# aras-p/ToyPathTracer

Hardware: AMD Instinct MI355X
Metric: Mray/s (higher is better)
Workload: dtype f32

## Files before the change

include/tpt_hip.h:

```cpp
#ifndef TPT_HIP_H
#define TPT_HIP_H
#include <stdint.h>

#if defined(__GNUC__)
#define TPT_API __attribute__((visibility("default")))
#else
#define TPT_API
#endif

#ifdef __cplusplus
extern "C" {
#endif

enum { TPT_FLAG_ANIMATE = 1 << 0, TPT_FLAG_PROGRESSIVE = 1 << 1 };


TPT_API int tptInitialize(void);
TPT_API int tptShutdown(void);
TPT_API int tptUpdate(float time, int frameCount, int screenWidth, int screenHeight, unsigned testFlags);
TPT_API int tptDraw(float time, int frameCount, int screenWidth, int screenHeight, float* backbuffer, int* outRayCount,
            unsigned testFlags);
TPT_API int tptSetHostBufferMode(int hostBufferOnlyWrittenByDrawTest);
TPT_API int tptSetHostLookahead(int frames);
TPT_API int tptGetLookaheadHits(long long* outHits);
TPT_API int tptGetObjectCount(int* outCount, int* outObjectSize, int* outMaterialSize, int* outCamSize);
TPT_API int tptGetSceneDesc(void* outObjects, void* outMaterials, void* outCam, void* outEmissives, int* outEmissiveCount);


TPT_API int tptSetSamplesPerPixel(int spp);
TPT_API int tptSetConfig(int lightSampling, float animateSmoothing, int mitsubaCompare);
TPT_API int tptSetSeedMode(int mode);
TPT_API int tptSetFoldMode(int mode);
TPT_API int tptSetScene(const void* spheres, const void* materials, int count);
TPT_API int tptSetCamera(const float* lookFrom, const float* lookAt, float vfovDegrees, float aperture, float focusDist);


TPT_API int tptSetStream(void* hipStream);
TPT_API int tptSetRowShard(int stripeRows, int numParts, int part);
TPT_API int tptLocalRowCount(int screenHeight);
TPT_API int tptLocalRowToGlobal(int localRow);
TPT_API int tptDrawDevice(float time, int frameCount, int screenWidth, int screenHeight, float* deviceTile, unsigned testFlags);
TPT_API int tptDrawDeviceBatch(float time, int firstFrame, int nFrames, int screenWidth, int screenHeight, float* deviceTile, unsigned testFlags);
TPT_API int tptDrawDeviceAnimation(int firstFrame, int nFrames, const float* times, int screenWidth, int screenHeight,
                                   float* deviceTile, float* deviceFrameImages, int64_t* deviceFrameRays, unsigned testFlags);
TPT_API int tptDrawDeviceAov(float time, int frameCount, int screenWidth, int screenHeight, float* deviceTile,
                             float* deviceAlbedo, float* deviceNormalDepth, unsigned testFlags);
enum { TPT_DENOISE_DEMODULATE = 1 << 0 };
TPT_API int tptDenoiseDevice(int screenWidth, int screenHeight, const float* deviceColour, const float* deviceAlbedo,
                             const float* deviceNormalDepth, float* deviceOut, int iterations, float sigmaColour,
                             float sigmaNormal, float sigmaDepth, unsigned denoiseFlags);
TPT_API int tptDrawDeviceMoments(float time, int frameCount, int screenWidth, int screenHeight, float* deviceTile,
                                 float* deviceAlbedo, float* deviceNormalDepth, float* deviceMoments, unsigned testFlags);
TPT_API int tptDrawDeviceAnimationMoments(int firstFrame, int nFrames, const float* times, int screenWidth, int screenHeight,
                                          float* deviceTile, float* deviceMoments,
                                          float* deviceFrameImages, float* deviceFrameAlbedo, float* deviceFrameNormalDepth,
                                          float* deviceFrameMoments, int64_t* deviceFrameRays, unsigned testFlags);
TPT_API int tptDrawDeviceCameraClip(int firstFrame, int nFrames, const float* times, const float* views,
                                    int screenWidth, int screenHeight, float* deviceTile, float* deviceMoments,
                                    float* deviceFrameImages, float* deviceFrameAlbedo, float* deviceFrameNormalDepth,
                                    float* deviceFrameMoments, int64_t* deviceFrameRays, void* outCameras, unsigned testFlags);
#define TPT_DENOISE_VARIANCE_EPS 1e-4f
TPT_API int tptDenoiseDeviceVariance(int screenWidth, int screenHeight, const float* deviceColour, const float* deviceAlbedo,
                                     const float* deviceNormalDepth, const float* deviceMoments, float samples, float* deviceOut,
                                     int iterations, float sigmaLuminance, float sigmaNormal, float sigmaDepth, unsigned denoiseFlags);
#define TPT_TEMPORAL_SNAP (1.0f / 128)
TPT_API int tptTemporalAccumulateDevice(int screenWidth, int screenHeight, const void* camera, const void* prevCamera,
                                        const float* deviceColour, const float* deviceAlbedo, const float* deviceNormalDepth,
                                        const float* deviceMoments, const float* devicePrevColour, const float* devicePrevAlbedo,
                                        const float* devicePrevNormalDepth, const float* devicePrevMoments, float* deviceOutColour,
                                        float* deviceOutAlbedo, float* deviceOutMoments, float* deviceOutVariance, float maxHistory,
                                        float depthTolerance, float normalTolerance, float coverageTolerance);
TPT_API int tptDrawDeviceAdaptive(float time, int frameCount, int screenWidth, int screenHeight, float* deviceTile, float* deviceAlbedo,
                                  float* deviceNormalDepth, float* deviceMoments, const int32_t* deviceSampleCounts,
                                  unsigned testFlags);
#define TPT_ADAPTIVE_LUM_FLOOR 1e-2f
TPT_API int tptAdaptiveSamplesDevice(int screenWidth, int screenHeight, const float* deviceMoments, float targetError, int minSamples,
                                     int maxSamples, int32_t* deviceSampleCounts, float* deviceOutVariance,
                                     int64_t* deviceTotalSamples);
TPT_API int tptDrawDeviceViews(float time, int frameCount, int screenWidth, int screenHeight, int nViews, const float* views,
                               float* deviceTiles, int64_t* deviceViewRays, unsigned testFlags);
TPT_API int tptSetFrameOverlap(int frames);
TPT_API int tptSetStreamBatching(int enable);
TPT_API int tptDisplayRGBA8(const float* deviceTile, int screenWidth, int screenHeight, unsigned char* deviceRGBA);
TPT_API int tptRayCounterRead(int64_t* outTotalRays);
TPT_API int tptSetRayCounter(void* deviceU64);
TPT_API int tptSetTileMirror(float* deviceMirror, void* deviceCounterOut);
TPT_API int tptSynchronize(void);

#define TPT_COMM_ID_BYTES 128
TPT_API int tptCommGetUniqueId(void* outId128);
TPT_API int tptCommInit(const void* id128, int nRanks, int rank, int stripeRows);
TPT_API int tptCommInitLoopback(int nRanks, int stripeRows);
TPT_API int tptCommInfo(int* outRanks, int* outRank, int* outLoopback);
TPT_API int tptCommDestroy(void);
TPT_API int tptDrawSharded(float time, int frameCount, int screenWidth, int screenHeight, float* deviceImageOnRoot, unsigned testFlags);
TPT_API int tptSetShardExchangeInterval(int everyKFrames);
TPT_API int tptDrawShardedBatch(float time, int firstFrame, int nFrames, int screenWidth, int screenHeight, float* deviceImageOnRoot, unsigned testFlags);
TPT_API int tptShardedFinish(int64_t* outTotalRays);

TPT_API int tptTimerBegin(void);
TPT_API int tptTimerEnd(float* outMilliseconds);

TPT_API int tptKernelTimingBegin(int maxLaunches);
TPT_API int tptKernelTimingEnd(float* outSumMilliseconds, int* outLaunches);


TPT_API int tptSetKernelVariant(int hitSpheres, int persistent, int ldsScene);
TPT_API int tptGetSceneInfo(int* outSpheres, int* outGroups, int* outBoundsOnMatrixCores);
TPT_API int tptGetLaunchInfo(int* outBlocksPerCU, int* outLdsBytes, int* outGridBlocks, int* outNumCUs);
TPT_API int tptGetPipelineInfo(int* outHwQueues, int* outOverlapEffective, int* outStreamDepth, int* outSlotReservations);
TPT_API const char* tptGetLastError(void);
typedef void (*tptErrorHandler)(const char* where, const char* message);
TPT_API int tptSetErrorHandler(tptErrorHandler handler);
TPT_API const char* tptGetDeviceName(void);

#ifdef __cplusplus
}
#endif
#endif
```

include/tpt_test_hooks.h:

```cpp
#ifndef TPT_TEST_HOOKS_H
#define TPT_TEST_HOOKS_H
#include "tpt_hip.h"
#ifdef __cplusplus
extern "C" {
#endif
TPT_API int tptTestMath(int op, const float* a, const float* b, float* out, int n);
TPT_API int tptTestHitSpheres(int hitSpheres, const float* rays, int* outId, float* outT, int n);
TPT_API int tptTestMathExhaustive(int op, unsigned lo, unsigned hi, unsigned long long* outMismatches, unsigned* outFirst8);
TPT_API int tptTestMatrixFilter(const float* rays, unsigned long long* outMask, int* outId, float* outT, int n);
TPT_API int tptTestGroupFilter(const float* rays, int n, unsigned long long* outViolations, unsigned long long* outTouched, unsigned long long* outExact);
TPT_API int tptTestSetDealCapacities(int superGroupEntries, int groupEntries, int survivorEntries);
TPT_API int tptDebugStats(unsigned long long* out128, int reset);
TPT_API int tptDebugChunkOrder(unsigned* outCost, unsigned* outOrder, int capacity);
#ifdef __cplusplus
}
#endif
#endif
```

toypathtracer_amd/api.py:

```python
import ctypes as C
import os

import numpy as np

kFlagAnimate = 1 << 0
kFlagProgressive = 1 << 1
SEED_ROW_SERIAL, SEED_PER_PIXEL = 0, 1
FOLD_RECURSIVE, FOLD_FORWARD = 0, 1

SPHERE_DT = np.dtype([("cx", "<f4"), ("cy", "<f4"), ("cz", "<f4"), ("radius", "<f4"), ("invRadius", "<f4")])
MATERIAL_DT = np.dtype([("type", "<i4"), ("albedo", "<f4", 3), ("emissive", "<f4", 3), ("roughness", "<f4"), ("ri", "<f4")])
CAMERA_DT = np.dtype([("origin", "<f4", 3), ("lowerLeftCorner", "<f4", 3), ("horizontal", "<f4", 3), ("vertical", "<f4", 3),
                      ("uu", "<f4", 3), ("vv", "<f4", 3), ("ww", "<f4", 3), ("lensRadius", "<f4")])


class TptError(RuntimeError):
    pass


_lib = None
_product = None
_hooks = None

C_ABI_SYMBOLS = [
    "tptInitialize", "tptShutdown", "tptUpdate", "tptDraw", "tptGetObjectCount", "tptGetSceneDesc",
    "tptSetSamplesPerPixel", "tptSetConfig", "tptSetSeedMode", "tptSetFoldMode", "tptSetScene", "tptSetCamera", "tptSetStream",
    "tptSetRowShard", "tptLocalRowCount", "tptLocalRowToGlobal", "tptDrawDevice", "tptRayCounterRead", "tptSetRayCounter", "tptSetFrameOverlap", "tptDisplayRGBA8", "tptKernelTimingBegin", "tptKernelTimingEnd",
    "tptSynchronize", "tptTimerBegin", "tptTimerEnd", "tptSetKernelVariant",
    "tptDrawDeviceBatch", "tptDrawDeviceViews", "tptDrawDeviceAnimation", "tptDrawDeviceAov", "tptDenoiseDevice", "tptDrawDeviceMoments", "tptDrawDeviceAnimationMoments", "tptDrawDeviceCameraClip", "tptDenoiseDeviceVariance", "tptTemporalAccumulateDevice", "tptDrawDeviceAdaptive", "tptAdaptiveSamplesDevice", "tptDrawShardedBatch", "tptGetLookaheadHits", "tptCommGetUniqueId", "tptCommInit", "tptCommInitLoopback", "tptCommInfo", "tptCommDestroy", "tptDrawSharded", "tptSetShardExchangeInterval", "tptShardedFinish", "tptGetLaunchInfo", "tptGetPipelineInfo", "tptGetSceneInfo", "tptSetHostBufferMode", "tptSetHostLookahead", "tptSetStreamBatching", "tptSetTileMirror", "tptGetLastError", "tptSetErrorHandler", "tptGetDeviceName",
]
HOOK_SYMBOLS = ["tptTestMath", "tptTestMathExhaustive", "tptTestHitSpheres", "tptTestMatrixFilter", "tptTestGroupFilter", "tptTestSetDealCapacities", "tptDebugStats", "tptDebugChunkOrder"]
CXX_ABI_SYMBOLS = [
    "_Z14InitializeTestv", "_Z12ShutdownTestv", "_Z10UpdateTestfiiij", "_Z8DrawTestfiiiPfRij",
    "_Z14GetObjectCountRiS_S_S_", "_Z12GetSceneDescPvS_S_S_Pi",
]


def _lib_dir():
    return os.environ.get("TPT_LIB_DIR") or os.path.join(os.path.dirname(os.path.abspath(__file__)), "lib")


def library_path():
    return os.environ.get("TPT_LIB") or os.path.join(_lib_dir(), "libtoypathtracer_hip.so")


def hooks_library_path():
    return os.environ.get("TPT_LIB") or os.path.join(_lib_dir(), "libtoypathtracer_hip_hooks.so")


def _bind(path, hooks):
    lib = C.CDLL(path)
    i, f, u, p = C.c_int, C.c_float, C.c_uint, C.c_void_p
    sigs = {
        "tptInitialize": [], "tptShutdown": [], "tptUpdate": [f, i, i, i, u],
        "tptDraw": [f, i, i, i, p, C.POINTER(i), u],
        "tptGetObjectCount": [C.POINTER(i)] * 4, "tptGetSceneDesc": [p, p, p, p, C.POINTER(i)],
        "tptSetSamplesPerPixel": [i], "tptSetConfig": [i, f, i], "tptSetSeedMode": [i], "tptSetFoldMode": [i], "tptSetScene": [p, p, i],
        "tptSetCamera": [p, p, f, f, f], "tptSetStream": [p], "tptSetRowShard": [i, i, i], "tptLocalRowCount": [i],
        "tptLocalRowToGlobal": [i], "tptDrawDevice": [f, i, i, i, p, u], "tptRayCounterRead": [C.POINTER(C.c_int64)],
        "tptSetRayCounter": [p], "tptSetTileMirror": [p, p], "tptSetFrameOverlap": [i], "tptDisplayRGBA8": [p, i, i, p], "tptKernelTimingBegin": [i],
        "tptKernelTimingEnd": [C.POINTER(f), C.POINTER(i)],
        "tptSynchronize": [], "tptTimerBegin": [], "tptTimerEnd": [C.POINTER(f)], "tptSetKernelVariant": [i, i, i],
        "tptGetLaunchInfo": [C.POINTER(i)] * 4, "tptGetPipelineInfo": [C.POINTER(i)] * 4, "tptGetSceneInfo": [C.POINTER(i)] * 3, "tptCommGetUniqueId": [p], "tptCommInit": [p, i, i, i], "tptCommInitLoopback": [i, i], "tptCommInfo": [C.POINTER(i)] * 3, "tptCommDestroy": [], "tptDrawSharded": [f, i, i, i, p, u], "tptSetShardExchangeInterval": [i], "tptDrawShardedBatch": [f, i, i, i, i, p, u], "tptDrawDeviceBatch": [f, i, i, i, i, p, u], "tptDrawDeviceViews": [f, i, i, i, i, p, p, p, u], "tptDrawDeviceAnimation": [i, i, p, i, i, p, p, p, u], "tptDrawDeviceAov": [f, i, i, i, p, p, p, u], "tptDenoiseDevice": [i, i, p, p, p, p, i, f, f, f, u], "tptDrawDeviceMoments": [f, i, i, i, p, p, p, p, u], "tptDrawDeviceAnimationMoments": [i, i, p, i, i] + [p] * 7 + [u], "tptDrawDeviceCameraClip": [i, i, p, p, i, i] + [p] * 8 + [u], "tptDenoiseDeviceVariance": [i, i, p, p, p, p, f, p, i, f, f, f, u], "tptTemporalAccumulateDevice": [i, i] + [p] * 14 + [f] * 4, "tptDrawDeviceAdaptive": [f, i, i, i, p, p, p, p, p, u], "tptAdaptiveSamplesDevice": [i, i, p, f, i, i, p, p, p], "tptShardedFinish": [C.POINTER(C.c_int64)], "tptSetHostBufferMode": [i], "tptGetLookaheadHits": [C.POINTER(C.c_longlong)], "tptSetHostLookahead": [i], "tptSetStreamBatching": [i],
    }
    if hooks:
        sigs.update({"tptDebugStats": [p, i], "tptDebugChunkOrder": [p, p, i], "tptTestMath": [i, p, p, p, i], "tptTestMathExhaustive": [i, u, u, p, p],
                     "tptTestHitSpheres": [i, p, p, p, i], "tptTestMatrixFilter": [p, p, p, p, i], "tptTestGroupFilter": [p, i, p, p, p], "tptTestSetDealCapacities": [i, i, i]})
    for name, args in sigs.items():
        fn = getattr(lib, name)
        fn.argtypes = args
        fn.restype = i
    lib.tptGetLastError.restype = C.c_char_p
    lib.tptGetDeviceName.restype = C.c_char_p
    return lib


def _preload():
    try:
        import torch
    except ImportError:
        pass


def load_library():
    global _lib, _product
    if _lib is not None:
        return _lib
    _preload()
    path = library_path()
    if not os.path.exists(path):
        raise TptError(f"{path} is missing: build it with `python -c 'import __graft_entry__ as g; g.build()'` "
                       "(toypathtracer_amd/csrc/build.sh). There is no CPU fallback.")
    _product = _bind(path, hooks=bool(os.environ.get("TPT_LIB")) and _has_hooks(path))
    _lib = _product
    return _lib


def _has_hooks(path):
    try:
        return hasattr(C.CDLL(path), "tptTestMath")
    except OSError:
        return False


class using_hooks:

    def __enter__(self):
        global _lib, _hooks
        load_library()
        if _hooks is None:
            path = hooks_library_path()
            if path == library_path():
                _hooks = _product
            else:
                if not os.path.exists(path):
                    raise TptError(f"{path} is missing (toypathtracer_amd/csrc/build.sh builds it beside the product library)")
                _hooks = _bind(path, hooks=True)
        self._prev = _lib
        _lib = _hooks
        _chk(_lib.tptInitialize(), "tptInitialize (hooks build)")
        return self

    def __exit__(self, *exc):
        global _lib
        if _lib is not _product:
            _lib.tptShutdown()
        _lib = self._prev
        return False


def shutdown_hooks():
    global _hooks
    if _hooks is not None and _hooks is not _product:
        _hooks.tptShutdown()
    _hooks = None


def _hook(name):
    fn = getattr(load_library(), name, None)
    if fn is None:
        raise TptError(f"{name} is a unit-test hook (include/tpt_test_hooks.h): call it inside `with api.using_hooks():` -- the product library does not export it")
    return fn


def _chk(rc, where):
    if rc != 0:
        raise TptError(f"{where}: {_lib.tptGetLastError().decode()}")


def InitializeTest():
# ... 382 lines not shown
def temporal_accumulate_device(w, h, camera, colour_ptr, albedo_ptr, normal_depth_ptr, moments_ptr, out_colour_ptr, out_albedo_ptr,
                               out_moments_ptr, out_variance_ptr, prev=None, max_history=TEMPORAL_DEFAULTS["max_history"],
                               depth_tolerance=TEMPORAL_DEFAULTS["depth_tolerance"],
                               normal_tolerance=TEMPORAL_DEFAULTS["normal_tolerance"],
                               coverage_tolerance=TEMPORAL_DEFAULTS["coverage_tolerance"]):
    _positive_ints(("w", w), ("h", h))
    cur = (("colour_ptr", colour_ptr), ("albedo_ptr", albedo_ptr), ("normal_depth_ptr", normal_depth_ptr), ("moments_ptr", moments_ptr),
           ("out_colour_ptr", out_colour_ptr), ("out_albedo_ptr", out_albedo_ptr), ("out_moments_ptr", out_moments_ptr),
           ("out_variance_ptr", out_variance_ptr))
    _pointers(*cur)
    if not all(v for _, v in cur):
        raise ValueError("%s: device buffers are required" % ", ".join(n for n, v in cur if not v))
    cam = _camera_bytes("camera", camera)
    prev_cam, prev_ptrs = None, (None,) * 4
    if prev is not None:
        if not isinstance(prev, (tuple, list)) or len(prev) != 5:
            raise ValueError("prev: None or (camera, colour_ptr, albedo_ptr, normal_depth_ptr, moments_ptr) expected, got %r" % (prev,))
        prev_cam = _camera_bytes("prev camera", prev[0])
        named = tuple(zip(("prev colour_ptr", "prev albedo_ptr", "prev normal_depth_ptr", "prev moments_ptr"), prev[1:]))
        _pointers(*named)
        if not all(v for _, v in named):
            raise ValueError("prev: all four device buffers are required")
        prev_ptrs = tuple(C.c_void_p(v) for v in prev[1:])
    if not isinstance(max_history, (int, float, np.integer, np.floating)) or isinstance(max_history, bool) or not 1 <= max_history <= 65536:
        raise ValueError("max_history: a number in 1..65536 expected, got %r" % (max_history,))
    _sigmas(("depth_tolerance", depth_tolerance), ("normal_tolerance", normal_tolerance), ("coverage_tolerance", coverage_tolerance))
    _chk(load_library().tptTemporalAccumulateDevice(w, h, cam, prev_cam, C.c_void_p(colour_ptr), C.c_void_p(albedo_ptr),
                                                    C.c_void_p(normal_depth_ptr), C.c_void_p(moments_ptr), *prev_ptrs,
                                                    C.c_void_p(out_colour_ptr), C.c_void_p(out_albedo_ptr), C.c_void_p(out_moments_ptr),
                                                    C.c_void_p(out_variance_ptr), max_history, depth_tolerance, normal_tolerance,
                                                    coverage_tolerance), "tptTemporalAccumulateDevice")


ADAPTIVE_MAX_SAMPLES = 2047


def draw_device_adaptive(time, frame, w, h, tile_ptr, moments_ptr, counts_ptr, flags, albedo_ptr=None, normal_depth_ptr=None):
    _positive_ints(("w", w), ("h", h))
    _pointers(("tile_ptr", tile_ptr), ("moments_ptr", moments_ptr), ("counts_ptr", counts_ptr), ("albedo_ptr", albedo_ptr),
              ("normal_depth_ptr", normal_depth_ptr))
    if not tile_ptr or not moments_ptr or not counts_ptr:
        raise ValueError("tile_ptr, moments_ptr, counts_ptr: device buffers are required")
    _chk(load_library().tptDrawDeviceAdaptive(time, frame, w, h, C.c_void_p(tile_ptr), C.c_void_p(albedo_ptr) if albedo_ptr else None,
                                              C.c_void_p(normal_depth_ptr) if normal_depth_ptr else None, C.c_void_p(moments_ptr),
                                              C.c_void_p(counts_ptr), flags), "tptDrawDeviceAdaptive")


def adaptive_samples_device(w, h, moments_ptr, target_error, counts_ptr, min_samples=0, max_samples=64, out_variance_ptr=None,
                            total_ptr=None):
    _positive_ints(("w", w), ("h", h))
    _pointers(("moments_ptr", moments_ptr), ("counts_ptr", counts_ptr), ("out_variance_ptr", out_variance_ptr), ("total_ptr", total_ptr))
    if not moments_ptr or not counts_ptr:
        raise ValueError("moments_ptr, counts_ptr: device buffers are required")
    if not isinstance(target_error, (int, float, np.integer, np.floating)) or isinstance(target_error, bool) or not 0 < target_error <= 1e6:
        raise ValueError("target_error: a float in (0, 1e6] expected, got %r" % (target_error,))
    for name, v in (("min_samples", min_samples), ("max_samples", max_samples)):
        if not isinstance(v, (int, np.integer)) or isinstance(v, bool) or not 0 <= v <= ADAPTIVE_MAX_SAMPLES:
            raise ValueError("%s: an int in 0..%d expected, got %r" % (name, ADAPTIVE_MAX_SAMPLES, v))
    if min_samples > max_samples:
        raise ValueError("min_samples: at most max_samples (%d) expected, got %d" % (max_samples, min_samples))
    _chk(load_library().tptAdaptiveSamplesDevice(w, h, C.c_void_p(moments_ptr), target_error, min_samples, max_samples,
                                                 C.c_void_p(counts_ptr), C.c_void_p(out_variance_ptr) if out_variance_ptr else None,
                                                 C.c_void_p(total_ptr) if total_ptr else None), "tptAdaptiveSamplesDevice")


def sharded_finish():
    v = C.c_int64()
    _chk(load_library().tptShardedFinish(C.byref(v)), "tptShardedFinish")
    return v.value


def set_host_buffer_mode(only_written_by_drawtest):
    _chk(load_library().tptSetHostBufferMode(1 if only_written_by_drawtest else 0), "tptSetHostBufferMode")


def set_host_lookahead(frames):
    _chk(load_library().tptSetHostLookahead(frames), "tptSetHostLookahead")


def set_stream_batching(enable):
    _chk(load_library().tptSetStreamBatching(1 if enable else 0), "tptSetStreamBatching")


def lookahead_hits():
    v = C.c_longlong()
    _chk(load_library().tptGetLookaheadHits(C.byref(v)), "tptGetLookaheadHits")
    return v.value


def pipeline_info():
    v = [C.c_int() for _ in range(4)]
    _chk(load_library().tptGetPipelineInfo(*[C.byref(x) for x in v]), "tptGetPipelineInfo")
    return dict(hw_queues=v[0].value, overlap_effective=v[1].value, stream_depth=v[2].value, slot_reservations=v[3].value)


def scene_info():
    v = [C.c_int() for _ in range(3)]
    _chk(load_library().tptGetSceneInfo(*[C.byref(x) for x in v]), "tptGetSceneInfo")
    return dict(spheres=v[0].value, groups=v[1].value, bounds_on_matrix_cores=bool(v[2].value))


def debug_stats(reset=True):
    out = np.zeros(128, np.uint64)
    _chk(_hook("tptDebugStats")(out.ctypes.data, 1 if reset else 0), "tptDebugStats")
    return out


def debug_chunk_order(capacity=1 << 20):
    cost = np.zeros(capacity, np.uint32)
    order = np.zeros(capacity, np.uint32)
    n = _hook("tptDebugChunkOrder")(cost.ctypes.data, order.ctypes.data, capacity)
    if n < 0:
        raise TptError("tptDebugChunkOrder: " + _lib.tptGetLastError().decode())
    return cost[:n].copy(), order[:n].copy()


def device_name():
    return load_library().tptGetDeviceName().decode()


def test_math(op, a, b=None):
    a = np.ascontiguousarray(a, np.float32)
    out = np.empty_like(a)
    bp = None
    if b is not None:
        b = np.ascontiguousarray(b, np.float32)
        bp = b.ctypes.data
    _chk(_hook("tptTestMath")(op, a.ctypes.data, bp, out.ctypes.data, a.size), "tptTestMath")
    return out


def test_math_exhaustive(op, lo=0, hi=0xFFFFFFFF):
    bad = C.c_ulonglong(0)
    first = (C.c_uint * 8)()
    _chk(_hook("tptTestMathExhaustive")(op, lo, hi, C.byref(bad), first), "tptTestMathExhaustive")
    return int(bad.value), [int(v) for v in first][: min(8, int(bad.value))]


def test_hit_spheres(rays, hit_spheres=0):
    rays = np.ascontiguousarray(rays, np.float32).reshape(-1, 6)
    n = rays.shape[0]
    ids = np.empty(n, np.int32)
    ts = np.empty(n, np.float32)
    _chk(_hook("tptTestHitSpheres")(hit_spheres, rays.ctypes.data, ids.ctypes.data, ts.ctypes.data, n),
         "tptTestHitSpheres")
    return ids, ts


def test_matrix_filter(rays, hits=False):
    rays = np.ascontiguousarray(rays, np.float32).reshape(-1, 6)
    n = rays.shape[0]
    masks = np.empty(n, np.uint64)
    ids = np.empty(n, np.int32) if hits else None
    ts = np.empty(n, np.float32) if hits else None
    _chk(_hook("tptTestMatrixFilter")(rays.ctypes.data, masks.ctypes.data, ids.ctypes.data if hits else None,
                                            ts.ctypes.data if hits else None, n), "tptTestMatrixFilter")
    return (masks, ids, ts) if hits else masks


def test_set_deal_capacities(super_group_entries=0, group_entries=0, survivor_entries=0):
    _chk(_hook("tptTestSetDealCapacities")(super_group_entries, group_entries, survivor_entries), "tptTestSetDealCapacities")


def test_group_filter(rays):
    rays = np.ascontiguousarray(rays, np.float32).reshape(-1, 6)
    n = rays.shape[0]
    v = [C.c_ulonglong(0) for _ in range(3)]
    _chk(_hook("tptTestGroupFilter")(rays.ctypes.data, n, C.byref(v[0]), C.byref(v[1]), C.byref(v[2])), "tptTestGroupFilter")
    return int(v[0].value), v[1].value / n, v[2].value / n
```

toypathtracer_amd/csrc/tpt_context.h:

```cpp
#pragma once
#include "../../include/tpt_hip.h"
#if defined(TPT_TEST_HOOKS)
#include "../../include/tpt_test_hooks.h"
#endif
#include "../../include/tpt_test_api.h"
#include "tpt_device.h"
#include "tpt_queue_layout.h"
#include "tpt_scene.h"
#include "tpt_shard.h"
#include "tpt_stream_batch.h"
#include "tpt_animation.h"
#include <hip/hip_runtime.h>
#include <thread>
#include <rccl/rccl.h>
#include <chrono>
#include <dlfcn.h>
#include <map>
#include <stdio.h>
#include <stdlib.h>
#include <string>


namespace tpth {
using namespace tpt;

const int kMaxBatch = 32;
static_assert(kMaxBatch == TPT_Q_VIEWS_MAX, "a batch's cameras, centres and ray counts have their places in the path-queue kernel's LDS");
struct TraceTicket {
    int slot = 0, nPixels = 0;
    bool pipelined = false, valid = false;
    float lerpFac = 0;
    const f4* colour = nullptr;
    int batch = 1;
    tptLerpTable lerp = {};
    const f4* moments = nullptr;
    TraceTicket plane(int j) const
    {
        TraceTicket t = *this;
        t.colour = colour + (size_t)j * (size_t)nPixels;
        if (batch > 1) t.lerpFac = lerp.v[j];
        t.batch = 1;
        return t;
    }
};

struct Streak {
    int frame = 0, w = 0, h = 0, n = 0;
    unsigned flags = 0;
    unsigned long long key = 0;
    int next(int frame_, int w_, int h_, unsigned flags_, unsigned long long key_)
    {
        n = frame_ == frame + 1 && w_ == w && h_ == h && flags_ == flags && key_ == key ? n + 1 : 0;
        frame = frame_; w = w_; h = h_; flags = flags_; key = key_;
        return n;
    }
};

struct PendingLaunch {
    enum Kind { AHEAD, ROW_SERIAL, STREAM } kind = AHEAD;
    TraceTicket T;
    int firstFrame = 0, next = 0;
    int w = 0, h = 0;
    unsigned flags = 0;
    unsigned long long key = 0;
    unsigned long long* rays = nullptr;
};
struct LaunchQueue {
    static const int kCap = 4;
    PendingLaunch e[kCap];
    int n = 0;
    bool empty() const { return n == 0; }
    bool holds(PendingLaunch::Kind kind) const { return n > 0 && e[0].kind == kind; }
    bool frontMatches(PendingLaunch::Kind kind, int frame, int w, int h, unsigned flags, unsigned long long key) const;
    void serveFront(bool wasOpen, TraceTicket& T, const unsigned long long*& rays);
    int push(const PendingLaunch& L);
    int discard();
    void closeStream();
};

struct Context {
    static const int kMaxOverlap = 16;
    static const int kMaxSlots = 2 * kMaxOverlap;
    static const int kOrderTables = kMaxSlots + 2;
    bool inited = false;
    int device = 0, numCUs = 0;
    int traceCUs = 0;
    std::string deviceName, err;
    hipStream_t ownStream = nullptr, stream = nullptr;
    hipEvent_t ev0 = nullptr, ev1 = nullptr;

    std::vector<SpherePOD> spheres;
    std::vector<MaterialPOD> mats;
    CameraSetup camSetup = defaultCameraSetup();
    CameraPOD cam;
    PackedScene packed;
    bool sceneDirty = true;
    bool updated = false;
    int updatedW = 0, updatedH = 0;

    static const int kSceneSets = 2 * kMaxSlots;
    struct SceneSet {
        char* dev = nullptr;
        char* stage = nullptr;
        size_t cap = 0, bytes = 0;
        size_t offSph4 = 0, offInvR = 0, offMats = 0, offLights = 0;
        size_t offGPairs = 0, offGSph = 0, offGId = 0, offBSph = 0, offBId = 0;
        size_t offSPairs = 0;
        int nSuperPairs = 0;
        size_t offAmat = 0;
        int mxR1 = -1;
        size_t offGmat = 0;
        int gmxTiles = 0;
        int flags = 0;
        int nSpheres = 0, nPairs = 0, nLights = 0;
        int nGroups = 0, nGroupPairs = 0, nBig = 0;
        hipEvent_t evUploaded = nullptr;
        hipStream_t uploadStream = nullptr;
        bool copyEnqueued = false, copyDone = false;
    } sets[kSceneSets];
    int curSet = -1, pendingSet = -1;
    unsigned uploadSeq = 0;

    int spp = 4;
    int config = CFG_LIGHT_SAMPLING;
    float animateSmoothing = 0.9f;
    int seedMode = SEED_PER_PIXEL;
    int foldMode = FOLD_RECURSIVE;
    int allowGroups = 1;
    int useMatrix = 1;
    int groupMatrix = 0;
    int hs = HS_TWO_PHASE, persist = 3, ldsScene = -1;
    int stripeRows = 0, numParts = 1, part = 0;
    int gridFill = 0;
    int gridDiv = 0;
    unsigned long long oldestPending = 0;
    int streamDepth = 1, prevInFlight = -1;
    int depthOverride = 0;
    int ldsStackLevels = 6;

    float* mirror = nullptr;
    unsigned long long* mirrorCounter = nullptr;
    unsigned* dWork = nullptr;
    unsigned long long* dRays = nullptr;
    unsigned long long* dRaysOwn = nullptr;
    long long lastTotal = 0;

    f4* dStack[kMaxSlots] = {};
    size_t stackCap = 0, colourCap = 0;
    int slotsReserved = 0;
    int smallStreak = 0;
    int slotReservations = 0;
    unsigned* dChunkCost = nullptr;
    unsigned* dChunkOrder[kOrderTables] = {};
    unsigned* dChunkSnap[kMaxOverlap] = {};
    int chunkCap = 0, chunkCount = 0;
    int costOrder = 1;
    hipEvent_t evOrder = nullptr;
    hipStream_t orderStream = nullptr;
    unsigned long long orderSeq = 0;
    int lastOrderTable = 0;
    float* dFrame = nullptr;
    hipStream_t hostStream2 = nullptr;
    hipEvent_t evBand = nullptr, evBandEnd = nullptr;
    int hostTrust = 0;
    const float* tileSrc = nullptr;
    int tileW = 0, tileH = 0;
    int lookahead = 2;
    LaunchQueue pending;
    struct HostCaller {
        Streak seq;
        int refusedW = 0, refusedH = 0;
        unsigned long long refusedKey = 0;
    } hostCaller;
    static const int kStreamBatchMax = 8, kStreamRing = 64;
    unsigned long long streamBatches = 0;
    int streamRun = 0, streamNext = -1;
    int streamBatch = 1;
    struct DeviceCaller {
        int lastSlot = -1, syncStreak = 0;
        Streak seq;
    } devCaller;
    struct ViewSlot {
        CameraPOD* dev = nullptr;
        unsigned long long* rays = nullptr;
        CameraPOD* stage = nullptr;
        hipEvent_t evUploaded = nullptr;
        bool copyEnqueued = false;
    } views[kMaxSlots];
    char* dViews = nullptr;
    CameraPOD* hViewsStage = nullptr;
    f4* dAovSums = nullptr;
    size_t aovSumsBytes = 0;
    hipEvent_t evAov = nullptr;
    f4* dMoments = nullptr;
    size_t momentsBytes = 0;
    hipEvent_t evClip[2] = {nullptr, nullptr};
    unsigned clipSeq = 0;
    f4* dDenoise = nullptr;
    size_t denoiseBytes = 0;
    long long aheadHits = 0;
    unsigned long long *dRaysAhead = nullptr, *dRaysBatch = nullptr, *dRaysStream = nullptr;
    unsigned long long configEpoch = 1;

    struct Shard {
        static const int kRing = 4;
        void* lib = nullptr;
        ncclComm_t comm = nullptr;
        bool active = false, loopback = false;
        int nRanks = 0, rank = 0, stripeRows = 8;
        int w = 0, h = 0, padRows = 0;
        hipStream_t commStream = nullptr;
        float* tile = nullptr;
        float* send[kRing] = {};
        float* gathered = nullptr;
        hipEvent_t evSnap[kRing] = {}, evSent[kRing] = {};
        bool sentRecorded[kRing] = {};
        unsigned long long frames = 0;
        int exchangeEvery = 0;
        int pendCount = 0, pendFirst = 0, pendW = 0, pendH = 0;
        unsigned pendFlags = 0;
        float pendTime = 0.0f;
        float* lastImage = nullptr;
        decltype(&ncclGetUniqueId) GetUniqueId = nullptr;
        decltype(&ncclCommInitRank) CommInitRank = nullptr;
        decltype(&ncclCommDestroy) CommDestroy = nullptr;
        decltype(&ncclGather) Gather = nullptr;
        decltype(&ncclCommCount) CommCount = nullptr;
        decltype(&ncclCommUserRank) CommUserRank = nullptr;
        decltype(&ncclGetErrorString) GetErrorString = nullptr;
    } shard;
    size_t frameCap = 0;

    int overlap = 16;
    hipStream_t traceStream[kMaxOverlap] = {};
    hipEvent_t evTrace[kMaxSlots] = {}, evResolve[kMaxSlots] = {};
    bool resolveRecorded[kMaxSlots] = {};
    f4* dColour[kMaxSlots] = {};
    int hwQueues = 0, overlapCap = kMaxOverlap;
    int slotFactor = 2;
    hipEvent_t evPre[kMaxSlots] = {};
    struct HelperRec {
        KernelArgs a;
        bool ldsScene = false, valid = false, helped = false;
        hipStream_t ts = nullptr;
        int blocks = 0, maxBlocks = 0;
        size_t lds = 0;
    } hrec[kMaxSlots];
    unsigned launchGen = 0;
    int helpersOn = 1;
    static const int kHelperPct = 3;
    static const int kHelperMax = 8;
    long long helperLaunches = 0;
    int hostPace = 1;
    int shardOverlapCap = kMaxOverlap;
    unsigned long long frameSeq = 0;

    bool kernelTiming = false;
    std::vector<hipEvent_t> ktStart, ktStop;
    size_t ktUsed = 0;

    std::map<int, int> occCache;
    int lastBlocksPerCU = 0, lastLds = 0, lastGrid = 0;
};

extern Context g;

struct DepthScope {
    explicit DepthScope(int d) { g.depthOverride = d; }
    ~DepthScope() { g.depthOverride = 0; }
};

const unsigned kOrderingEvent = hipEventDisableTiming;
const unsigned kTimingEvent = hipEventDefault;

inline int fail(const std::string& what)
{
    g.err = what;
    return -1;
}
inline int hipFail(hipError_t e, const char* what)
{
    g.err = std::string(what) + ": " + hipGetErrorString(e);
    (void)hipGetLastError();
    return -2;
}
const int kRefused = -4;
inline int refuse(const std::string& what)
{
    g.err = what;
    return kRefused;
}
inline bool overlapsAny(const void* p, std::initializer_list<const void*> others, uintptr_t bytes)
{
    const uintptr_t a = reinterpret_cast<uintptr_t>(p);
    for (const void* other : others) {
        const uintptr_t o = reinterpret_cast<uintptr_t>(other);
        if (other && a < o + bytes && o < a + bytes) return true;
    }
    return false;
}
#define HIPCHK(x)                                   \
    do {                                            \
        hipError_t _e = (x);                        \
        if (_e != hipSuccess) return hipFail(_e, #x); \
    } while (0)

int localRows(int h);
int localToGlobal(int ly);
int stageScene();
Context::SceneSet* activeSet();
SceneView deviceView();
int enqueueSceneUpload(hipStream_t ts);
int framesInFlight(int nOverlap);
int uploadBackbuffer(const float* backbuffer, int w, int h);
int requireInit();
int drainPipeline();
int effectiveOverlap();
struct BatchTable {
    const CameraPOD* cams = nullptr;
    const f4* centres = nullptr;
};
struct AovPlanes {
    f4* albedo = nullptr;
    f4* normalDepth = nullptr;
    bool moments = false;
    bool continues = false;
    const int32_t* sampleCounts = nullptr;
};
int enqueueTrace(int frameCount, int w, int h, unsigned testFlags, unsigned long long* frameRays, TraceTicket& T, int batch = 1, int rayStride = 0,
                 const BatchTable* table = nullptr, const AovPlanes* aov = nullptr);
int enqueueResolve(const TraceTicket& T, float* deviceTile, const unsigned long long* frameRays);
int syncAllStreams();
int launchTailHelpers();
int flushShardDeferred();
int traceAhead(int frameCount, int w, int h, unsigned testFlags, unsigned long long key, int want);

}
```

toypathtracer_amd/csrc/tpt_device.h:

```cpp
#pragma once
#include "tpt_trace.h"

#ifndef TPT_BLOCK
#define TPT_BLOCK 64
#endif
#define TPT_CHUNK_PIXELS 256

namespace tpt {

struct KernelArgs {
    SceneView scene;
    FrameConsts fc;
    f4* frameColour;
    int nLocalRows, stripeRows, stripeStride, stripeOffset;
    int tilesX;
    int numItems;
    int numChunks, chunkSize;
    int batchFrames, chunksPerFrame, framePlane;
    unsigned totalWaves;
    int laneCap;
    int noRefill;
    f4* stackBuf;
    int stackStride;
    int ldsStackLevels;
    f4* pathBuf;
    const unsigned* chunkOrder;
    unsigned* chunkCost;
    int chunkShift;
    unsigned* work;
    unsigned long long* rayCounter;
    int rayCounterStride;
    unsigned gen;
    int helperBase;
    int helperPct;
    int ldsGroupPairs;
    const CameraPOD* viewCams = nullptr;
    const f4* moveCentres = nullptr;
    f4* aovSums = nullptr;
    f4* aovAlbedo = nullptr;
    f4* aovNormalDepth = nullptr;
    f4* momentsOut = nullptr;
    int aovPlane = 0;
    const int32_t* sampleCounts = nullptr;
};

}

hipError_t tptLaunchTrace(const tpt::KernelArgs& a, int hs, int fold, bool ldsScene, int blocks, size_t lds, hipStream_t stream);
int tptTraceOccupancy(int hs, int fold, bool ldsScene, size_t lds);
hipError_t tptLaunchTraceQueue(const tpt::KernelArgs& a, bool ldsScene, int blocks, size_t lds, hipStream_t stream);
int tptQueueMatrixFilter();
int tptQueueGroupMatrixBounds();
hipError_t tptLaunchDisplay(const float* tile, unsigned char* rgba, int width, int height, hipStream_t stream);
__attribute__((weak)) hipError_t tptLaunchDenoise(const float* colour, const float* albedo, const float* normalDepth, float* out,
                                                  float* scratch, int width, int height, int iterations, float ic, float in, float id,
                                                  bool demodulate, hipStream_t stream);
__attribute__((weak)) hipError_t tptLaunchDenoiseVariance(const float* colour, const float* albedo, const float* normalDepth,
                                                          const float* moments, float* out, float* scratch, int width, int height,
                                                          int iterations, float samples, float sl2, float in, float id, bool demodulate,
                                                          hipStream_t stream);
struct tptTemporalConsts {
    float o[3], ll[3], H[3], V[3];
    float po[3], pa[3], pw[3], pH[3], pV[3];
    float pf, phh, pvv;
    float maxHistory, depthTol, normalTol, coverageTol;
};
__attribute__((weak)) hipError_t tptLaunchTemporal(const float* colour, const float* albedo, const float* normalDepth, const float* moments,
                                                   const float* prevColour, const float* prevAlbedo, const float* prevNormalDepth,
                                                   const float* prevMoments, float* outColour, float* outAlbedo, float* outMoments,
                                                   float* outVariance, int width, int height, const tptTemporalConsts& k,
                                                   hipStream_t stream);
__attribute__((weak)) hipError_t tptLaunchAdaptiveResolve(float* tile, float* moments, const tpt::f4* frameColour, const tpt::f4* stagedMoments,
                                                          const int32_t* counts, int nPixels, bool progressive, hipStream_t stream);
__attribute__((weak)) hipError_t tptLaunchAdaptivePlan(const float* moments, int32_t* counts, float* outVariance, int64_t* totalSamples,
                                                       int width, int height, float targetError, int minSamples, int maxSamples,
                                                       hipStream_t stream);
hipError_t tptLaunchAssemble(const float* gathered, float* image, int width, int height, int stripeRows, int nRanks, int padRows, hipStream_t stream);
hipError_t tptLaunchQueueProbe(unsigned long long ticks, hipStream_t stream);
hipError_t tptLaunchChunkOrder(const unsigned* cost, unsigned* snap, unsigned* order, int numChunks, hipStream_t stream);
struct tptLerpTable { float v[32]; };
hipError_t tptLaunchResolveBatch(float* tile, const tpt::f4* frameColour, int nPixels, int planeStride, int nFrames, const tptLerpTable& lerp,
                                 float* mirror, unsigned long long* rayCounter, unsigned long long* counterOut, hipStream_t stream);
hipError_t tptLaunchResolve(float* tile, const tpt::f4* frameColour, int nPixels, float lerpFac, float* mirror,
                            unsigned long long* rayCounter, unsigned long long* counterOut, const unsigned long long* frameRays, hipStream_t stream);
hipError_t tptLaunchMathTest(int op, const float* a, const float* b, float* out, int n, hipStream_t stream);
hipError_t tptLaunchMathExhaustive(int op, unsigned lo, unsigned hi, unsigned long long* nBad, unsigned* firstBad, hipStream_t stream);
hipError_t tptLaunchMatrixFilterTest(const tpt::KernelArgs& a, const float* rays, unsigned long long* outMask, int* outId, float* outT, int n, hipStream_t stream);
hipError_t tptSetDealCapacitiesForTest(int ca, int cb, int cs);
hipError_t tptLaunchGroupFilterTest(const tpt::KernelArgs& a, const float* rays, int n, int nPad, unsigned long long* out4, hipStream_t stream);
hipError_t tptLaunchHitTest(const tpt::KernelArgs& a, int hs, const float* rays, int* outId, float* outT, int n, hipStream_t stream);
int tptReadStats(unsigned long long* out64);
int tptResetStats();
```

toypathtracer_amd/csrc/tpt_host.cpp:

```cpp
#include "tpt_context.h"

using namespace tpt;
using namespace tpth;

namespace tpth {

Context g;

int localRows(int h) { return shardLocalRows(h, g.stripeRows, g.numParts, g.part); }
int localToGlobal(int ly) { return shardLocalToGlobal(ly, g.stripeRows, g.numParts, g.part); }

template <class T>
int ensureDev(T*& p, int& cap, int need)
{
    if (need <= cap && p) return 0;
    if (p) HIPCHK(hipFree(p));
    p = nullptr;
    int n = need < 64 ? 64 : need;
    HIPCHK(hipMalloc(reinterpret_cast<void**>(&p), sizeof(T) * (size_t)n));
    cap = n;
    return 0;
}

size_t align256(size_t v) { return (v + 255) & ~(size_t)255; }
// ... 198 lines not shown
}

int createTraceStreams()
{
    g.traceCUs = g.numCUs;
    for (int k = 0; k < Context::kMaxOverlap; ++k) HIPCHK(hipStreamCreateWithFlags(&g.traceStream[k], hipStreamNonBlocking));
    return 0;
}

int drainPipeline()
{
    if (g.inited) {
        if (g.pending.discard()) return -2;
        HIPCHK(hipStreamSynchronize(g.stream));
        for (int k = 0; k < Context::kMaxOverlap; ++k)
            if (g.traceStream[k]) HIPCHK(hipStreamSynchronize(g.traceStream[k]));
    }
    g.oldestPending = g.frameSeq;
    g.streamDepth = 1; g.prevInFlight = -1;
    for (int k = 0; k < Context::kMaxSlots; ++k) g.resolveRecorded[k] = false;
    return 0;
}
int effectiveOverlap()
{
    int n = g.overlap < 1 ? 1 : (g.overlap > Context::kMaxOverlap ? Context::kMaxOverlap : g.overlap);
    if (n > g.overlapCap) n = g.overlapCap;
    if (n > g.shardOverlapCap) n = g.shardOverlapCap;
    return n;
}

}

extern "C" {

const char* tptGetLastError(void) { return g.err.c_str(); }
const char* tptGetDeviceName(void) { return g.deviceName.c_str(); }

int tptInitialize(void)
{
    if (g.inited) return 0;
    int count = 0;
    hipError_t e = hipGetDeviceCount(&count);
    if (e != hipSuccess || count <= 0)
        return fail("tptInitialize: no HIP device visible (this library has no CPU fallback)");
    int dev = 0;
    const char* env = getenv("TPT_DEVICE");
    if (!env) env = getenv("LOCAL_RANK");
    if (env) dev = atoi(env);
    if (dev < 0) return fail("tptInitialize: negative device index in TPT_DEVICE / LOCAL_RANK");
    if (dev >= count) dev = dev % count;
    HIPCHK(hipSetDevice(dev));
    hipDeviceProp_t prop;
    HIPCHK(hipGetDeviceProperties(&prop, dev));
    g.device = dev;
    g.numCUs = prop.multiProcessorCount;
    g.deviceName = std::string(prop.name) + " (" + prop.gcnArchName + ")";
    HIPCHK(hipStreamCreateWithFlags(&g.ownStream, hipStreamDefault));
    g.stream = g.ownStream;
    HIPCHK(hipEventCreateWithFlags(&g.evOrder, kOrderingEvent));
    HIPCHK(hipEventCreate(&g.ev0));
    HIPCHK(hipEventCreate(&g.ev1));
    HIPCHK(hipMalloc(reinterpret_cast<void**>(&g.dWork), 64 * Context::kMaxSlots));
    HIPCHK(hipMemsetAsync(g.dWork, 0, 64 * Context::kMaxSlots, g.stream));
    {
        int rc = createTraceStreams();
        if (rc) return rc;
    }
    for (int k = 0; k < Context::kMaxSlots; ++k) {
        HIPCHK(hipEventCreateWithFlags(&g.evTrace[k], kOrderingEvent));
        HIPCHK(hipEventCreateWithFlags(&g.evResolve[k], kOrderingEvent));
        g.resolveRecorded[k] = false;
    }

    g.frameSeq = 0;
    g.oldestPending = 0;
    HIPCHK(hipStreamCreateWithFlags(&g.hostStream2, hipStreamNonBlocking));
    HIPCHK(hipEventCreateWithFlags(&g.evBand, kOrderingEvent));
    HIPCHK(hipEventCreateWithFlags(&g.evBandEnd, kOrderingEvent));
    const size_t pendingRays = sizeof(unsigned long long) * (Context::kMaxSlots + 2 * kMaxBatch + Context::kStreamRing * Context::kStreamBatchMax);
    HIPCHK(hipMalloc(reinterpret_cast<void**>(&g.dRaysAhead), pendingRays));
    HIPCHK(hipMemsetAsync(g.dRaysAhead, 0, pendingRays, g.stream));
    g.dRaysBatch = g.dRaysAhead + Context::kMaxSlots;
    g.dRaysStream = g.dRaysBatch + 2 * kMaxBatch;
    g.pending.n = 0;
    if (const char* esb = getenv("TPT_STREAM_BATCH")) g.streamBatch = atoi(esb) != 0;
    HIPCHK(hipMalloc(reinterpret_cast<void**>(&g.dRaysOwn), 64));
    HIPCHK(hipMemsetAsync(g.dRaysOwn, 0, 64, g.stream));
    HIPCHK(hipStreamSynchronize(g.stream));
    g.dRays = g.dRaysOwn;
    g.lastTotal = 0;
    if (g.spheres.empty()) defaultScene(g.spheres, g.mats);
    if (const char* e6 = getenv("TPT_GRID_FILL")) g.gridFill = atoi(e6);
    if (const char* e7 = getenv("TPT_HOST_PACE")) g.hostPace = atoi(e7);
    if (const char* eh = getenv("TPT_TAIL_HELPERS")) g.helpersOn = atoi(eh) != 0;
    for (int k = 0; k < Context::kMaxSlots; ++k) {
        HIPCHK(hipEventCreateWithFlags(&g.evPre[k], kOrderingEvent));
        g.hrec[k].valid = false;
    }
    g.launchGen = 0;
    if (const char* e5 = getenv("TPT_GRID_DIV")) g.gridDiv = atoi(e5) > 0 ? atoi(e5) : 0;
    g.sceneDirty = true;
    {
        int rc = probeHardwareQueues();
        if (rc) return rc;
    }
    g.inited = true;
    return 0;
}

int tptShutdown(void)
{
    if (!g.inited) return 0;
    (void)g.pending.discard();
    (void)tptCommDestroy();
    (void)hipStreamSynchronize(g.stream);
    (void)hipDeviceSynchronize();
    for (int k = 0; k < Context::kMaxSlots; ++k) {
        if (g.evPre[k]) (void)hipEventDestroy(g.evPre[k]);
        g.evPre[k] = nullptr;
        g.hrec[k].valid = false;
    }
    for (int k = 0; k < Context::kSceneSets; ++k) {
        Context::SceneSet& S = g.sets[k];
        (void)hipFree(S.dev);
        if (S.stage) (void)hipHostFree(S.stage);
        if (S.evUploaded) (void)hipEventDestroy(S.evUploaded);
        S = Context::SceneSet();
    }
    g.curSet = -1; g.pendingSet = -1; g.uploadSeq = 0;
    (void)hipFree(g.dWork); (void)hipFree(g.dRaysOwn); (void)hipFree(g.dFrame);
    (void)hipFree(g.dChunkCost); g.dChunkCost = nullptr; g.chunkCap = 0; g.chunkCount = 0; g.orderSeq = 0;
    for (int k = 0; k < Context::kOrderTables; ++k) { (void)hipFree(g.dChunkOrder[k]); g.dChunkOrder[k] = nullptr; }
    for (int k = 0; k < Context::kMaxOverlap; ++k) { (void)hipFree(g.dChunkSnap[k]); g.dChunkSnap[k] = nullptr; }
    g.dWork = nullptr; g.dRays = nullptr; g.dRaysOwn = nullptr; g.dFrame = nullptr;
    g.frameCap = 0;
    for (size_t i = 0; i < g.ktStart.size(); ++i) { (void)hipEventDestroy(g.ktStart[i]); (void)hipEventDestroy(g.ktStop[i]); }
    g.ktStart.clear(); g.ktStop.clear(); g.ktUsed = 0; g.kernelTiming = false;
    for (int k = 0; k < Context::kMaxOverlap; ++k) {
        if (g.traceStream[k]) { (void)hipStreamSynchronize(g.traceStream[k]); (void)hipStreamDestroy(g.traceStream[k]); }
        g.traceStream[k] = nullptr;
    }
    for (int k = 0; k < Context::kMaxSlots; ++k) {
        if (g.evTrace[k]) (void)hipEventDestroy(g.evTrace[k]);
        if (g.evResolve[k]) (void)hipEventDestroy(g.evResolve[k]);
        (void)hipFree(g.dColour[k]);
        (void)hipFree(g.dStack[k]); g.dStack[k] = nullptr;
        g.evTrace[k] = nullptr; g.evResolve[k] = nullptr; g.dColour[k] = nullptr;
    }
    g.stackCap = g.colourCap = 0; g.slotsReserved = 0; g.slotReservations = 0;
    (void)hipEventDestroy(g.ev0); (void)hipEventDestroy(g.ev1);
    if (g.evOrder) { (void)hipEventDestroy(g.evOrder); g.evOrder = nullptr; }
    (void)hipStreamDestroy(g.ownStream);
    g.ownStream = g.stream = nullptr;
    for (int k = 0; k < Context::kMaxSlots; ++k) {
        if (g.views[k].evUploaded) (void)hipEventDestroy(g.views[k].evUploaded);
        g.views[k] = Context::ViewSlot();
    }
    (void)hipFree(g.dViews); g.dViews = nullptr;
    (void)hipFree(g.dAovSums); g.dAovSums = nullptr;
    g.aovSumsBytes = 0;
    if (g.evAov) { (void)hipEventDestroy(g.evAov); g.evAov = nullptr; }
    for (hipEvent_t& e : g.evClip)
        if (e) { (void)hipEventDestroy(e); e = nullptr; }
    (void)hipFree(g.dMoments); g.dMoments = nullptr;
    g.momentsBytes = 0;
    (void)hipFree(g.dDenoise); g.dDenoise = nullptr;
    g.denoiseBytes = 0;
    if (g.hViewsStage) (void)hipHostFree(g.hViewsStage);
    g.hViewsStage = nullptr;
    g.inited = false;
    g.updated = false;
    g.updatedW = g.updatedH = 0;
    g.occCache.clear();
    g.mirror = nullptr; g.mirrorCounter = nullptr;
    if (g.hostStream2) { (void)hipStreamSynchronize(g.hostStream2); (void)hipStreamDestroy(g.hostStream2); g.hostStream2 = nullptr; }
    if (g.evBand) { (void)hipEventDestroy(g.evBand); g.evBand = nullptr; }
    if (g.evBandEnd) { (void)hipEventDestroy(g.evBandEnd); g.evBandEnd = nullptr; }
    g.tileSrc = nullptr; g.tileW = g.tileH = 0;
    g.pending.n = 0;
    (void)hipFree(g.dRaysAhead); g.dRaysAhead = g.dRaysBatch = g.dRaysStream = nullptr;
    g.orderStream = nullptr; g.oldestPending = 0; g.frameSeq = 0;
    g.streamDepth = 1; g.prevInFlight = -1;
    g.hostCaller = Context::HostCaller(); g.devCaller = Context::DeviceCaller();
    g.smallStreak = 0; g.configEpoch = 1;
    return 0;
}

int tptSetStream(void* hipStream)
{
    if (int rc_ = flushShardDeferred()) return rc_;
    if (requireInit()) return -1;
    if (g.pending.discard()) return -2;
    HIPCHK(hipStreamSynchronize(g.stream));
    g.stream = hipStream ? reinterpret_cast<hipStream_t>(hipStream) : g.ownStream;
    return 0;
}

int tptSetSamplesPerPixel(int spp)
{
    if (int rc_ = flushShardDeferred()) return rc_;
    if (spp < 1 || spp > 65536) return fail("tptSetSamplesPerPixel: spp out of range");
    if (spp == g.spp) return 0;
    g.spp = spp;
    g.configEpoch++;
    return 0;
}
int tptSetConfig(int lightSampling, float animateSmoothing, int mitsubaCompare)
{
    if (int rc_ = flushShardDeferred()) return rc_;
    const int config = (lightSampling ? CFG_LIGHT_SAMPLING : 0) | (mitsubaCompare ? CFG_MITSUBA_COMPARE : 0);
    if (config == g.config && animateSmoothing == g.animateSmoothing) return 0;
    g.config = config;
    g.animateSmoothing = animateSmoothing;
    g.configEpoch++;
    return 0;
}
int tptSetSeedMode(int mode)
{
    if (int rc_ = flushShardDeferred()) return rc_;
    if (mode != SEED_ROW_SERIAL && mode != SEED_PER_PIXEL) return fail("tptSetSeedMode: 0 (ROW_SERIAL) or 1 (PER_PIXEL)");
    if (mode == g.seedMode) return 0;
    g.seedMode = mode;
    g.configEpoch++;
    return 0;
}
int tptSetFoldMode(int mode)
{
    if (int rc_ = flushShardDeferred()) return rc_;
    if (mode != FOLD_RECURSIVE && mode != FOLD_FORWARD) return fail("tptSetFoldMode: 0 (RECURSIVE) or 1 (FORWARD)");
    if (mode == g.foldMode) return 0;
    g.foldMode = mode;
    g.configEpoch++;
    return 0;
}
int tptKernelTimingBegin(int maxLaunches)
{
    if (requireInit()) return -1;
    if (maxLaunches < 1) maxLaunches = 1;
    while ((int)g.ktStart.size() < maxLaunches) {
        hipEvent_t a = nullptr, b = nullptr;
        HIPCHK(hipEventCreateWithFlags(&a, kTimingEvent));
        HIPCHK(hipEventCreateWithFlags(&b, kTimingEvent));
        g.ktStart.push_back(a);
        g.ktStop.push_back(b);
    }
    g.ktUsed = 0;
    g.kernelTiming = true;
    return 0;
}

int tptKernelTimingEnd(float* outSumMs, int* outLaunches)
{
    if (requireInit()) return -1;
    g.kernelTiming = false;
    HIPCHK(hipStreamSynchronize(g.stream));
    double sum = 0;
    for (size_t i = 0; i < g.ktUsed; ++i) {
        HIPCHK(hipEventSynchronize(g.ktStop[i]));
        float ms = 0;
        HIPCHK(hipEventElapsedTime(&ms, g.ktStart[i], g.ktStop[i]));
        sum += ms;
    }
    if (outSumMs) *outSumMs = (float)sum;
// ... 219 lines not shown
```

toypathtracer_amd/csrc/tpt_host_draw.cpp:

```cpp
#include "tpt_context.h"

using namespace tpt;
using namespace tpth;

namespace tpth {

bool LaunchQueue::frontMatches(PendingLaunch::Kind kind, int frame, int w, int h, unsigned flags, unsigned long long key) const
{
    const PendingLaunch& F = e[0];
    return holds(kind) && frame == F.firstFrame + F.next && F.w == w && F.h == h && F.flags == flags && F.key == key;
}

void LaunchQueue::serveFront(bool wasOpen, TraceTicket& T, const unsigned long long*& rays)
{
    PendingLaunch& F = e[0];
    if (wasOpen && F.kind != PendingLaunch::STREAM) g.aheadHits++;
    T = F.T.plane(F.next);
    rays = F.rays + F.next;
    if (++F.next < F.T.batch) return;
    for (int k = 0; k + 1 < n; ++k) e[k] = e[k + 1];
    --n;
}

int LaunchQueue::push(const PendingLaunch& L)
{
    if (n == kCap || (n > 0 && !holds(L.kind))) return fail("internal: launch queue full or of another kind");
    e[n++] = L;
    return 0;
}

int LaunchQueue::discard()
{
    if (n > 0 && !holds(PendingLaunch::STREAM))
        for (int k = 0; k < Context::kMaxOverlap; ++k) HIPCHK(hipStreamSynchronize(g.traceStream[k]));
    n = 0;
    return 0;
}

void LaunchQueue::closeStream()
{
    if (holds(PendingLaunch::STREAM)) n = 0;
    g.streamNext = -1;
}

int traceAhead(int frameCount, int w, int h, unsigned testFlags, unsigned long long key, int want)
{
    LaunchQueue& Q = g.pending;
    int nextFrame = Q.n ? Q.e[Q.n - 1].firstFrame + 1 : frameCount + 1;
    const int nSlots = effectiveOverlap();
    const int maxAhead = want < nSlots - 2 ? want : nSlots - 2;
    while (Q.n < maxAhead) {
        PendingLaunch A;
        A.firstFrame = nextFrame++; A.w = w; A.h = h; A.flags = testFlags; A.key = key;
        A.rays = g.dRaysAhead + g.frameSeq % (unsigned long long)Context::kMaxSlots;
        int rc = enqueueTrace(A.firstFrame, w, h, testFlags, A.rays, A.T);
        if (rc) return rc;
        if (!A.T.valid) break;
        if ((rc = Q.push(A))) return rc;
    }
    return 0;
}

static int checkDenoise(const char* fn, bool variance, int w, int h, const float* colour, const float* albedo, const float* normalDepth,
                        const float* moments, const float* out, int iterations, float samples, float sigma0, float sigmaNormal,
                        float sigmaDepth, unsigned flags)
{
    const std::string f(fn);
    if (w < 1 || w > 8192 || h < 1 || h > 8192) return fail(f + ": w and h must lie in 1..8192");
    if (!colour || !out) return fail(f + ": deviceColour and deviceOut are required");
    if (variance && !moments) return fail(f + ": deviceMoments is required");
    if (overlapsAny(out, {colour, albedo, normalDepth, moments}, (uintptr_t)w * (uintptr_t)h * 16u)) return fail(f + ": deviceOut overlaps an input");
    if (iterations < 1 || iterations > 8) return fail(f + ": iterations must lie in 1..8");
    auto sigmaOk = [](float s) { return s == 0.0f || (s >= 1e-6f && s <= 1e6f); };
    if (variance) {
        if (!(samples >= 1.0f && samples <= 3.40282347e38f)) return fail(f + ": samples must be finite and at least 1");
        if (!(sigma0 > 0.0f && sigma0 <= 1e6f)) return fail(f + ": sigmaLuminance must lie in (0, 1e6]");
        if (!sigmaOk(sigmaNormal) || !sigmaOk(sigmaDepth)) return fail(f + ": sigmaNormal and sigmaDepth must be 0 or lie in [1e-6, 1e6]");
    } else if (!sigmaOk(sigma0) || !sigmaOk(sigmaNormal) || !sigmaOk(sigmaDepth)) {
        return fail(f + ": every sigma must be 0 or lie in [1e-6, 1e6]");
    }
    if ((sigmaNormal != 0.0f || sigmaDepth != 0.0f) && !normalDepth) return fail(f + ": sigmaNormal and sigmaDepth need deviceNormalDepth");
    if (flags & ~(unsigned)TPT_DENOISE_DEMODULATE) return fail(f + ": unknown flag bits");
    if ((flags & TPT_DENOISE_DEMODULATE) && !albedo) return fail(f + ": TPT_DENOISE_DEMODULATE needs deviceAlbedo");
    return 0;
}

static int ensureDenoisePlane(int w, int h)
{
    const uintptr_t bytes = (uintptr_t)w * (uintptr_t)h * 16u;
    if (bytes <= g.denoiseBytes) return 0;
    HIPCHK(hipStreamSynchronize(g.stream));
    (void)hipFree(g.dDenoise);
    g.dDenoise = nullptr;
    g.denoiseBytes = 0;
    HIPCHK(hipMalloc(reinterpret_cast<void**>(&g.dDenoise), bytes));
    g.denoiseBytes = bytes;
    return 0;
}

}

extern "C" {

int tptSetHostBufferMode(int hostBufferOnlyWrittenByDrawTest)
{
    g.hostTrust = hostBufferOnlyWrittenByDrawTest ? 1 : 0;
    g.tileSrc = nullptr;
    return 0;
}

int tptSetStreamBatching(int enable)
{
    if (requireInit()) return -1;
    int rc = g.pending.discard();
    if (rc) return rc;
    g.streamBatch = enable ? 1 : 0;
    return 0;
}

int tptSetHostLookahead(int frames)
{
    if (frames < 0 || frames > 3) return fail("tptSetHostLookahead: 0..3");
    if (g.inited) {
        int rc = g.pending.discard();
        if (rc) return rc;
// ... 270 lines not shown
```

toypathtracer_amd/csrc/tpt_host_hooks.cpp:

```cpp
#include "tpt_context.h"

using namespace tpt;
using namespace tpth;

extern "C" {
#if defined(TPT_TEST_HOOKS)
int tptDebugChunkOrder(unsigned* outCost, unsigned* outOrder, int capacity)
{
    if (requireInit()) return -1;
    HIPCHK(hipStreamSynchronize(g.stream));
    for (int k = 0; k < Context::kMaxOverlap; ++k) HIPCHK(hipStreamSynchronize(g.traceStream[k]));
    int n = g.chunkCount < capacity ? g.chunkCount : capacity;
    if (n <= 0 || !g.dChunkCost) return 0;
    if (outCost) HIPCHK(hipMemcpy(outCost, g.dChunkCost, sizeof(unsigned) * n, hipMemcpyDeviceToHost));
    if (outOrder) HIPCHK(hipMemcpy(outOrder, g.dChunkOrder[g.lastOrderTable], sizeof(unsigned) * n, hipMemcpyDeviceToHost));
    return n;
}

int tptDebugStats(unsigned long long* out64, int reset)
{
    if (requireInit()) return -1;
    HIPCHK(hipStreamSynchronize(g.stream));
    int rc = out64 ? tptReadStats(out64) : 0;
    if (rc == -1) return fail("tptDebugStats: library not built with -DTPT_STATS (profiling build, tools/build_stats.sh)");
// ... 69 lines not shown
    HIPCHK(hipMemcpy(dr, padded.data(), sizeof(float) * 6 * nPad, hipMemcpyHostToDevice));
    HIPCHK(tptLaunchMatrixFilterTest(a, dr, dm, outId ? di : nullptr, dt, nPad, g.stream));
    HIPCHK(hipStreamSynchronize(g.stream));
    if (outMask) HIPCHK(hipMemcpy(outMask, dm, sizeof(unsigned long long) * n, hipMemcpyDeviceToHost));
    if (outId) {
        HIPCHK(hipMemcpy(outId, di, sizeof(int) * n, hipMemcpyDeviceToHost));
        HIPCHK(hipMemcpy(outT, dt, sizeof(float) * n, hipMemcpyDeviceToHost));
    }
    (void)hipFree(dr); (void)hipFree(dm); (void)hipFree(di); (void)hipFree(dt);
    return 0;
}

int tptTestGroupFilter(const float* rays, int n, unsigned long long* outViolations, unsigned long long* outTouched, unsigned long long* outExact)
{
    if (requireInit()) return -1;
    if (!rays || n <= 0 || !outViolations) return fail("tptTestGroupFilter: bad arguments");
    if (g.sceneDirty || (g.curSet < 0 && g.pendingSet < 0)) {
        int rc = stageScene();
        if (rc) return rc;
    }
    int rc = enqueueSceneUpload(g.stream);
    if (rc) return rc;
    KernelArgs a;
    memset(&a, 0, sizeof(a));
    a.scene = deviceView();
    if (a.scene.nGroups <= 0 || (a.scene.gmxTiles <= 0 && a.scene.nSuperPairs <= 0)) return fail("tptTestGroupFilter: the current scene is not grouped (fewer than 256 spheres, a group too loose, or hit-spheres variant 2)");
    const int nPad = (n + 63) / 64 * 64;
    float* dr = nullptr;
    unsigned long long* dout = nullptr;
    HIPCHK(hipMalloc(reinterpret_cast<void**>(&dr), sizeof(float) * 6 * (size_t)nPad));
    HIPCHK(hipMalloc(reinterpret_cast<void**>(&dout), sizeof(unsigned long long) * 4));
    HIPCHK(hipMemsetAsync(dr, 0, sizeof(float) * 6 * (size_t)nPad, g.stream));
    HIPCHK(hipMemsetAsync(dout, 0, sizeof(unsigned long long) * 4, g.stream));
    HIPCHK(hipMemcpyAsync(dr, rays, sizeof(float) * 6 * (size_t)n, hipMemcpyHostToDevice, g.stream));
    HIPCHK(tptLaunchGroupFilterTest(a, dr, n, nPad, dout, g.stream));
    unsigned long long h[4] = {0, 0, 0, 0};
    HIPCHK(hipMemcpyAsync(h, dout, sizeof(h), hipMemcpyDeviceToHost, g.stream));
    HIPCHK(hipStreamSynchronize(g.stream));
    *outViolations = h[0];
    if (outTouched) *outTouched = h[1];
    if (outExact) *outExact = h[2];
    (void)hipFree(dr); (void)hipFree(dout);
    return 0;
}

int tptTestSetDealCapacities(int superGroupEntries, int groupEntries, int survivorEntries)
{
    if (requireInit()) return -1;
    if (int rc = tptSynchronize()) return rc;
    if (tptSetDealCapacitiesForTest(superGroupEntries, groupEntries, survivorEntries) != hipSuccess)
        return fail("tptTestSetDealCapacities: each size between 64 and its compiled value, or 0, 0, 0 for the compiled ones");
    return 0;
}

int tptTestHitSpheres(int hitSpheres, const float* rays, int* outId, float* outT, int n)
{
    if (requireInit()) return -1;
    if (!rays || !outId || !outT || n <= 0) return fail("tptTestHitSpheres: bad arguments");
    if (g.sceneDirty || (g.curSet < 0 && g.pendingSet < 0)) {
        int rc = stageScene();
        if (rc) return rc;
    }
    {
        int rc = enqueueSceneUpload(g.stream);
        if (rc) return rc;
    }
    float *dr = nullptr, *dt = nullptr;
    int* di = nullptr;
    HIPCHK(hipMalloc(reinterpret_cast<void**>(&dr), sizeof(float) * 6 * n));
    HIPCHK(hipMalloc(reinterpret_cast<void**>(&dt), sizeof(float) * n));
    HIPCHK(hipMalloc(reinterpret_cast<void**>(&di), sizeof(int) * n));
    HIPCHK(hipMemcpy(dr, rays, sizeof(float) * 6 * n, hipMemcpyHostToDevice));
    KernelArgs a;
    memset(&a, 0, sizeof(a));
    a.scene = deviceView();
    HIPCHK(tptLaunchHitTest(a, hitSpheres == 1 ? HS_SIMPLE : HS_TWO_PHASE, dr, di, dt, n, g.stream));
    HIPCHK(hipStreamSynchronize(g.stream));
    HIPCHK(hipMemcpy(outId, di, sizeof(int) * n, hipMemcpyDeviceToHost));
    HIPCHK(hipMemcpy(outT, dt, sizeof(float) * n, hipMemcpyDeviceToHost));
    (void)hipFree(dr); (void)hipFree(dt); (void)hipFree(di);
    return 0;
}

#endif
}
```

toypathtracer_amd/csrc/tpt_host_pipeline.cpp:

```cpp
#include "tpt_context.h"

using namespace tpt;
using namespace tpth;

namespace tpth {

struct FramePlan {
    KernelArgs a;
    bool rowSerial = false, queued = false, ldsScene = false, useOrder = false;
    size_t lds = 0;
    int occ = 0, threadsPerBlock = 0, blocks = 0;
    int nOverlap = 1;
    int nSlots = 1, slot = 0;
    int batch = 1;
};

int syncAllStreams();
int reserveSlotBuffers(int nSlots, size_t colourBytes, size_t stackBytes)
{
    const bool small = colourBytes * 4 <= g.colourCap && g.colourCap * (size_t)g.slotsReserved > (1ull << 30);
    g.smallStreak = small ? g.smallStreak + 1 : 0;
    const bool shrink = small && g.smallStreak >= 8 && g.pending.empty();
    if (shrink) g.smallStreak = 0;
    if (!shrink && nSlots <= g.slotsReserved && colourBytes <= g.colourCap && stackBytes <= g.stackCap) return 0;
// ... 266 lines not shown
    }
    if (g.chunkCount != a.numChunks) {
        int rc = syncAllStreams();
        if (rc) return rc;
        HIPCHK(hipMemsetAsync(g.dChunkCost, 0, bytes, g.stream));
        HIPCHK(hipStreamSynchronize(g.stream));
        g.chunkCount = a.numChunks;
        g.orderSeq = 0;
    }
    a.chunkCost = g.dChunkCost;
    return 0;
}

int enqueueChunkOrder(FramePlan& P, hipStream_t ts)
{
    if (!P.useOrder) return 0;
    if (g.orderSeq > 0) {
        const int fresh = (int)(g.orderSeq % Context::kOrderTables);
        if (g.orderSeq <= (unsigned long long)(2 * P.nSlots + 2) || (g.orderSeq & 31ull) == 0ull) {
            HIPCHK(tptLaunchChunkOrder(g.dChunkCost, g.dChunkSnap[P.slot % P.nOverlap], g.dChunkOrder[fresh], P.a.numChunks, ts));
            HIPCHK(hipEventRecord(g.evOrder, ts));
            g.orderStream = ts;
            g.lastOrderTable = fresh;
        } else if (g.orderStream && g.orderStream != ts) {
            HIPCHK(hipStreamWaitEvent(ts, g.evOrder, 0));
        }
        P.a.chunkOrder = g.dChunkOrder[g.lastOrderTable];
    }
    g.orderSeq++;
    return 0;
}

static const size_t kViewCamBytes = sizeof(CameraPOD) * kMaxBatch;
int ensureViewSlots()
{
    if (g.dViews) return 0;
    const size_t camBytes = kViewCamBytes, tableBytes = camBytes + 2 * sizeof(f4) * kMaxBatch, perSlot = tableBytes + sizeof(unsigned long long) * kMaxBatch;
    static_assert(kViewCamBytes % 16 == 0, "the centres and the ray counters behind a slot's cameras stay aligned");
    HIPCHK(hipMalloc(reinterpret_cast<void**>(&g.dViews), perSlot * Context::kMaxSlots));
    if (hipHostMalloc(reinterpret_cast<void**>(&g.hViewsStage), tableBytes * Context::kMaxSlots, 0) != hipSuccess) {
        (void)hipFree(g.dViews);
        g.dViews = nullptr;
        g.hViewsStage = nullptr;
        return hipFail(hipErrorOutOfMemory, "tptDrawDeviceViews: pinned camera staging");
    }
    for (int k = 0; k < Context::kMaxSlots; ++k) {
        Context::ViewSlot& V = g.views[k];
        V.dev = reinterpret_cast<CameraPOD*>(g.dViews + perSlot * k);
        V.rays = reinterpret_cast<unsigned long long*>(g.dViews + perSlot * k + tableBytes);
        V.stage = reinterpret_cast<CameraPOD*>(reinterpret_cast<char*>(g.hViewsStage) + tableBytes * k);
        V.copyEnqueued = false;
        if (!V.evUploaded) HIPCHK(hipEventCreateWithFlags(&V.evUploaded, kOrderingEvent));
    }
    return 0;
}

int ensureAovSums(const FramePlan& P, size_t momentsBytes, int halves)
{
    if (!g.evAov) HIPCHK(hipEventCreateWithFlags(&g.evAov, kOrderingEvent));
    for (hipEvent_t& e : g.evClip)
        if (!e) HIPCHK(hipEventCreateWithFlags(&e, kOrderingEvent));
    const size_t need = (momentsBytes ? 3 : 2) * sizeof(f4) * (size_t)maxGridBlocks(P) * (size_t)tptQueuePathsPerBlock() * (size_t)halves;
    momentsBytes *= (size_t)halves;
    if (need <= g.aovSumsBytes && momentsBytes <= g.momentsBytes) return 0;
    int rc = syncAllStreams();
    if (rc) return rc;
    if (need > g.aovSumsBytes) {
        (void)hipFree(g.dAovSums);
        g.dAovSums = nullptr;
        g.aovSumsBytes = 0;
        HIPCHK(hipMalloc(reinterpret_cast<void**>(&g.dAovSums), need));
        g.aovSumsBytes = need;
    }
    if (momentsBytes > g.momentsBytes) {
        (void)hipFree(g.dMoments);
        g.dMoments = nullptr;
        g.momentsBytes = 0;
        HIPCHK(hipMalloc(reinterpret_cast<void**>(&g.dMoments), momentsBytes));
        g.momentsBytes = momentsBytes;
    }
    return 0;
}

int enqueueTrace(int frameCount, int w, int h, unsigned testFlags, unsigned long long* frameRays, TraceTicket& T, int batch, int rayStride,
                 const BatchTable* table, const AovPlanes* aov)
{
    const CameraPOD* viewCams = table ? table->cams : nullptr;
    const f4* centres = table ? table->centres : nullptr;
    if (g.sceneDirty || (g.curSet < 0 && g.pendingSet < 0)) {
        int rc = stageScene();
        if (rc) return rc;
    }
    FramePlan P;
    KernelArgs& a = P.a;
    a.scene = deviceView();
    a.fc = makeFrameConsts(g.cam, w, h, g.spp, frameCount, testFlags, g.seedMode, g.config, g.animateSmoothing);
    a.nLocalRows = localRows(h);
    if (g.numParts > 1 && g.stripeRows > 0) {
        a.stripeRows = g.stripeRows;
        a.stripeStride = g.stripeRows * g.numParts;
        a.stripeOffset = g.stripeRows * g.part;
    } else {
        a.stripeRows = h > 0 ? h : 1;
        a.stripeStride = a.stripeRows;
        a.stripeOffset = 0;
    }
    T.valid = false;
    if (a.nLocalRows <= 0) return 0;
    a.tilesX = (w + 7) / 8;
    const int tilesY = (a.nLocalRows + 7) / 8;
    a.numItems = g.seedMode == SEED_ROW_SERIAL ? a.nLocalRows : a.tilesX * tilesY * 64;
    P.batch = batch;
    a.batchFrames = batch;
    a.framePlane = a.nLocalRows * w;
    a.chunksPerFrame = 0;
    P.nOverlap = effectiveOverlap();
    P.nSlots = P.nOverlap;
    const size_t colourBytesPerSlot = (size_t)a.nLocalRows * (size_t)w * sizeof(f4) * (size_t)batch;
    if (P.nOverlap > 1 && g.slotFactor > 1 && colourBytesPerSlot <= (32ull << 20)) P.nSlots = 2 * P.nOverlap;
    if (colourBytesPerSlot > (4ull << 30))
        return refuse("tptDrawDeviceBatch: " + std::to_string(colourBytesPerSlot >> 20) + " MiB of frame colour per launch (rows x width x 16 B x frames): over the 4096 MiB limit, use a smaller batch");
    while (P.nSlots > 2 && colourBytesPerSlot * (size_t)P.nSlots > (8ull << 30)) P.nSlots /= 2;
    if (rayStride > 0 && g.seedMode == SEED_ROW_SERIAL && P.nSlots > 4) P.nSlots = 4;
    if (P.nOverlap > P.nSlots) P.nOverlap = P.nSlots;
    P.slot = (int)(g.frameSeq % (unsigned long long)P.nSlots);
    g.frameSeq++;
    struct SeqGuard {
        bool launched = false;
        ~SeqGuard() { if (!launched) g.frameSeq--; }
    } seqGuard;

    int rc = 0;
    a.viewCams = nullptr;
    a.moveCentres = nullptr;
    a.sampleCounts = aov ? aov->sampleCounts : nullptr;
    if (table) {
        if ((rc = ensureViewSlots())) return rc;
        if (viewCams) a.viewCams = g.views[P.slot].dev;
        if (centres) a.moveCentres = reinterpret_cast<const f4*>(reinterpret_cast<const char*>(g.views[P.slot].dev) + (viewCams ? kViewCamBytes : 0));
        frameRays = g.views[P.slot].rays;
        rayStride = 1;
    }
    if ((rc = chooseKernel(P))) return rc;
    if (viewCams && !P.queued)
        return refuse("tptDrawDeviceViews: needs the path-queue kernel (per-pixel seeds, recursive fold, two-phase HitSpheres, at most 2047 spp)");
    if (centres && (!P.queued || a.scene.nGroups > 0))
        return refuse("tptDrawDeviceAnimation: one launch per batch needs the path-queue kernel and a flat scene");
    const bool clip = aov && aov->moments && centres;
    if (viewCams && centres && !clip) return fail("enqueueTrace: a camera and the centres per frame go with a clip's planes");
    if (aov && (!P.queued || !(clip || (batch == 1 && !viewCams && !centres))))
        return refuse("tptDrawDeviceAov: needs the path-queue kernel (per-pixel seeds, recursive fold, two-phase HitSpheres, at most 2047 spp)");
    if (batch > 1 && (!(P.queued || P.rowSerial) || w > 8192 || h > 8192 || (long long)a.nLocalRows * w * batch > (1ll << 30)))
        return refuse("tptDrawDeviceBatch: needs the path-queue kernel (per-pixel seeds, recursive fold, two-phase HitSpheres) or row-serial seeds, and a frame of at most 8192 x 8192 (2^30 pixels per batch)");
    sizeGrid(P);
    if ((rc = ensureFrameBuffers(P, w))) return rc;
    a.aovSums = a.aovAlbedo = a.aovNormalDepth = a.momentsOut = nullptr;
    if (aov) {
        if ((rc = ensureAovSums(P, aov->moments ? (size_t)a.nLocalRows * (size_t)w * sizeof(f4) * (size_t)batch : 0, clip ? 2 : 1))) return rc;
        const size_t half = clip ? (size_t)(g.clipSeq & 1u) : 0;
        a.aovSums = g.dAovSums + half * (g.aovSumsBytes / (2 * sizeof(f4)));
        a.aovAlbedo = aov->albedo;
        a.aovNormalDepth = aov->normalDepth;
        if (aov->moments) a.momentsOut = g.dMoments + half * (g.momentsBytes / (2 * sizeof(f4)));
        a.aovPlane = clip ? h * w : 0;
    }
    if (frameRays) a.rayCounter = frameRays;
    a.rayCounterStride = rayStride;
    if ((rc = prepareChunkOrder(P))) return rc;
    g.lastBlocksPerCU = P.occ;
    g.lastLds = (int)P.lds;
    g.lastGrid = P.blocks;

    const int slot = P.slot;
    const bool pipelined = P.nOverlap > 1;
    hipStream_t ts = pipelined ? g.traceStream[slot % P.nOverlap] : g.stream;
    if (pipelined && g.resolveRecorded[slot]) {
        if (g.hostPace) {
            const auto t0 = std::chrono::steady_clock::now();
            unsigned spins = 0;
            while (hipEventQuery(g.evResolve[slot]) == hipErrorNotReady) {
                std::this_thread::yield();
                if ((++spins & 255u) == 0u && std::chrono::steady_clock::now() - t0 > std::chrono::milliseconds(200)) break;
            }
            (void)hipGetLastError();
        }
        HIPCHK(hipStreamWaitEvent(ts, g.evResolve[slot], 0));
    }
    if ((rc = enqueueSceneUpload(ts))) return rc;
    if (aov && ts != g.stream) {
        if (clip) {
            const unsigned h = g.clipSeq & 1u;
            HIPCHK(hipEventRecord(g.evClip[h ^ 1u], g.stream));
            HIPCHK(hipStreamWaitEvent(ts, aov->continues ? g.evClip[h] : g.evClip[h ^ 1u], 0));
        } else {
            HIPCHK(hipEventRecord(g.evAov, g.stream));
            HIPCHK(hipStreamWaitEvent(ts, g.evAov, 0));
        }
    }
    if (clip) g.clipSeq++;
    if (viewCams || centres) {
        static_assert(2 * sizeof(f4) * kMaxBatch <= sizeof(CameraPOD) * kMaxBatch, "a batch's moving centres fit the slot's camera table");
        Context::ViewSlot& V = g.views[slot];
        const size_t camBytes = sizeof(CameraPOD) * (size_t)batch, centreBytes = 2 * sizeof(f4) * (size_t)batch;
        const size_t bytes = viewCams && centres ? kViewCamBytes + centreBytes : (viewCams ? camBytes : centreBytes);
        if (V.copyEnqueued) HIPCHK(hipEventSynchronize(V.evUploaded));
        if (viewCams) memcpy(V.stage, viewCams, camBytes);
        if (centres) memcpy(reinterpret_cast<char*>(V.stage) + (viewCams ? kViewCamBytes : 0), centres, centreBytes);
        HIPCHK(hipMemcpyAsync(V.dev, V.stage, bytes, hipMemcpyHostToDevice, ts));
        HIPCHK(hipEventRecord(V.evUploaded, ts));
        V.copyEnqueued = true;
    }
    if ((rc = enqueueChunkOrder(P, ts))) return rc;
    if (frameRays && frameRays != g.dRays) HIPCHK(hipMemsetAsync(frameRays, 0, sizeof(unsigned long long) * (size_t)(rayStride > 0 ? batch : 1), ts));
    const bool helpable = P.queued && pipelined && batch == 1 && !P.rowSerial && !table && !aov;
    a.helperBase = 0;
    a.helperPct = 0;
    a.gen = 0u;
    g.hrec[slot].valid = false;
    if (helpable) {
        if (++g.launchGen == 0u) g.launchGen = 1u;
        a.gen = g.launchGen;
        HIPCHK(hipEventRecord(g.evPre[slot], ts));
    }
    const bool timeIt = g.kernelTiming && g.ktUsed < g.ktStart.size();
    if (timeIt) HIPCHK(hipEventRecord(g.ktStart[g.ktUsed], ts));
    if (P.queued)
        HIPCHK(tptLaunchTraceQueue(a, P.ldsScene, P.blocks, P.lds, ts));
    else
        HIPCHK(tptLaunchTrace(a, g.hs, g.foldMode, P.ldsScene, P.blocks, P.lds, ts));
    seqGuard.launched = true;
    if (timeIt) {
        HIPCHK(hipEventRecord(g.ktStop[g.ktUsed], ts));
        g.ktUsed++;
    }
    if (pipelined) HIPCHK(hipEventRecord(g.evTrace[slot], ts));
    if (helpable) {
        Context::HelperRec& R = g.hrec[slot];
        R.a = a; R.ldsScene = P.ldsScene; R.blocks = P.blocks; R.maxBlocks = maxGridBlocks(P); R.lds = P.lds;
        R.helped = false; R.valid = true; R.ts = ts;
    }
    T.slot = slot;
    T.nPixels = a.nLocalRows * w;
    T.pipelined = pipelined;
    T.lerpFac = a.fc.lerpFac;
    T.colour = a.frameColour;
    T.moments = a.momentsOut;
    T.batch = batch;
    for (int j = 0; j < batch && batch > 1; ++j)
        T.lerp.v[j] = makeFrameConsts(g.cam, w, h, g.spp, frameCount + j, testFlags, g.seedMode, g.config, g.animateSmoothing).lerpFac;
    T.valid = true;
    return 0;
}

int enqueueResolve(const TraceTicket& T, float* deviceTile, const unsigned long long* frameRays)
{
    if (!T.valid) return 0;
    if (T.pipelined) HIPCHK(hipStreamWaitEvent(g.stream, g.evTrace[T.slot], 0));
    if (T.batch > 1)
        HIPCHK(tptLaunchResolveBatch(deviceTile, T.colour, T.nPixels, T.nPixels, T.batch, T.lerp, g.mirror, g.dRays, g.mirrorCounter, g.stream));
    else
        HIPCHK(tptLaunchResolve(deviceTile, T.colour, T.nPixels, T.lerpFac, g.mirror, g.dRays, g.mirrorCounter, frameRays, g.stream));
    if (T.pipelined) {
        HIPCHK(hipEventRecord(g.evResolve[T.slot], g.stream));
        g.resolveRecorded[T.slot] = true;
    }
    return 0;
}


enum { kQueueKernel = 1, kQueueSpp = 2 };
template <typename Own>
static int checkPathQueueDraw(const char* fn, const char* things, int w, int h, unsigned checks, Own own)
{
    const std::string f(fn);
    if (!g.updated || w != g.updatedW || h != g.updatedH) return fail(f + ": call tptUpdate (UpdateTest) at this size first");
    if (w > 8192 || h > 8192) return fail(f + ": frames of at most 8192 x 8192");
    if (int rc = own()) return rc;
    if (checks & kQueueKernel) {
        if (g.seedMode == SEED_ROW_SERIAL) return fail(f + ": needs per-pixel seeds (tptSetSeedMode(1)); row-serial " + things + " not supported");
        if (g.foldMode != FOLD_RECURSIVE) return fail(f + ": needs the recursive fold (tptSetFoldMode(0))");
        if (g.persist != 3 || g.hs != HS_TWO_PHASE) return fail(f + ": needs the path-queue kernel (tptSetKernelVariant(0, 3, ..))");
    }
    if ((checks & kQueueSpp) && g.spp > 2047) return fail(f + ": at most 2047 samples per pixel (the path-queue kernel)");
    if (g.numParts > 1 || g.shard.active) return fail(f + ": not with row sharding or a communicator (sharded " + things + " not supported)");
    if (g.mirror) return fail(f + ": not with a tile mirror (tptSetTileMirror)");
    return 0;
}

static int enqueuePlaneResolves(const TraceTicket& T, float* tiles, size_t tileStep, bool ownLerp, float* images, int64_t* rays,
                                float* moments = nullptr, float* momentImages = nullptr)
{
    const Context::ViewSlot& V = g.views[T.slot];
    if (T.pipelined) HIPCHK(hipStreamWaitEvent(g.stream, g.evTrace[T.slot], 0));
    if (rays) HIPCHK(hipMemcpyAsync(rays, V.rays, sizeof(unsigned long long) * (size_t)T.batch, hipMemcpyDeviceToDevice, g.stream));
    const size_t plane = (size_t)T.nPixels * 4;
    for (int j = 0; j < T.batch; ++j) {
        const TraceTicket P = T.plane(j);
        HIPCHK(tptLaunchResolve(tiles + (size_t)j * tileStep, P.colour, T.nPixels, ownLerp ? P.lerpFac : T.lerpFac,
                                images ? images + (size_t)j * plane : nullptr, g.dRays, nullptr, V.rays + j, g.stream));
        if (moments)
            HIPCHK(tptLaunchResolve(moments, T.moments + (size_t)j * (size_t)T.nPixels, T.nPixels, ownLerp ? P.lerpFac : T.lerpFac,
                                    momentImages ? momentImages + (size_t)j * plane : nullptr, g.dRays, nullptr, nullptr, g.stream));
    }
    if (T.pipelined) {
        HIPCHK(hipEventRecord(g.evResolve[T.slot], g.stream));
        g.resolveRecorded[T.slot] = true;
    }
    return 0;
}

static CameraSetup viewSetup(const float* p)
{
    CameraSetup cs = defaultCameraSetup();
    for (int i = 0; i < 3; ++i) {
        cs.lookFrom[i] = p[i];
        cs.lookAt[i] = p[3 + i];
    }
    cs.vfov = p[6];
// ... 73 lines not shown
}

static int drawClip(const char* name, int firstFrame, int nFrames, const float* times, bool cameras, const float* views, int w, int h,
                    float* deviceTile, const ClipPlanes& planes, float* deviceFrameImages, int64_t* deviceFrameRays, CameraPOD* outCameras,
                    unsigned testFlags)
{
    const std::string fn = name;
    float* const deviceMoments = planes.moments;
    if (int rc_ = flushShardDeferred()) return rc_;
    if (requireInit()) return -1;
    if (nFrames < 1) return fail(fn + ": nFrames must be at least 1");
    if (!times || (cameras && !views) || !deviceTile || !deviceMoments || w <= 0 || h <= 0)
        return fail(fn + (cameras ? ": bad arguments (times, views, deviceTile, deviceMoments, size)" : ": bad arguments (times, deviceTile, deviceMoments, size)"));
    const bool animate = (testFlags & TPT_FLAG_ANIMATE) && g.spheres.size() > 8;
    const bool flat = g.spheres.size() < TPT_GROUP_MIN_SPHERES;
    const int perLaunch = flat && (animate || (cameras && g.spheres.size() > 8)) ? kMaxBatch : 1;
    int rc = checkPathQueueDraw(fn.c_str(), "clip planes are", w, h, kQueueKernel | kQueueSpp, [&] {
        const size_t plane = (size_t)h * (size_t)w * sizeof(f4), staged = 2 * plane * (size_t)(nFrames < perLaunch ? nFrames : perLaunch);
        if (staged > (4ull << 30))
            return refuse(fn + ": " + std::to_string(staged >> 20) + " MiB of frame colour and moments per launch: over the 4096 MiB limit");
        if (g.spheres.size() > 65534) return fail(fn + ": at most 65534 spheres (the path-queue kernel)");
        const struct { const void* p; size_t bytes; } bufs[7] = {
            {deviceTile, plane}, {deviceMoments, plane}, {deviceFrameImages, plane * (size_t)nFrames}, {planes.frameAlbedo, plane * (size_t)nFrames},
            {planes.frameNormalDepth, plane * (size_t)nFrames}, {planes.frameMoments, plane * (size_t)nFrames},
            {deviceFrameRays, sizeof(int64_t) * (size_t)nFrames}};
        for (int i = 0; i < 7; ++i)
            for (int k = i + 1; k < 7; ++k) {
                const uintptr_t a = reinterpret_cast<uintptr_t>(bufs[i].p), b = reinterpret_cast<uintptr_t>(bufs[k].p);
                if (a && b && a < b + bufs[k].bytes && b < a + bufs[i].bytes) return fail(fn + ": two of the tile, moments and per-frame buffers overlap");
            }
        return 0;
    });
    if (rc) return rc;
    return enqueueAnimation(firstFrame, nFrames, times, w, h, deviceTile, deviceFrameImages, deviceFrameRays, testFlags, animate, perLaunch, &planes,
                            views, outCameras);
}

}

extern "C" {

int tptDrawDevice(float time, int frameCount, int w, int h, float* deviceTile, unsigned testFlags)
{
    (void)time;
    if (int rc_ = flushShardDeferred()) return rc_;
    if (requireInit()) return -1;
    if (!g.updated) return fail("tptDrawDevice: call tptUpdate (UpdateTest) first");
    if (!deviceTile || w <= 0 || h <= 0) return fail("tptDrawDevice: bad arguments");
    Context::DeviceCaller& D = g.devCaller;
    const unsigned long long key = g.configEpoch;
    const bool pipelined = effectiveOverlap() > 1;
    const bool stable = !g.sceneDirty && g.pendingSet < 0 && !(testFlags & TPT_FLAG_ANIMATE);
    bool prevDone = false;
    if (D.lastSlot >= 0 && g.resolveRecorded[D.lastSlot]) {
        prevDone = hipEventQuery(g.evResolve[D.lastSlot]) == hipSuccess;
        (void)hipGetLastError();
    }
    D.syncStreak = prevDone ? D.syncStreak + 1 : 0;
    const int seqStreak = D.seq.next(frameCount, w, h, testFlags, key);
    const bool lookAhead = pipelined && stable && !g.mirror && g.lookahead > 0 && D.syncStreak >= 2 && seqStreak >= 2;

    LaunchQueue& Q = g.pending;
    TraceTicket T;
    const unsigned long long* rays = nullptr;
    int rc;
    const bool hit = stable && !g.mirror && Q.frontMatches(PendingLaunch::AHEAD, frameCount, w, h, testFlags, key);
    if (!hit && !lookAhead) {
        if (stable && Q.frontMatches(PendingLaunch::STREAM, frameCount, w, h, testFlags, key)) {
            Q.serveFront(true, T, rays);
        } else {
            const bool continues = Q.empty() && seqStreak >= 2 && frameCount == g.streamNext;
            if ((rc = Q.discard())) return rc;
            g.streamNext = -1;
            int nBatch = 1;
            if (g.streamBatch && pipelined && stable && seqStreak >= 2 && pathQueueContext() && w <= 8192 && h <= 8192) {
                g.streamRun = continues ? g.streamRun + 1 : 0;
                nBatch = streamBatchFrames((long long)localRows(h) * w * g.spp, effectiveOverlap(), Context::kMaxOverlap, g.streamRun,
                                           (long long)localRows(h) * w * (long long)sizeof(f4), Context::kStreamBatchMax);
            }
            if (nBatch > 1) {
                PendingLaunch S;
                S.kind = PendingLaunch::STREAM;
                S.firstFrame = frameCount; S.w = w; S.h = h; S.flags = testFlags; S.key = key;
                S.rays = g.dRaysStream + (g.streamBatches % (unsigned long long)Context::kStreamRing) * Context::kStreamBatchMax;
                rc = enqueueTrace(frameCount, w, h, testFlags, S.rays, S.T, nBatch, 1);
                if (rc == kRefused && localRows(h) * (long long)w * g.spp >= kStreamLaunchSamples) {
                    nBatch = 1;
                } else if (rc) {
                    return rc;
                } else if (S.T.valid) {
                    g.streamBatches++;
                    g.streamNext = frameCount + nBatch;
                    if ((rc = Q.push(S))) return rc;
                    Q.serveFront(false, T, rays);
                }
            }
            if (nBatch == 1 && (rc = enqueueTrace(frameCount, w, h, testFlags, nullptr, T)))
                return rc;
        }
        rc = enqueueResolve(T, deviceTile, rays);
        if (T.valid) D.lastSlot = T.slot;
        return rc;
    }
    const int devAhead = g.lookahead + 1 < 3 ? g.lookahead + 1 : 3;
    DepthScope depthScope(1 + devAhead);
    if (hit) {
        Q.serveFront(true, T, rays);
    } else {
        if ((rc = Q.discard())) return rc;
        unsigned long long* own = g.dRaysAhead + g.frameSeq % (unsigned long long)Context::kMaxSlots;
        if ((rc = enqueueTrace(frameCount, w, h, testFlags, own, T))) return rc;
        rays = T.valid ? own : nullptr;
    }
    if (lookAhead && T.valid && (rc = traceAhead(frameCount, w, h, testFlags, key, devAhead))) return rc;
    rc = enqueueResolve(T, deviceTile, rays);
    if (T.valid) D.lastSlot = T.slot;
    return rc;
}

int tptDrawDeviceBatch(float time, int firstFrame, int nFrames, int w, int h, float* deviceTile, unsigned testFlags)
{
    (void)time;
    if (int rc_ = flushShardDeferred()) return rc_;
    if (requireInit()) return -1;
    if (!g.updated) return fail("tptDrawDeviceBatch: call tptUpdate (UpdateTest) first");
    if (!deviceTile || w <= 0 || h <= 0 || nFrames < 1) return fail("tptDrawDeviceBatch: bad arguments");
    if (nFrames > 1 && (testFlags & TPT_FLAG_ANIMATE))
        return fail("tptDrawDeviceBatch: an animated scene changes every frame (Test.cpp:304-308): one tptUpdate + tptDrawDevice per frame");
    int rc = g.pending.discard();
    if (rc) return rc;
    for (int f = 0; f < nFrames; f += kMaxBatch) {
        const int n = nFrames - f < kMaxBatch ? nFrames - f : kMaxBatch;
        TraceTicket T;
        if ((rc = enqueueTrace(firstFrame + f, w, h, testFlags, nullptr, T, n))) return rc;
        if ((rc = enqueueResolve(T, deviceTile, nullptr))) return rc;
    }
    return 0;
}

int tptDrawDeviceViews(float time, int frameCount, int w, int h, int nViews, const float* views, float* deviceTiles, int64_t* deviceViewRays,
                       unsigned testFlags)
{
    (void)time;
    if (int rc_ = flushShardDeferred()) return rc_;
    if (requireInit()) return -1;
    if (nViews < 1 || nViews > kMaxBatch) return fail("tptDrawDeviceViews: nViews must be 1.." + std::to_string(kMaxBatch));
    if (!views || !deviceTiles || w <= 0 || h <= 0) return fail("tptDrawDeviceViews: bad arguments (views, deviceTiles, size)");
    int rc = checkPathQueueDraw("tptDrawDeviceViews", "views are", w, h, kQueueKernel, [&] {
        const size_t colour = (size_t)h * (size_t)w * sizeof(f4) * (size_t)nViews;
        return colour > (4ull << 30) ? refuse("tptDrawDeviceViews: " + std::to_string(colour >> 20) + " MiB of view colour per launch: over the 4096 MiB limit, use fewer views") : 0;
    });
    if (rc) return rc;
    CameraPOD cams[kMaxBatch];
    for (int v = 0; v < nViews; ++v) cams[v] = viewCamera(viewSetup(views + 9 * v), w, h);
    if ((rc = g.pending.discard())) return rc;
    TraceTicket T;
    BatchTable table;
    table.cams = cams;
    if ((rc = enqueueTrace(frameCount, w, h, testFlags, nullptr, T, nViews, 1, &table))) return rc;
    return T.valid ? enqueuePlaneResolves(T, deviceTiles, (size_t)T.nPixels * 4, false, nullptr, deviceViewRays) : 0;
}

int tptDrawDeviceAnimation(int firstFrame, int nFrames, const float* times, int w, int h, float* deviceTile, float* deviceFrameImages,
                           int64_t* deviceFrameRays, unsigned testFlags)
{
    if (int rc_ = flushShardDeferred()) return rc_;
    if (requireInit()) return -1;
    if (nFrames < 1) return fail("tptDrawDeviceAnimation: nFrames must be at least 1");
    if (!times || !deviceTile || w <= 0 || h <= 0) return fail("tptDrawDeviceAnimation: bad arguments (times, deviceTile, size)");
    const bool animate = (testFlags & TPT_FLAG_ANIMATE) && g.spheres.size() > 8;
    const int perLaunch = pathQueueContext() && (!animate || g.spheres.size() < TPT_GROUP_MIN_SPHERES) ? kMaxBatch : 1;
    int rc = checkPathQueueDraw("tptDrawDeviceAnimation", "animation is", w, h, 0, [&] {
        const size_t colour = (size_t)h * (size_t)w * sizeof(f4) * (size_t)(nFrames < perLaunch ? nFrames : perLaunch);
        return colour > (4ull << 30) ? refuse("tptDrawDeviceAnimation: " + std::to_string(colour >> 20) + " MiB of frame colour per launch: over the 4096 MiB limit") : 0;
    });
// ... 34 lines not shown
    aov.normalDepth = reinterpret_cast<f4*>(deviceNormalDepth);
    if ((rc = enqueueTrace(frameCount, w, h, testFlags, nullptr, T, 1, 0, nullptr, &aov))) return rc;
    return enqueueResolve(T, deviceTile, nullptr);
}

int tptDrawDeviceMoments(float time, int frameCount, int w, int h, float* deviceTile, float* deviceAlbedo, float* deviceNormalDepth,
                         float* deviceMoments, unsigned testFlags)
{
    (void)time;
    if (int rc_ = flushShardDeferred()) return rc_;
    if (requireInit()) return -1;
    if (!deviceTile || !deviceMoments || w <= 0 || h <= 0)
        return fail("tptDrawDeviceMoments: bad arguments (deviceTile, deviceMoments, size)");
    int rc = checkPathQueueDraw("tptDrawDeviceMoments", "moments are", w, h, kQueueKernel | kQueueSpp, [&] {
        return overlapsAny(deviceMoments, {deviceTile, deviceAlbedo, deviceNormalDepth}, (uintptr_t)w * (uintptr_t)h * 16u)
                   ? fail("tptDrawDeviceMoments: deviceMoments overlaps the tile or a plane") : 0;
    });
    if (rc || (rc = g.pending.discard())) return rc;
    TraceTicket T;
    AovPlanes aov;
    aov.albedo = reinterpret_cast<f4*>(deviceAlbedo);
    aov.normalDepth = reinterpret_cast<f4*>(deviceNormalDepth);
    aov.moments = true;
    if ((rc = enqueueTrace(frameCount, w, h, testFlags, nullptr, T, 1, 0, nullptr, &aov))) return rc;
    if ((rc = enqueueResolve(T, deviceTile, nullptr))) return rc;
    if (!T.valid) return 0;
    HIPCHK(tptLaunchResolve(deviceMoments, g.dMoments, T.nPixels, T.lerpFac, nullptr, g.dRays, nullptr, nullptr, g.stream));
    return 0;
}

int tptDrawDeviceAdaptive(float time, int frameCount, int w, int h, float* deviceTile, float* deviceAlbedo, float* deviceNormalDepth,
                          float* deviceMoments, const int32_t* deviceSampleCounts, unsigned testFlags)
{
    (void)time;
    const std::string fn = "tptDrawDeviceAdaptive";
    if (int rc_ = flushShardDeferred()) return rc_;
    if (requireInit()) return -1;
    if (!deviceTile || !deviceMoments || !deviceSampleCounts || w <= 0 || h <= 0)
        return fail(fn + ": bad arguments (deviceTile, deviceMoments, deviceSampleCounts, size)");
    int rc = checkPathQueueDraw(fn.c_str(), "sample counts are", w, h, kQueueKernel, [&] {
        const uintptr_t plane = (uintptr_t)w * (uintptr_t)h * 16u, counts = (uintptr_t)w * (uintptr_t)h * 4u;
        if (overlapsAny(deviceMoments, {deviceTile, deviceAlbedo, deviceNormalDepth}, plane))
            return fail(fn + ": deviceMoments overlaps the tile or a plane");
        const uintptr_t c = reinterpret_cast<uintptr_t>(deviceSampleCounts);
        for (const void* out : {(const void*)deviceTile, (const void*)deviceMoments, (const void*)deviceAlbedo, (const void*)deviceNormalDepth}) {
            const uintptr_t o = reinterpret_cast<uintptr_t>(out);
            if (out && c < o + plane && o < c + counts) return fail(fn + ": deviceSampleCounts overlaps the tile, the moments or a plane");
        }
        return 0;
    });
    if (rc) return rc;
    if (!tptLaunchAdaptiveResolve) return fail(fn + ": this build has no adaptive blend kernel");
    if ((rc = g.pending.discard())) return rc;
    TraceTicket T;
    AovPlanes aov;
    aov.albedo = reinterpret_cast<f4*>(deviceAlbedo);
    aov.normalDepth = reinterpret_cast<f4*>(deviceNormalDepth);
    aov.moments = true;
    aov.sampleCounts = deviceSampleCounts;
    if ((rc = enqueueTrace(frameCount, w, h, testFlags, nullptr, T, 1, 0, nullptr, &aov))) return rc;
    if (!T.valid) return 0;
    if (T.pipelined) HIPCHK(hipStreamWaitEvent(g.stream, g.evTrace[T.slot], 0));
    HIPCHK(tptLaunchAdaptiveResolve(deviceTile, deviceMoments, T.colour, T.moments, deviceSampleCounts, T.nPixels,
                                    (testFlags & TPT_FLAG_PROGRESSIVE) != 0, g.stream));
    if (T.pipelined) {
        HIPCHK(hipEventRecord(g.evResolve[T.slot], g.stream));
        g.resolveRecorded[T.slot] = true;
    }
    return 0;
}

int tptRayCounterRead(int64_t* outTotalRays)
{
    if (int rc_ = flushShardDeferred()) return rc_;
    if (requireInit()) return -1;
    g.pending.closeStream();
    unsigned long long v = 0;
    HIPCHK(hipMemcpyAsync(&v, g.dRays, sizeof(v), hipMemcpyDeviceToHost, g.stream));
    HIPCHK(hipStreamSynchronize(g.stream));
    if (outTotalRays) *outTotalRays = (int64_t)v;
    return 0;
}

int tptSetTileMirror(float* deviceMirror, void* deviceCounterOut)
{
    g.mirror = deviceMirror;
    g.mirrorCounter = deviceMirror ? static_cast<unsigned long long*>(deviceCounterOut) : nullptr;
    return 0;
}

int tptSetRayCounter(void* deviceU64)
{
    if (int rc_ = flushShardDeferred()) return rc_;
    if (requireInit()) return -1;
    if (g.pending.discard()) return -2;
    HIPCHK(hipStreamSynchronize(g.stream));
    g.dRays = deviceU64 ? static_cast<unsigned long long*>(deviceU64) : g.dRaysOwn;
    int64_t total = 0;
    int rc = tptRayCounterRead(&total);
    if (rc) return rc;
    g.lastTotal = total;
    return 0;
}

int tptSynchronize(void)
{
    if (int rc_ = flushShardDeferred()) return rc_;
    if (requireInit()) return -1;
    g.pending.closeStream();
    if (int rc = launchTailHelpers()) return rc;
    HIPCHK(hipStreamSynchronize(g.stream));
    return 0;
}

int tptTimerBegin(void)
{
    if (requireInit()) return -1;
    HIPCHK(hipEventRecord(g.ev0, g.stream));
    return 0;
}
int tptTimerEnd(float* outMs)
{
    if (int rc_ = flushShardDeferred()) return rc_;
    if (requireInit()) return -1;
    HIPCHK(hipEventRecord(g.ev1, g.stream));
    if (int rc = launchTailHelpers()) return rc;
    HIPCHK(hipEventSynchronize(g.ev1));
    float ms = 0;
    HIPCHK(hipEventElapsedTime(&ms, g.ev0, g.ev1));
    if (outMs) *outMs = ms;
    return 0;
}

}
```

toypathtracer_amd/csrc/tpt_host_shard.cpp:

```cpp
#include "tpt_context.h"

using namespace tpt;
using namespace tpth;

namespace tpth {
int flushShardDeferred()
{
    Context::Shard& S = g.shard;
    if (!S.active || S.pendCount <= 0) return 0;
    const int first = S.pendFirst, n = S.pendCount;
    S.pendCount = 0;
    const int keep = S.exchangeEvery;
    S.exchangeEvery = 1;
    const int rc = tptDrawShardedBatch(S.pendTime, first, n, S.pendW, S.pendH, S.lastImage, S.pendFlags);
    S.exchangeEvery = keep;
    return rc;
}
}

extern "C" {
namespace {
int loadRccl()
{
    Context::Shard& S = g.shard;
// ... 131 lines not shown
    for (int k = 0; k < Context::Shard::kRing; ++k) {
        if (S.evSnap[k]) (void)hipEventDestroy(S.evSnap[k]);
        if (S.evSent[k]) (void)hipEventDestroy(S.evSent[k]);
        S.evSnap[k] = S.evSent[k] = nullptr;
    }
    if (S.commStream) (void)hipStreamDestroy(S.commStream);
    S.commStream = nullptr;
    S.nRanks = 0;
    return tptSetRowShard(0, 1, 0);
}

int tptDrawSharded(float time, int frameCount, int w, int h, float* deviceImageOnRoot, unsigned testFlags)
{
    return tptDrawShardedBatch(time, frameCount, 1, w, h, deviceImageOnRoot, testFlags);
}

int tptDrawShardedBatch(float time, int frameCount, int nFrames, int w, int h, float* deviceImageOnRoot, unsigned testFlags)
{
    if (requireInit()) return -1;
    Context::Shard& S = g.shard;
    if (!S.active) return fail("tptDrawSharded: call tptCommInit first");
    if (w <= 0 || h <= 0 || nFrames < 1 || nFrames > kMaxBatch) return fail("tptDrawSharded: bad size / batch (1..32 frames)");
    if (S.rank == 0 && !deviceImageOnRoot) return fail("tptDrawSharded: rank 0 needs the image buffer");
    if (w != S.w || h != S.h) {
        int rc = releaseShardBuffers();
        if (rc) return rc;
        HIPCHK(hipStreamSynchronize(g.stream));
        S.padRows = shardPadRows(h, S.stripeRows, S.nRanks);
        const size_t rowBytes = (size_t)w * 4 * sizeof(float);
        HIPCHK(hipMalloc(reinterpret_cast<void**>(&S.tile), rowBytes * (size_t)S.padRows));
        HIPCHK(hipMemsetAsync(S.tile, 0, rowBytes * (size_t)S.padRows, g.stream));
        for (int k = 0; k < Context::Shard::kRing; ++k) {
            HIPCHK(hipMalloc(reinterpret_cast<void**>(&S.send[k]), shardSnapshotPixels(S.padRows, w) * sizeof(f4)));
            HIPCHK(hipMemsetAsync(S.send[k], 0, shardSnapshotPixels(S.padRows, w) * sizeof(f4), g.stream));
        }
        if (S.rank == 0) {
            HIPCHK(hipMalloc(reinterpret_cast<void**>(&S.gathered), shardSnapshotPixels(S.padRows, w) * sizeof(f4) * (size_t)S.nRanks));
            HIPCHK(hipMemsetAsync(S.gathered, 0, shardSnapshotPixels(S.padRows, w) * sizeof(f4) * (size_t)S.nRanks, g.stream));
            HIPCHK(hipStreamSynchronize(g.stream));
        }
        S.w = w; S.h = h;
    }
    S.lastImage = deviceImageOnRoot;
    int every = S.exchangeEvery;
    if (every <= 0) {
        const long long samples = (long long)shardPadRows(h, S.stripeRows, S.nRanks) * w * g.spp;
        every = (S.nRanks <= 1 || (testFlags & TPT_FLAG_ANIMATE) || samples >= 2400000) ? 1 : (samples >= 1200000 ? 2 : samples >= 600000 ? 4 : 8);
    }
    if (every > kMaxBatch) every = kMaxBatch;
    if (S.pendCount > 0 && !(nFrames == 1 && every > 1 && frameCount == S.pendFirst + S.pendCount && w == S.pendW && h == S.pendH && testFlags == S.pendFlags)) {
        int rc = flushShardDeferred();
        if (rc) return rc;
    }
    if (nFrames == 1 && every > 1) {
        if (S.pendCount == 0) { S.pendFirst = frameCount; S.pendW = w; S.pendH = h; S.pendFlags = testFlags; S.pendTime = time; }
        if (++S.pendCount < every) return 0;
        frameCount = S.pendFirst; nFrames = S.pendCount; time = S.pendTime;
        S.pendCount = 0;
    }
    const int k = shardRingSlot(S.frames, Context::Shard::kRing);
    S.frames++;
    if (S.sentRecorded[k]) HIPCHK(hipStreamWaitEvent(g.stream, S.evSent[k], 0));
    const size_t tileFloats = shardCounterPixel(S.padRows, w) * 4;
    int rc = tptSetTileMirror(S.send[k], S.send[k] + tileFloats);
    if (rc) return rc;
    if ((rc = nFrames > 1 ? tptDrawDeviceBatch(time, frameCount, nFrames, w, h, S.tile, testFlags) : tptDrawDevice(time, frameCount, w, h, S.tile, testFlags))) return rc;
    return enqueueExchange(k);
}

int tptSetShardExchangeInterval(int k)
{
    if (k < 0 || k > kMaxBatch) return fail("tptSetShardExchangeInterval: 0 (automatic) or 1..32 frames");
    if (int rc = flushShardDeferred()) return rc;
    g.shard.exchangeEvery = k;
    return 0;
}

int tptShardedFinish(int64_t* outTotalRays)
{
    if (requireInit()) return -1;
    Context::Shard& S = g.shard;
    if (!S.active) return fail("tptShardedFinish: call tptCommInit first");
    if (int rc = flushShardDeferred()) return rc;
    if (int rc = launchTailHelpers()) return rc;
    HIPCHK(hipStreamSynchronize(g.stream));
    HIPCHK(hipStreamSynchronize(S.commStream));
    long long total = 0;
    if (S.frames == 0 || !S.w) {
        int64_t own = 0;
        int rc = tptRayCounterRead(&own);
        if (rc) return rc;
        if (outTotalRays) *outTotalRays = own;
        return 0;
    }
    if (S.rank == 0) {
        for (int r = 0; r < S.nRanks; ++r) {
            unsigned long long v = 0;
            const char* src = reinterpret_cast<const char*>(S.gathered) + sizeof(f4) * ((size_t)r * shardSnapshotPixels(S.padRows, S.w) + shardCounterPixel(S.padRows, S.w));
            HIPCHK(hipMemcpy(&v, src, sizeof(v), hipMemcpyDeviceToHost));
            total += (long long)v;
        }
    } else {
        const int k = shardRingSlot(S.frames - 1, Context::Shard::kRing);
        unsigned long long v = 0;
        HIPCHK(hipMemcpy(&v, reinterpret_cast<const char*>(S.send[k]) + sizeof(f4) * shardCounterPixel(S.padRows, S.w), sizeof(v), hipMemcpyDeviceToHost));
        total = (long long)v;
    }
    if (outTotalRays) *outTotalRays = total;
    return 0;
}

}
```

toypathtracer_amd/csrc/tpt_kernels.hip:

```cpp
#include "../../include/tpt_hip.h"
#include "tpt_device.h"
#include "tpt_queue_layout.h"
#include "tpt_shard.h"

namespace tpt {

__device__ __forceinline__ unsigned waveReduceAdd(unsigned v)
{
#pragma unroll
    for (int off = 32; off > 0; off >>= 1) v += __shfl_down(v, off, 64);
    return v;
}

__device__ __forceinline__ void storeColour(const KernelArgs& a, const Lane& L)
{
    f3 c = lanePixelColour(L, a.fc);
    f4 v;
    v.x = c.x; v.y = c.y; v.z = c.z; v.w = 0.0f;
    a.frameColour[L.pix] = v;
}

__global__ void __launch_bounds__(256) tptResolveKernel(float* __restrict__ tile, const f4* __restrict__ colour, int nPixels, float lerpFac,
                                                        const unsigned long long* frameRays, unsigned long long* totalRays)
{
// ... 1078 lines not shown
            if (go && memberFilter(s, o, dk1)) testSphereTie(s, sid, o, d, TPT_MIN_T, hitT, id);
        }
    }
    TPT_DEAL_T(tb1_);
    TPT_DEAL_ADD(90, tb0_, tb1_);
    const v2f ox = {o.x, o.x}, oy = {o.y, o.y}, oz = {o.z, o.z};
    const float gx = d.x * TPT_PG_K, gy = d.y * TPT_PG_K, gz = d.z * TPT_PG_K;
    const v2f dx = {gx, gx}, dy = {gy, gy}, dz = {gz, gz};
    bool parked = false;
    const bool boundsOnMatrix = TPT_MATRIX_FILTER && TPT_GROUP_MATRIX_BOUNDS && sv.gmxTiles > 0;
    const bool twoLevel = !boundsOnMatrix && boundsMode >= 0 && sv.nSuperPairs > 0;
    if (twoLevel) {
        if (boundsMode > 0)
            dealThreeStage<PATHS>(sv, ldsGpairs, TPT_GPAIR_LDS_STRIDE, go, o, d, ox, oy, oz, dx, dy, dz, list, listCount, st, p, lane, hitT, id, parked);
        else
            dealThreeStage<PATHS>(sv, sv.gpairs, (TPT_SUPER / 2) * 8, go, o, d, ox, oy, oz, dx, dy, dz, list, listCount, st, p, lane, hitT, id, parked);
    }
    MatrixRayOps mops;
    if (boundsOnMatrix) matrixRayOperands(o, d, 1, mops);
    for (int pb0 = 0; !twoLevel && pb0 < sv.nGroupPairs; pb0 += 128) {
        uint64_t cm0 = 0, cm1 = 0, cm2 = 0, cm3 = 0;
        if (boundsOnMatrix) {
            const int g0 = pb0 * 2, left = sv.nGroups - g0;
            const uint4* A = reinterpret_cast<const uint4*>(sv.gmatH) + (size_t)(g0 / 64) * (TPT_MXH_TABLE_DWORDS / 4);
            cm0 = matrixApply(A, 16, left < 64 ? left : 64, mops);
            if (left > 64) cm1 = matrixApply(A + TPT_MXH_TABLE_DWORDS / 4, 16, left - 64 < 64 ? left - 64 : 64, mops);
            if (left > 128) cm2 = matrixApply(A + 2 * (TPT_MXH_TABLE_DWORDS / 4), 16, left - 128 < 64 ? left - 128 : 64, mops);
            if (left > 192) cm3 = matrixApply(A + 3 * (TPT_MXH_TABLE_DWORDS / 4), 16, left - 192 < 64 ? left - 192 : 64, mops);
        } else {
            const int left = sv.nGroupPairs - pb0;
            cm0 = phase1Chunk(pairPtr(sv.gpairs + (size_t)pb0 * 8), left < 32 ? left : 32, ox, oy, oz, dx, dy, dz);
            if (left > 32) cm1 = phase1Chunk(pairPtr(sv.gpairs + (size_t)(pb0 + 32) * 8), left - 32 < 32 ? left - 32 : 32, ox, oy, oz, dx, dy, dz);
            if (left > 64) cm2 = phase1Chunk(pairPtr(sv.gpairs + (size_t)(pb0 + 64) * 8), left - 64 < 32 ? left - 64 : 32, ox, oy, oz, dx, dy, dz);
            if (left > 96) cm3 = phase1Chunk(pairPtr(sv.gpairs + (size_t)(pb0 + 96) * 8), left - 96 < 32 ? left - 96 : 32, ox, oy, oz, dx, dy, dz);
        }
        if (!go) cm0 = cm1 = cm2 = cm3 = 0ull;
        while (__ballot((cm0 | cm1 | cm2 | cm3) != 0ull) != 0ull) {
            const unsigned n = (unsigned)(__popcll(cm0) + __popcll(cm1) + __popcll(cm2) + __popcll(cm3));
            if (lane == 0) *listCount = 0u;
            __builtin_amdgcn_wave_barrier();
            if (n != 0u) {
                unsigned pos = atomicAdd(listCount, n);
                while (pos < (unsigned)TPT_GROUP_DEAL_CAP) {
                    const int sel = cm0 ? 0 : cm1 ? 1 : cm2 ? 2 : 3;
                    const uint64_t w = cm0 ? cm0 : cm1 ? cm1 : cm2 ? cm2 : cm3;
                    if (!w) break;
                    const int k = __builtin_clzll(w);
                    const uint64_t keep = ~(0x8000000000000000ull >> k);
                    cm0 &= sel == 0 ? keep : ~0ull;
                    cm1 &= sel == 1 ? keep : ~0ull;
                    cm2 &= sel == 2 ? keep : ~0ull;
                    cm3 &= sel == 3 ? keep : ~0ull;
                    list[pos] = ((unsigned)p << 16) | (unsigned)((pb0 + sel * 32) * 2 + k);
                    ++pos;
                }
                if (!parked) {
                    st[p] = mk4(u2f((uint32_t)id), hitT, o.x, o.y);
                    st[PATHS + p] = mk4(o.z, d.x, d.y, d.z);
                    parked = true;
                }
            }
            __builtin_amdgcn_wave_barrier();
            dealProcessList<PATHS>(sv, list, listCount, st, lane);
            __builtin_amdgcn_wave_barrier();
        }
    }
    if (parked) {
        const f4 k = st[p];
        id = (int)f2u(k.x);
        hitT = k.y;
    }
    outT = hitT;
    return id;
}
#endif

#ifndef TPT_Q_MIN_WAVES_PER_SIMD
#define TPT_Q_MIN_WAVES_PER_SIMD 4
#endif
#ifndef TPT_Q_MAX_VGPR
#define TPT_Q_MAX_VGPR 60
#endif
template <bool LDS_SCENE, bool BATCH, bool VIEWS = false, bool MOVING = false, bool AOV = false, bool MOMENTS = false, bool ADAPTIVE = false,
          bool CAMERAS = false>
__device__ __forceinline__ void traceQueueBody(const KernelArgs& a)
{
    extern __shared__ __attribute__((aligned(16))) unsigned char smem[];
    static_assert(BATCH || !VIEWS, "views are frames of a batched launch");
    static_assert((BATCH || !MOVING) && !(VIEWS && MOVING), "animation frames are frames of a batched launch of their own");
    static_assert(!AOV || !BATCH || (MOVING && MOMENTS), "first-hit planes are made by single-frame launches, or beside the moments of an animated clip's frames");
    static_assert(!MOMENTS || AOV, "moments are summed beside the first-hit sums");
    static_assert(!ADAPTIVE || (MOMENTS && !BATCH), "a count per pixel belongs to a single frame with its moments");
    static_assert(!CAMERAS || (BATCH && MOVING && AOV && MOMENTS && !VIEWS && !ADAPTIVE), "a camera per frame belongs to the frames of a clip with their planes");
    constexpr bool CAM_TABLE = VIEWS || CAMERAS;
    constexpr int kPaths = (LDS_SCENE ? TPT_Q_PATHS : TPT_Q_PATHS_GROUPED) - (CAM_TABLE ? TPT_Q_VIEW_PATHS : 0) -
                           (MOVING ? TPT_Q_ANIM_PATHS : 0);
    constexpr int kOffSt = LDS_SCENE ? TPT_Q_SPH_FIXED : 0;
    constexpr int kOffQ = kOffSt + TPT_Q_NF4 * kPaths * 16;
    constexpr int kOffCtl = kOffQ + Q_COUNT * TPT_Q_P * 2;
    constexpr int kOffDeal = kOffCtl + (((int)sizeof(QueueCtl) + 63) & ~63);
    constexpr int kDealBytes = (!LDS_SCENE && TPT_GROUP_DEAL) ? TPT_Q_WAVES * TPT_GROUP_DEAL_WAVE_BYTES : 0;
    constexpr int kOffFc = kOffDeal + kDealBytes;
    constexpr int kOffCams = kOffFc + (((int)sizeof(FrameConsts) + 15) & ~15);
    constexpr int kOffMoved = kOffCams + (CAM_TABLE ? TPT_Q_VIEW_CAM_BYTES : 0);
    constexpr int kOffScene = kOffMoved + (MOVING ? TPT_Q_ANIM_TABLE_BYTES : 0);
    f4* st = reinterpret_cast<f4*>(smem + kOffSt);
    LdsRing q = (LdsRing)(smem + kOffQ);
    QueueCtl* ctl = reinterpret_cast<QueueCtl*>(smem + kOffCtl);
    FrameConsts* ldsFc = reinterpret_cast<FrameConsts*>(smem + kOffFc);
    CameraPOD* ldsCams = reinterpret_cast<CameraPOD*>(smem + kOffCams);
    f4* ldsMoved = reinterpret_cast<f4*>(smem + kOffMoved);
    const LdsMovedPtr movedLds = (LdsMovedPtr)ldsMoved;
    const int nPad = a.scene.nPairs * 2;
    const bool sphFixed = LDS_SCENE && nPad * 16 <= TPT_Q_SPH_FIXED;
    f4* ldsSphFixed = reinterpret_cast<f4*>(smem);
    f4* ldsSph = sphFixed ? ldsSphFixed : reinterpret_cast<f4*>(smem + kOffScene);
    int off = kOffScene + ((LDS_SCENE && !sphFixed) ? nPad * 16 : 0);
    float* ldsInvR = reinterpret_cast<float*>(smem + off);
    off += LDS_SCENE ? ((nPad * 4 + 15) & ~15) : 0;
    f4* ldsLights = reinterpret_cast<f4*>(smem + off);
    off += a.scene.nLights * 32;
    f4* ldsMats = reinterpret_cast<f4*>(smem + off);
    off += LDS_SCENE ? a.scene.nSpheres * 48 : 0;
#if TPT_MATRIX_FILTER
    const bool useMatrix = LDS_SCENE && a.scene.mxR1 >= 0;
    uint32_t* ldsA = reinterpret_cast<uint32_t*>(smem + off);
#endif

    const int tid = threadIdx.x, lane = tid & 63;
    const bool helper = a.helperBase > 0;
    if (helper) {
        unsigned* seen = reinterpret_cast<unsigned*>(smem);
        if (tid == 0) {
            const unsigned was = __hip_atomic_fetch_add(&a.work[2], 1u, __ATOMIC_RELAXED, __HIP_MEMORY_SCOPE_AGENT);
            const unsigned closed = __hip_atomic_fetch_or(&a.work[3], dependentZero(was), __ATOMIC_RELAXED, __HIP_MEMORY_SCOPE_AGENT);
            const unsigned taken = __hip_atomic_load(&a.work[0], __ATOMIC_RELAXED, __HIP_MEMORY_SCOPE_AGENT);
            const long long left = (long long)a.numChunks - (long long)taken;
            const bool join = (int)(closed - a.gen) < 0 && left > 0 && left * 100 >= (long long)a.numChunks * a.helperPct;
            if (!join) __hip_atomic_fetch_sub(&a.work[2], 1u, __ATOMIC_RELAXED, __HIP_MEMORY_SCOPE_AGENT);
            *seen = join ? 1u : 0u;
        }
        __syncthreads();
        const unsigned join = *seen;
        __syncthreads();
        if (!join) return;
    }
    SceneView sv = a.scene;
    if (LDS_SCENE) {
        for (int i = tid; i < nPad; i += TPT_Q_T) {
            ldsSph[i] = a.scene.sph4[i];
            ldsInvR[i] = a.scene.invR[i];
        }
        for (int i = tid; i < a.scene.nSpheres * 3; i += TPT_Q_T) ldsMats[i] = a.scene.mats[i];
        sv.sph4 = ldsSph;
        sv.invR = ldsInvR;
        sv.mats = ldsMats;
    }
    for (int i = tid; i < a.scene.nLights * 2; i += TPT_Q_T) ldsLights[i] = a.scene.lights[i];
    sv.lights = ldsLights;
    float* ldsGpairs = reinterpret_cast<float*>(smem + ((off + 15) & ~15));
    if (!LDS_SCENE && a.ldsGroupPairs > 0)
        for (int i = tid; i < a.ldsGroupPairs * 8; i += TPT_Q_T) ldsGpairs[(i / TPT_GPAIR_FLOATS) * TPT_GPAIR_LDS_STRIDE + (i % TPT_GPAIR_FLOATS)] = a.scene.gpairs[i];
#if TPT_MATRIX_FILTER
    if (useMatrix)
        for (int i = tid; i < TPT_MXH_TABLE_DWORDS; i += TPT_Q_T) ldsA[i] = a.scene.amatH[i];
    const int mxR1 = a.scene.mxR1;
#endif
#if defined(__HIP_DEVICE_COMPILE__) && defined(TPT_STATS) && TPT_STATS >= 2
    if (tid < 4) g_hsLds[tid] = 0ull;
#if TPT_GROUP_DEAL
    if (tid < 18) g_dealLds[tid] = 0ull;
#endif
#endif
    for (int i = tid; i < (int)(sizeof(FrameConsts) / 4); i += TPT_Q_T) reinterpret_cast<uint32_t*>(ldsFc)[i] = reinterpret_cast<const uint32_t*>(&a.fc)[i];
    if (CAM_TABLE)
        for (int i = tid; i < a.batchFrames * (int)(sizeof(CameraPOD) / 4); i += TPT_Q_T)
            reinterpret_cast<uint32_t*>(ldsCams)[i] = reinterpret_cast<const uint32_t*>(a.viewCams)[i];
    if (MOVING)
        for (int i = tid; i < a.batchFrames * 2; i += TPT_Q_T) ldsMoved[i] = a.moveCentres[i];
    for (int i = tid; i < Q_COUNT * TPT_Q_P; i += TPT_Q_T) q[i] = (unsigned short)(i < kPaths ? i : 0xFFFF);
    if (tid < 8) {
        ctl->head[tid] = 0u;
        ctl->tail[tid] = tid == Q_FREE ? (unsigned)kPaths : 0u;
    }
    if (tid == 0) {
        ctl->poolTotal = 0u;
        ctl->globalExhausted = 0u;
    }
    if (BATCH && tid < 32) ctl->frameRays[tid] = 0u;
    __syncthreads();

    const FrameConsts& fc = a.fc;
    const unsigned long long laneBelow = (1ull << lane) - 1ull;
#if TPT_MATRIX_FILTER
    SceneView svM = sv;
    svM.sph4 = ldsSphFixed;
#endif
#if TPT_GROUP_DEAL
    LdsList dealList = (LdsList)(smem + kOffDeal + (tid >> 6) * TPT_GROUP_DEAL_WAVE_BYTES);
    unsigned* dealCount = reinterpret_cast<unsigned*>(smem + kOffDeal + (tid >> 6) * TPT_GROUP_DEAL_WAVE_BYTES + TPT_GROUP_DEAL_ENTRIES * 4);
    const bool groupDeal = !MOVING && !LDS_SCENE && sv.nGroups > 0 && sv.nGroups <= 65536;
#endif
    f4* colSum = st + 2 * kPaths;
    int chunkNext = 0, chunkEnd = 0;
    int chunkFrame = 0;
    bool noMoreChunks = false;
    unsigned myRays = 0;
#if defined(TPT_STATS)
    const unsigned long long qT0 = wall_clock64();
    unsigned qSteps = 0, qBatches = 0, qIdle = 0;
    unsigned long long qSec[5] = {0, 0, 0, 0, 0};
#endif

#if defined(TPT_STATS)
#define TPT_TSTAMP(v)                      \
    __builtin_amdgcn_sched_barrier(0);     \
    __builtin_amdgcn_s_waitcnt(0);         \
    const unsigned long long v = __builtin_amdgcn_s_memtime(); \
    __builtin_amdgcn_sched_barrier(0)
#if TPT_STATS < 2
#define TPT_TADD(slot, a, b) do { if (lane == 0) atomicAdd(&g_tptStats[slot], (b) - (a)); } while (0)
#else
#define TPT_TADD(slot, a, b) do { qSec[(slot) == 64 + 24 ? 4 : ((slot) & 3)] += (b) - (a); } while (0)
#endif
#else
#define TPT_TSTAMP(v) do { } while (0)
#define TPT_TADD(slot, a, b) do { } while (0)
#endif
    for (;;) {
        TPT_TSTAMP(tsTop);
        unsigned myAvail = 0, myHead = 0, myTail = 0;
        if (lane < Q_COUNT) {
            myTail = __hip_atomic_load(&ctl->tail[lane], __ATOMIC_RELAXED, __HIP_MEMORY_SCOPE_WORKGROUP);
            myHead = __hip_atomic_load(&ctl->head[lane], __ATOMIC_RELAXED, __HIP_MEMORY_SCOPE_WORKGROUP);
            myAvail = myTail - myHead;
        }
        unsigned avail[Q_COUNT];
#pragma unroll
        for (int c = 0; c < Q_COUNT; ++c) avail[c] = (unsigned)__builtin_amdgcn_readlane((int)myAvail, c);
        const bool canStart = (chunkEnd > chunkNext) || !noMoreChunks;
        int pick = -1;
        unsigned best = 0;
        if (canStart && avail[Q_FREE] >= 64u) pick = Q_FREE;
        if (pick < 0) {
#pragma unroll
            for (int c = 1; c < Q_COUNT; ++c)
                if (avail[c] >= 64u && avail[c] > best) {
                    best = avail[c];
                    pick = c;
                }
        }
        if (pick < 0) {
#pragma unroll
            for (int c = 0; c < Q_COUNT; ++c)
                if ((c != Q_FREE || canStart) && avail[c] > best) {
                    best = avail[c];
                    pick = c;
                }
        }
        if (pick < 0) {
            const unsigned pool = __hip_atomic_load(&ctl->poolTotal, __ATOMIC_RELAXED, __HIP_MEMORY_SCOPE_WORKGROUP);
            const unsigned exhausted = __hip_atomic_load(&ctl->globalExhausted, __ATOMIC_RELAXED, __HIP_MEMORY_SCOPE_WORKGROUP);
            if (avail[Q_FREE] == (unsigned)kPaths && pool == 0u && exhausted != 0u && !canStart) break;
            if (exhausted != 0u && pool == 0u) noMoreChunks = true;
            TPT_STAT(ST_REFILL);
#if defined(TPT_STATS)
            qIdle++;
#endif
            __builtin_amdgcn_s_sleep(4);
            TPT_TSTAMP(tsIdle);
            TPT_TADD(64 + 24, tsTop, tsIdle);
            continue;
        }
        int p = 0;
        const int n = qPop(q + pick * TPT_Q_P, &ctl->head[pick], &ctl->tail[pick], lane, p, (unsigned)__builtin_amdgcn_readlane((int)myHead, pick),
                           (unsigned)__builtin_amdgcn_readlane((int)myTail, pick));
        if (n == 0) continue;
#if defined(TPT_STATS)
        qBatches++;
#endif
        __builtin_amdgcn_fence(__ATOMIC_ACQUIRE, "workgroup");
        TPT_TSTAMP(tsPop);
        TPT_TADD(64 + pick * 4 + 0, tsTop, tsPop);
        const bool mine = lane < n;
#if defined(TPT_STATS)
        if (mine) { TPT_STAT(16 + pick); }
#endif

        f3 ro = mk3(0, 0, 0), rd = mk3(0, 0, 0);
        uint32_t rng = 0;
        int sample = 0, depth = 0, recId = -1;
        bool doMatE = true;
        bool ray = false;
        bool toFree = false;
        bool toEnd = false;
        QStack stack;
        stack.l0 = (LdsF4Ptr)(st + 3 * kPaths + p);
        stack.spill = a.stackBuf + ((size_t)(blockIdx.x + (unsigned)a.helperBase) * TPT_Q_PATHS + p);
        stack.stride = a.stackStride;
        constexpr int kAovSums = MOMENTS ? 3 : 2;
        auto aovSum = [&]() { return a.aovSums + kAovSums * ((size_t)(blockIdx.x + (unsigned)a.helperBase) * TPT_Q_PATHS + p); };
        QLambert lam;
        lam.sdir = lam.nl = lam.albedo = lam.lightE = mk3(0, 0, 0);
        lam.cosAMax = 0.0f;
        int movedAt = 0;
        if (pick != Q_FREE && mine) {
            if (MOVING) movedAt = 2 * (int)(f2u(colSum[p].w) >> 26);
            const f4 r0 = st[0 * kPaths + p], r1 = st[1 * kPaths + p];
            ro = mk3(r0.x, r0.y, r0.z);
            rng = f2u(r0.w);
            rd = mk3(r1.x, r1.y, r1.z);
            const uint32_t w = f2u(r1.w);
            sample = (int)(w & 0x7ffu);
            depth = (int)((w >> 11) & 15u);
            doMatE = ((w >> 15) & 1u) != 0;
            recId = (w >> 16) == 0xffffu ? -1 : (int)(w >> 16);
        }

        if (pick == Q_FREE) {
            bool need = mine, got = false;
            int px = 0, py = 0, laneFrame = 0;
            [[maybe_unused]] uint32_t laneCount = 0u;
            for (;;) {
                const unsigned long long needMask = __ballot(need);
                if (needMask == 0ull) break;
                if (chunkNext >= chunkEnd) {
                    if (noMoreChunks) break;
                    int c = 0;
                    if (lane == 0) {
                        atomicAdd(&ctl->poolTotal, 64u);
                        c = (int)atomicAdd(&a.work[0], 1u);
                    }
                    c = __builtin_amdgcn_readfirstlane(c);
                    if (c >= a.numChunks) {
                        if (lane == 0) {
                            atomicSub(&ctl->poolTotal, 64u);
                            __hip_atomic_store(&ctl->globalExhausted, 1u, __ATOMIC_RELAXED, __HIP_MEMORY_SCOPE_WORKGROUP);
                        }
                        noMoreChunks = true;
                        break;
                    }
                    chunkFrame = 0;
                    if (BATCH) {
                        chunkFrame = c / a.chunksPerFrame;
                        c -= chunkFrame * a.chunksPerFrame;
                    }
                    chunkNext = c * a.chunkSize;
                    chunkEnd = chunkNext + a.chunkSize;
                    if (chunkEnd > a.numItems) chunkEnd = a.numItems;
                    if (lane == 0 && chunkEnd - chunkNext != 64) atomicSub(&ctl->poolTotal, (unsigned)(64 - (chunkEnd - chunkNext)));
                }
                const int rank = __popcll(needMask & laneBelow);
                const int want = __popcll(needMask);
                const int availPx = chunkEnd - chunkNext;
                const int take = want < availPx ? want : availPx;
                if (need && rank < take) {
                    int x, ly;
                    bool take1 = mapItem(a, chunkNext + rank, x, ly);
                    if (ADAPTIVE && take1) {
                        const int c = a.sampleCounts[(size_t)ly * fc.width + x];
                        laneCount = (uint32_t)(c < 0 ? 0 : (c > 2047 ? 2047 : c));
                        take1 = laneCount != 0u;
                    }
                    if (take1) {
                        px = x;
                        py = localRowToGlobal(a, ly);
                        laneFrame = chunkFrame;
                        got = true;
                        need = false;
                    }
                }
                chunkNext += take;
                if (lane == 0) atomicSub(&ctl->poolTotal, (unsigned)take);
            }
            if (got) {
                rng = pixelSeed(fc.seedMode, px, py, fc.frame + ((BATCH && !VIEWS) ? laneFrame : 0));
                const uint32_t where = BATCH ? ((uint32_t)px | ((uint32_t)py << 13) | ((uint32_t)laneFrame << 26))
                                             : ((uint32_t)px | ((uint32_t)py << 16));
                colSum[p] = mk4(0.0f, 0.0f, 0.0f, u2f(where));
                if (AOV) aovSum()[0] = aovSum()[1] = mk4(0.0f, 0.0f, 0.0f, 0.0f);
                if (MOMENTS) aovSum()[2] = mk4(0.0f, 0.0f, ADAPTIVE ? u2f(laneCount) : 0.0f, 0.0f);
                if (MOVING) movedAt = 2 * laneFrame;
                if (CAM_TABLE)
                    qCameraView(ldsCams[laneFrame], *ldsFc, px, py, rng, ro, rd);
                else
                    qCamera(*ldsFc, px, py, rng, ro, rd);
                ray = true;
            } else if (mine) {
                toFree = true;
            }
        } else if (pick == Q_INT) {
            ray = mine;
        } else if (pick == Q_END) {
            if (mine) {
                const f3 c = qFold(sv, qEndTerm(sv, fc, rd, recId), depth, stack);
                const f4 c3 = colSum[p];
                const f3 col = mk3(c3.x, c3.y, c3.z) + c;
                int px, py, plane = 0;
                if (BATCH) {
                    px = (int)(f2u(c3.w) & 0x1fffu);
                    py = (int)((f2u(c3.w) >> 13) & 0x1fffu);
                    plane = (int)(f2u(c3.w) >> 26) * a.framePlane;
                } else {
                    px = (int)(f2u(c3.w) & 0xffffu);
                    py = (int)(f2u(c3.w) >> 16);
                }
                [[maybe_unused]] f4 mom;
                if (MOMENTS) {
                    const float l = (0.2126f * c.x + 0.7152f * c.y) + 0.0722f * c.z;
                    const f4 m = aovSum()[2];
                    mom = mk4(m.x + l, m.y + l * l, ADAPTIVE ? m.z : 0.0f, 0.0f);
                }
                sample++;
                if (sample < (ADAPTIVE ? (int)f2u(mom.z) : fc.spp)) {
                    colSum[p] = mk4(col.x, col.y, col.z, c3.w);
                    if (MOMENTS) aovSum()[2] = mom;
                    if (CAM_TABLE)
// ... 110 lines not shown
                    else
                        id = hitSpheres<LDS_SCENE ? HS_TWO_PHASE : HS_TWO_PHASE_GROUPS>(sv, ro, d2, TPT_MIN_T, TPT_MAX_T, t);
                    if (BATCH) iterRays++; else myRays++;
                    if (shadow) {
                        if (id == lightId) qLightShade(l1, d2, lam);
                    } else {
                        hitId = id;
                        hitT = t;
                    }
                }
            }
            if (ray) {
                if (hitId < 0 || depth >= TPT_MAX_DEPTH)
                    cls = Q_END;
                else {
                    const int type = (int)f2u(sv.mats[hitId * 3].w);
                    cls = type == MAT_LAMBERT ? Q_LAMBERT : type == MAT_METAL ? Q_METAL : type == MAT_DIELECTRIC ? Q_DIEL : Q_END;
                }
                if (hitId >= 0) ro = ro + rd * hitT;
                if (AOV && depth == 0 && hitId >= 0) {
                    const f3 nrm = qNormal<MOVING>(sv, hitId, ro, movedLds + movedAt);
                    const f4 m0 = sv.mats[hitId * 3];
                    f4* sum = aovSum();
                    const f4 s0 = sum[0], s1 = sum[1];
                    sum[0] = mk4(s0.x + m0.x, s0.y + m0.y, s0.z + m0.z, s0.w + 1.0f);
                    sum[1] = mk4(s1.x + nrm.x, s1.y + nrm.y, s1.z + nrm.z, s1.w + hitT);
                }
                recId = hitId;
            }
        } else if (ray) {
            cls = Q_INT;
        }
        if (toEnd) cls = Q_END;
        if (ray || toEnd) {
            const uint32_t w = ((uint32_t)sample & 0x7ffu) | (((uint32_t)depth & 15u) << 11) | ((uint32_t)doMatE << 15) | (((uint32_t)recId & 0xffffu) << 16);
            st[0 * kPaths + p] = mk4(ro.x, ro.y, ro.z, u2f(rng));
            st[1 * kPaths + p] = mk4(rd.x, rd.y, rd.z, u2f(w));
        }
        if (toFree) cls = Q_FREE;
        if (BATCH && iterRays != 0u) {
            const unsigned fr = f2u(colSum[p].w) >> 26;
            const unsigned old = atomicAdd(&ctl->frameRays[fr], iterRays);
            if (__builtin_expect(old < 0x80000000u && old + iterRays >= 0x80000000u, 0)) {
                atomicSub(&ctl->frameRays[fr], 0x80000000u);
                atomicAdd(a.rayCounter + (size_t)fr * a.rayCounterStride, 0x80000000ull);
            }
        }
        TPT_TSTAMP(tsInt);
        TPT_TADD(64 + pick * 4 + 2, tsClass, tsInt);
        __builtin_amdgcn_fence(__ATOMIC_RELEASE, "workgroup");
        qPushByClass(q, ctl, mine ? cls : -1, p, lane);
        TPT_TSTAMP(tsPush);
        TPT_TADD(64 + pick * 4 + 3, tsInt, tsPush);
    }

    const unsigned waveRays = waveReduceAdd(myRays);
    if (BATCH) {
        __syncthreads();
        if (tid < a.batchFrames && ctl->frameRays[tid] != 0u) atomicAdd(a.rayCounter + (size_t)tid * a.rayCounterStride, (unsigned long long)ctl->frameRays[tid]);
    }
    if (helper) {
        if (lane == 0 && !BATCH) atomicAdd(a.rayCounter, (unsigned long long)waveRays);
        __syncthreads();
        if (tid == 0) {
            __builtin_amdgcn_fence(__ATOMIC_RELEASE, "agent");
            __hip_atomic_fetch_sub(&a.work[2], 1u, __ATOMIC_SEQ_CST, __HIP_MEMORY_SCOPE_AGENT);
        }
        return;
    }
    if (lane == 0) {
        if (!BATCH) atomicAdd(a.rayCounter, (unsigned long long)waveRays);
        unsigned done = atomicAdd(&a.work[1], 1u) + 1u;
        if (done == a.totalWaves) {
            if (a.gen != 0u) {
                const unsigned prev = __hip_atomic_exchange(&a.work[3], a.gen, __ATOMIC_RELAXED, __HIP_MEMORY_SCOPE_AGENT);
                unsigned busy = __hip_atomic_fetch_or(&a.work[2], dependentZero(prev), __ATOMIC_RELAXED, __HIP_MEMORY_SCOPE_AGENT);
                while (busy != 0u) {
                    __builtin_amdgcn_s_sleep(127);
                    busy = __hip_atomic_fetch_or(&a.work[2], 0u, __ATOMIC_RELAXED, __HIP_MEMORY_SCOPE_AGENT);
                }
            }
            a.work[0] = 0u;
            a.work[1] = 0u;
        }
    }
#if defined(__HIP_DEVICE_COMPILE__) && defined(TPT_STATS) && TPT_STATS >= 2
    __syncthreads();
    if (tid < 4) TPT_COUNT(120 + tid, g_hsLds[tid]);
#if TPT_GROUP_DEAL
    if (tid < 15) TPT_COUNT(90 + tid, g_dealLds[tid]);
    if (tid >= 15 && tid < 18) TPT_COUNT(124 + tid - 15, g_dealLds[tid]);
#endif
#endif
#if defined(TPT_STATS)
    if (lane == 0) {
        const unsigned long long qT1 = wall_clock64();
        TPT_COUNT(106, qSteps);
        TPT_COUNT(107, waveRays);
        TPT_COUNT(108, qT1 - qT0);
        TPT_COUNT(109, 1);
        TPT_COUNT(110, qBatches);
        TPT_COUNT(105, qIdle);
#if TPT_STATS >= 2
        for (int k = 0; k < 5; ++k) TPT_COUNT(112 + k, qSec[k]);
#endif
    }
#endif
}

#ifndef TPT_Q_MAX_VGPR_GROUPED
#define TPT_Q_MAX_VGPR_GROUPED 64
#endif
template <bool LDS_SCENE, bool BATCH = false>
__global__ void __launch_bounds__(TPT_Q_T, TPT_Q_MIN_WAVES_PER_SIMD) __attribute__((amdgpu_num_vgpr(TPT_Q_MAX_VGPR)))
tptTraceQueueKernel(const KernelArgs a)
{
    traceQueueBody<LDS_SCENE, BATCH>(a);
}
template <>
__global__ void __launch_bounds__(TPT_Q_T, TPT_Q_MIN_WAVES_PER_SIMD) __attribute__((amdgpu_num_vgpr(TPT_Q_MAX_VGPR_GROUPED)))
tptTraceQueueKernel<false, false>(const KernelArgs a)
{
    traceQueueBody<false, false>(a);
}
template <>
__global__ void __launch_bounds__(TPT_Q_T, TPT_Q_MIN_WAVES_PER_SIMD) __attribute__((amdgpu_num_vgpr(TPT_Q_MAX_VGPR_GROUPED)))
tptTraceQueueKernel<false, true>(const KernelArgs a)
{
    traceQueueBody<false, true>(a);
}
enum { QF_BATCH = 1, QF_VIEWS = 2, QF_MOVING = 4, QF_AOV = 8, QF_MOMENTS = 16, QF_ADAPTIVE = 32, QF_CAMERAS = 64 };
#define TPT_QUEUE_VARIANT_KERNEL(NAME, F)                                                                                                    \
    template <bool LDS_SCENE>                                                                                                                \
    __global__ void __launch_bounds__(TPT_Q_T, TPT_Q_MIN_WAVES_PER_SIMD) __attribute__((amdgpu_num_vgpr(TPT_Q_MAX_VGPR)))                    \
    NAME(const KernelArgs a)                                                                                                                 \
    {                                                                                                                                        \
        traceQueueBody<LDS_SCENE, ((F) & QF_BATCH) != 0, ((F) & QF_VIEWS) != 0, ((F) & QF_MOVING) != 0, ((F) & QF_AOV) != 0, ((F) & QF_MOMENTS) != 0, \
                       ((F) & QF_ADAPTIVE) != 0, ((F) & QF_CAMERAS) != 0>(a);                                                                \
    }                                                                                                                                        \
    template <>                                                                                                                              \
    __global__ void __launch_bounds__(TPT_Q_T, TPT_Q_MIN_WAVES_PER_SIMD) __attribute__((amdgpu_num_vgpr(TPT_Q_MAX_VGPR_GROUPED)))            \
    NAME<false>(const KernelArgs a)                                                                                                          \
    {                                                                                                                                        \
        traceQueueBody<false, ((F) & QF_BATCH) != 0, ((F) & QF_VIEWS) != 0, ((F) & QF_MOVING) != 0, ((F) & QF_AOV) != 0, ((F) & QF_MOMENTS) != 0, \
                       ((F) & QF_ADAPTIVE) != 0, ((F) & QF_CAMERAS) != 0>(a);                                                                \
    }
TPT_QUEUE_VARIANT_KERNEL(tptTraceViewsKernel, QF_BATCH | QF_VIEWS)
TPT_QUEUE_VARIANT_KERNEL(tptTraceAnimationKernel, QF_BATCH | QF_MOVING)
TPT_QUEUE_VARIANT_KERNEL(tptTraceAovKernel, QF_AOV)
TPT_QUEUE_VARIANT_KERNEL(tptTraceMomentsKernel, QF_AOV | QF_MOMENTS)
TPT_QUEUE_VARIANT_KERNEL(tptTraceClipKernel, QF_BATCH | QF_MOVING | QF_AOV | QF_MOMENTS)
TPT_QUEUE_VARIANT_KERNEL(tptTraceAdaptiveKernel, QF_AOV | QF_MOMENTS | QF_ADAPTIVE)
TPT_QUEUE_VARIANT_KERNEL(tptCameraClipKernel, QF_BATCH | QF_MOVING | QF_AOV | QF_MOMENTS | QF_CAMERAS)
#undef TPT_QUEUE_VARIANT_KERNEL

#if defined(TPT_TEST_HOOKS)
__global__ void tptMathTestKernel(int op, const float* __restrict__ a, const float* __restrict__ b, float* __restrict__ out, int n)
{
    int i = blockIdx.x * blockDim.x + threadIdx.x;
    if (i >= n) return;
    float x = a[i], y = b ? b[i] : 0.0f, r = 0.0f;
    switch (op) {
    case 0: r = tsqrt(x); break;
    case 1: r = x / y; break;
    case 2: r = tsinf(x); break;
    case 3: r = tcosf(x); break;
    case 4: r = tpow5f(x); break;
    case 5: {
        uint32_t s = f2u(x) | 1u;
        for (int k = 0; k < 16; ++k) r = rnd01(s);
        break;
    }
    case 6: r = schlick(x, y); break;
    case 7: r = normalize(mk3(x, y, 1.0f)).x; break;
    case 8: { float sn, cs; tsincosf(x, sn, cs); r = sn; break; }
    case 9: { float sn, cs; tsincosf(x, sn, cs); r = cs; break; }
    case 10: r = tdivSafeNum(x, y); break;
    case 11: r = tdivByPi(x); break;
    }
    out[i] = r;
}

__global__ void __launch_bounds__(256) tptMathExhaustiveKernel(int op, uint32_t lo, uint32_t hi, unsigned long long* nBad, uint32_t* firstBad)
{
    const uint64_t n = (uint64_t)hi - lo + 1;
    for (uint64_t i = (uint64_t)blockIdx.x * blockDim.x + threadIdx.x; i < n; i += (uint64_t)gridDim.x * blockDim.x) {
        const uint32_t b = lo + (uint32_t)i;
        const float x = u2f(b);
        const float want = op == 0 ? __builtin_sqrtf(x) : 1.0f / __builtin_sqrtf(x);
        const float got = op == 0 ? tsqrt(x) : trsqrt2(x);
        if (f2u(got) != f2u(want) && !(got != got && want != want)) {
            const unsigned long long k = atomicAdd(nBad, 1ull);
            if (k < 8) firstBad[k] = b;
        }
    }
}

template <int HS>
__global__ void tptHitTestKernel(const KernelArgs a, const float* __restrict__ rays, int* __restrict__ outId,
                                 float* __restrict__ outT, int n)
{
    int i = blockIdx.x * blockDim.x + threadIdx.x;
    if (i >= n) return;
    f3 o = mk3(rays[i * 6], rays[i * 6 + 1], rays[i * 6 + 2]), d = mk3(rays[i * 6 + 3], rays[i * 6 + 4], rays[i * 6 + 5]);
    float t;
    int id = hitSpheres<HS>(a.scene, o, d, TPT_MIN_T, TPT_MAX_T, t);
    outId[i] = id;
    outT[i] = t;
}

__global__ void __launch_bounds__(64) tptMatrixFilterTestKernel(const KernelArgs a, const float* __restrict__ rays, unsigned long long* __restrict__ outMask,
                                                                int* __restrict__ outId, float* __restrict__ outT, int n)
{
    __shared__ __attribute__((aligned(16))) uint32_t ldsA[TPT_MXH_TABLE_DWORDS];
    for (int i = threadIdx.x; i < TPT_MXH_TABLE_DWORDS; i += 64) ldsA[i] = a.scene.amatH[i];
    __syncthreads();
    const int i = blockIdx.x * 64 + threadIdx.x;
    f3 o = mk3(rays[i * 6], rays[i * 6 + 1], rays[i * 6 + 2]), d = mk3(rays[i * 6 + 3], rays[i * 6 + 4], rays[i * 6 + 5]);
    const uint64_t cand = phase1MatrixH(ldsA, a.scene.mxR1, a.scene.nSpheres, o, d);
    if (outMask) outMask[i] = cand;
    if (outId) {
        float t;
        outId[i] = hitSpheresCandidates(a.scene, cand, o, d, TPT_MIN_T, TPT_MAX_T, t);
        outT[i] = t;
    }
}

__global__ void __launch_bounds__(64) tptGroupFilterTestKernel(const KernelArgs a, const float* __restrict__ rays, int n, unsigned long long* __restrict__ out)
{
    const SceneView& sv = a.scene;
    const int i = blockIdx.x * 64 + threadIdx.x;
    const bool real = i < n;
    f3 o = mk3(0.0f, 1.0e4f, 0.0f), d = mk3(0.0f, 1.0f, 0.0f);
    if (real) {
        o = mk3(rays[i * 6], rays[i * 6 + 1], rays[i * 6 + 2]);
        d = mk3(rays[i * 6 + 3], rays[i * 6 + 4], rays[i * 6 + 5]);
// ... 88 lines not shown
    (void)out64;
    return -1;
#endif
}
int tptResetStats()
{
#if defined(TPT_STATS)
    unsigned long long z[128] = {0};
    z[25] = ~0ull;
    return hipMemcpyToSymbol(HIP_SYMBOL(g_tptStats), z, sizeof(z)) == hipSuccess ? 0 : -2;
#else
    return -1;
#endif
}
#endif

template <int HS, int FOLD, bool LDS_SCENE>
static hipError_t launchOne(const KernelArgs& a, int blocks, size_t lds, hipStream_t stream)
{
    auto k = tptTraceKernel<HS, FOLD, LDS_SCENE>;
    if (lds > 48 * 1024) {
        hipError_t e = hipFuncSetAttribute(reinterpret_cast<const void*>(k), hipFuncAttributeMaxDynamicSharedMemorySize, (int)lds);
        if (e != hipSuccess) return e;
    }
    hipLaunchKernelGGL(k, dim3(blocks), dim3(TPT_BLOCK), lds, stream, a);
    return hipGetLastError();
}

template <int HS, int FOLD, bool LDS_SCENE>
static int occupancyOne(size_t lds)
{
    int nb = 0;
    auto k = tptTraceKernel<HS, FOLD, LDS_SCENE>;
    if (hipOccupancyMaxActiveBlocksPerMultiprocessor(&nb, reinterpret_cast<const void*>(k), TPT_BLOCK, lds) != hipSuccess) nb = 1;
    return nb < 1 ? 1 : nb;
}

#define TPT_DISPATCH(FN, ...)                                                                  \
    do {                                                                                       \
        const int key = (hs ? 4 : 0) | (fold ? 2 : 0) | (ldsScene ? 1 : 0);                    \
        switch (key) {                                                                         \
        case 0: return FN<HS_TWO_PHASE, FOLD_RECURSIVE, false>(__VA_ARGS__);                   \
        case 1: return FN<HS_TWO_PHASE, FOLD_RECURSIVE, true>(__VA_ARGS__);                    \
        case 2: return FN<HS_TWO_PHASE, FOLD_FORWARD, false>(__VA_ARGS__);                     \
        case 3: return FN<HS_TWO_PHASE, FOLD_FORWARD, true>(__VA_ARGS__);                      \
        case 4: return FN<HS_SIMPLE, FOLD_RECURSIVE, false>(__VA_ARGS__);                      \
        case 5: return FN<HS_SIMPLE, FOLD_RECURSIVE, true>(__VA_ARGS__);                       \
        case 6: return FN<HS_SIMPLE, FOLD_FORWARD, false>(__VA_ARGS__);                        \
        default: return FN<HS_SIMPLE, FOLD_FORWARD, true>(__VA_ARGS__);                        \
        }                                                                                      \
    } while (0)

hipError_t tptLaunchTrace(const KernelArgs& a, int hs, int fold, bool ldsScene, int blocks, size_t lds, hipStream_t stream)
{
    TPT_DISPATCH(launchOne, a, blocks, lds, stream);
}
int tptTraceOccupancy(int hs, int fold, bool ldsScene, size_t lds)
{
    TPT_DISPATCH(occupancyOne, lds);
}

static hipError_t launchQueueKernel(void (*k)(KernelArgs), const KernelArgs& a, int blocks, size_t lds, hipStream_t stream)
{
    hipError_t e = hipFuncSetAttribute(reinterpret_cast<const void*>(k), hipFuncAttributeMaxDynamicSharedMemorySize, (int)lds);
    if (e != hipSuccess) return e;
    hipLaunchKernelGGL(k, dim3(blocks), dim3(TPT_Q_T), lds, stream, a);
    return hipGetLastError();
}
hipError_t tptLaunchTraceQueue(const KernelArgs& a, bool ldsScene, int blocks, size_t lds, hipStream_t stream)
{
    static void (*const kernel[QV_INVALID][2])(KernelArgs) = {
         {tptTraceQueueKernel<false, false>, tptTraceQueueKernel<true, false>},
         {tptTraceQueueKernel<false, true>, tptTraceQueueKernel<true, true>},
         {tptTraceViewsKernel<false>, tptTraceViewsKernel<true>},
         {tptTraceAnimationKernel<false>, tptTraceAnimationKernel<true>},
         {tptTraceAovKernel<false>, tptTraceAovKernel<true>},
         {tptTraceMomentsKernel<false>, tptTraceMomentsKernel<true>},
         {tptTraceClipKernel<false>, tptTraceClipKernel<true>},
         {tptTraceAdaptiveKernel<false>, tptTraceAdaptiveKernel<true>},
         {tptCameraClipKernel<false>, tptCameraClipKernel<true>},
    };
    const QueueVariant variant = tptQueueVariant(a);
    if (variant == QV_INVALID) return hipErrorInvalidValue;
    return launchQueueKernel(kernel[variant][ldsScene ? 1 : 0], a, blocks, lds, stream);
}
#if defined(TPT_TEST_HOOKS)
hipError_t tptSetDealCapacitiesForTest(int ca, int cb, int cs)
{
    unsigned v[3] = {TPT_DEAL_CA, TPT_DEAL_CB, TPT_DEAL_CS};
    if (ca || cb || cs) {
        if (ca < 64 || ca > TPT_DEAL_CA || cb < 64 || cb > TPT_DEAL_CB || cs < 64 || cs > TPT_DEAL_CS) return hipErrorInvalidValue;
        v[0] = (unsigned)ca; v[1] = (unsigned)cb; v[2] = (unsigned)cs;
    }
    return hipMemcpyToSymbol(HIP_SYMBOL(g_dealCaps), v, sizeof(v));
}
#endif
int tptQueueMatrixFilter() { return TPT_MATRIX_FILTER; }
int tptQueueGroupMatrixBounds() { return TPT_MATRIX_FILTER && TPT_GROUP_MATRIX_BOUNDS; }

hipError_t tptLaunchDisplay(const float* tile, unsigned char* rgba, int width, int height, hipStream_t stream)
{
    hipLaunchKernelGGL(tptDisplayKernel, dim3((width * height + 255) / 256), dim3(256), 0, stream, reinterpret_cast<const f4*>(tile),
                       reinterpret_cast<uint32_t*>(rgba), width, height);
    return hipGetLastError();
}

template <typename Launch>
static hipError_t atrousIterations(const float* colour, float* out, float* scratch, int iterations, Launch launch)
{
    const f4* src = reinterpret_cast<const f4*>(colour);
    for (int i = 0; i < iterations; ++i) {
        f4* dst = reinterpret_cast<f4*>(((iterations - 1 - i) & 1) ? scratch : out);
        launch(i, src, dst);
        hipError_t e = hipGetLastError();
        if (e != hipSuccess) return e;
        src = dst;
    }
    return hipSuccess;
}

template <bool GUIDE>
static void launchDenoiseIteration(bool first, bool last, dim3 grid, hipStream_t stream, const f4* src, const f4* albedo, const f4* nd,
                                   f4* dst, int width, int height, int step, float ic, float in, float id, int demod)
{
    auto k = first ? (last ? tptDenoiseKernel<true, true, GUIDE> : tptDenoiseKernel<true, false, GUIDE>)
                   : (last ? tptDenoiseKernel<false, true, GUIDE> : tptDenoiseKernel<false, false, GUIDE>);
    hipLaunchKernelGGL(k, grid, dim3(64, 4), 0, stream, src, albedo, nd, dst, width, height, step, ic, in, id, demod);
}
hipError_t tptLaunchDenoise(const float* colour, const float* albedo, const float* normalDepth, float* out, float* scratch, int width,
                            int height, int iterations, float ic, float in, float id, bool demodulate, hipStream_t stream)
{
    const dim3 grid((unsigned)(width + 63) / 64, (unsigned)(height + 3) / 4);
    const f4* a = reinterpret_cast<const f4*>(albedo);
    const f4* nd = reinterpret_cast<const f4*>(normalDepth);
    return atrousIterations(colour, out, scratch, iterations, [&](int i, const f4* src, f4* dst) {
        const float scale = (float)(1u << (2 * i));
        (nd ? launchDenoiseIteration<true> : launchDenoiseIteration<false>)(i == 0, i == iterations - 1, grid, stream, src, a, nd, dst, width,
                                                                           height, 1 << i, ic * scale, in, id, demodulate ? 1 : 0);
    });
}

template <bool GUIDE>
static void launchDenoiseVarianceIteration(bool first, bool last, dim3 grid, hipStream_t stream, const f4* src, const f4* colour,
                                           const f4* albedo, const f4* nd, const f4* moments, f4* dst, int width, int height, int step,
                                           float samples, float sl2, float in, float id, int demod)
{
    auto k = first ? (last ? tptVarianceAtrousKernel<true, true, GUIDE> : tptVarianceAtrousKernel<true, false, GUIDE>)
                   : (last ? tptVarianceAtrousKernel<false, true, GUIDE> : tptVarianceAtrousKernel<false, false, GUIDE>);
    hipLaunchKernelGGL(k, grid, dim3(64, 4), 0, stream, src, colour, albedo, nd, moments, dst, width, height, step, samples, sl2, in, id,
                       demod);
}
hipError_t tptLaunchDenoiseVariance(const float* colour, const float* albedo, const float* normalDepth, const float* moments, float* out,
                                    float* scratch, int width, int height, int iterations, float samples, float sl2, float in, float id,
                                    bool demodulate, hipStream_t stream)
{
    const dim3 grid((unsigned)(width + 63) / 64, (unsigned)(height + 3) / 4);
    const f4* c = reinterpret_cast<const f4*>(colour);
    const f4* a = reinterpret_cast<const f4*>(albedo);
    const f4* nd = reinterpret_cast<const f4*>(normalDepth);
    const f4* m = reinterpret_cast<const f4*>(moments);
    return atrousIterations(colour, out, scratch, iterations, [&](int i, const f4* src, f4* dst) {
        (nd ? launchDenoiseVarianceIteration<true> : launchDenoiseVarianceIteration<false>)(i == 0, i == iterations - 1, grid, stream, src, c, a,
                                                                                           nd, m, dst, width, height, 1 << i, samples, sl2,
                                                                                           in, id, demodulate ? 1 : 0);
    });
}
// ... 112 lines not shown
```

toypathtracer_amd/csrc/tpt_queue_layout.h:

```cpp
#pragma once
#include "tpt_device.h"
#include "tpt_shard.h"

#ifndef TPT_Q_WAVES
#define TPT_Q_WAVES 8
#endif
#define TPT_Q_T (64 * TPT_Q_WAVES)
#ifndef TPT_Q_P
#define TPT_Q_P 1024
#endif
#ifndef TPT_MATRIX_FILTER
#define TPT_MATRIX_FILTER 1
#endif
#ifndef TPT_GROUP_DEAL
#define TPT_GROUP_DEAL 1
#endif
#ifndef TPT_GROUP_MATRIX_BOUNDS
#if defined(TPT_TEST_HOOKS)
#define TPT_GROUP_MATRIX_BOUNDS 1
#else
#define TPT_GROUP_MATRIX_BOUNDS 0
#endif
#endif
#ifndef TPT_GROUP_DEAL_EXACT
#define TPT_GROUP_DEAL_EXACT 1
#endif
#ifndef TPT_DEAL_HALF_LINE
#define TPT_DEAL_HALF_LINE 1
#endif
#ifndef TPT_MEMBER_UNROLL
#define TPT_MEMBER_UNROLL 8
#endif
#ifndef TPT_GROUP_DEAL_CAP
#define TPT_GROUP_DEAL_CAP 448
#endif
#ifndef TPT_DEAL_CA
#define TPT_DEAL_CA (TPT_SUPER == 8 ? 256 : 192)
#endif
#ifndef TPT_DEAL_CB
#define TPT_DEAL_CB (TPT_SUPER == 8 ? 256 : 320)
#endif
#ifndef TPT_DEAL_CS
#define TPT_DEAL_CS 128
#endif
#define TPT_GROUP_DEAL_ENTRIES (TPT_DEAL_CA + TPT_DEAL_CB + TPT_DEAL_CS)
static_assert(TPT_GROUP_DEAL_ENTRIES >= TPT_GROUP_DEAL_CAP, "the flat variants' pair list lives in the same area");
#define TPT_GROUP_DEAL_WAVE_BYTES (TPT_GROUP_DEAL_ENTRIES * 4 + 16)
#define TPT_Q_SPH_FIXED 1024
#ifndef TPT_Q_PATHS
#define TPT_Q_PATHS (TPT_MATRIX_FILTER ? 952 : TPT_Q_P)
#endif
#define TPT_Q_VIEWS_MAX 32
#define TPT_Q_VIEW_CAM_BYTES (TPT_Q_VIEWS_MAX * 88)
#define TPT_Q_VIEW_PATHS ((TPT_Q_VIEW_CAM_BYTES + TPT_Q_NF4 * 16 - 1) / (TPT_Q_NF4 * 16))
#define TPT_Q_ANIM_TABLE_BYTES (TPT_Q_VIEWS_MAX * 2 * 16)
#define TPT_Q_ANIM_PATHS ((TPT_Q_ANIM_TABLE_BYTES + TPT_Q_NF4 * 16 - 1) / (TPT_Q_NF4 * 16))
#ifndef TPT_Q_PATHS_GROUPED
#define TPT_Q_PATHS_GROUPED 608
#endif
#define TPT_GPAIR_FLOATS ((TPT_SUPER / 2) * 8)
#define TPT_GPAIR_LDS_STRIDE (TPT_GPAIR_FLOATS + 4)
#define TPT_Q_GROUP_LDS_BYTES 9808
#ifndef TPT_Q_FUSE_MIN
#define TPT_Q_FUSE_MIN 48
#endif
#define TPT_Q_NF4 4

namespace tpt {

enum { Q_FREE = 0, Q_INT = 1, Q_END = 2, Q_DIEL = 3, Q_METAL = 4, Q_LAMBERT = 5, Q_COUNT = 6 };
struct QueueCtl {
    unsigned head[8];
    unsigned tail[8];
    unsigned poolTotal;
    unsigned globalExhausted;
    unsigned frameRays[32];
};
static_assert(sizeof(QueueCtl::frameRays) / 4 == TPT_Q_VIEWS_MAX, "one ray count per frame of a batch");
static_assert(sizeof(tptLerpTable::v) / sizeof(float) == TPT_Q_VIEWS_MAX, "one lerp factor per frame of a batch");
static_assert(TPT_Q_VIEWS_MAX <= 64, "the path record holds 6 bits of frame index");

constexpr size_t kQueueLdsFixedPart = (size_t)TPT_Q_NF4 * TPT_Q_PATHS * 16 + (size_t)Q_COUNT * TPT_Q_P * 2 + ((sizeof(tpt::QueueCtl) + 63) & ~(size_t)63) +
                                      ((sizeof(tpt::FrameConsts) + 15) & ~(size_t)15);
constexpr size_t kDefaultSceneLds = TPT_Q_SPH_FIXED + ((46 * 4 + 15) & ~15) + 46 * 48 + 2 * 32 + (TPT_MATRIX_FILTER ? TPT_MXH_TABLE_DWORDS * 4 + 64 : 0);
static_assert(2 * (kQueueLdsFixedPart + kDefaultSceneLds + 256) <= 160 * 1024, "the default scene no longer fits two path-queue workgroups per CU: shrink TPT_Q_PATHS");
static_assert(TPT_Q_VIEW_CAM_BYTES <= TPT_Q_NF4 * TPT_Q_VIEW_PATHS * 16, "the views' cameras take no more LDS than the path records they replace");
static_assert(sizeof(tpt::CameraPOD) == 88 && sizeof(tpt::CameraPOD) % 4 == 0, "cameras are staged in LDS as 22 words");
static_assert(TPT_Q_ANIM_TABLE_BYTES == TPT_Q_NF4 * TPT_Q_ANIM_PATHS * 16, "the moving centres take exactly the LDS of the path records they replace");

TPT_HD bool mapItem(const KernelArgs& a, int idx, int& x, int& ly)
{
    if (a.fc.seedMode == SEED_ROW_SERIAL) {
        x = 0;
        ly = idx;
        return ly < a.nLocalRows;
    }
    int tile = idx >> 6, within = idx & 63;
    const int tilesX = uniformHere(a.tilesX);
    int tx = tile % tilesX, ty = tile / tilesX;
    x = tx * 8 + (within & 7);
    ly = ty * 8 + (within >> 3);
    return x < a.fc.width && ly < a.nLocalRows;
}
TPT_HD int localRowToGlobal(const KernelArgs& a, int ly) { return shardKernelLocalToGlobal(ly, uniformHere(a.stripeRows), uniformHere(a.stripeStride), a.stripeOffset); }
TPT_HD int globalRowToLocal(const KernelArgs& a, int gy) { return shardKernelGlobalToLocal(gy, uniformHere(a.stripeRows), uniformHere(a.stripeStride), a.stripeOffset); }

}

enum QueueVariant { QV_FRAME, QV_BATCH, QV_VIEWS, QV_ANIMATION, QV_AOV, QV_MOMENTS, QV_CLIP, QV_ADAPTIVE, QV_CAMERA_CLIP, QV_INVALID };
inline QueueVariant tptQueueVariant(const tpt::KernelArgs& a)
{
    if (a.sampleCounts) {
        if (a.batchFrames != 1 || a.viewCams || a.moveCentres || !a.aovSums || !a.momentsOut) return QV_INVALID;
        return QV_ADAPTIVE;
    }
    if (a.viewCams && a.moveCentres) {
        if (a.batchFrames < 1 || a.batchFrames > TPT_Q_VIEWS_MAX || a.scene.nGroups > 0 || !a.aovSums || !a.momentsOut) return QV_INVALID;
        return QV_CAMERA_CLIP;
    }
    if (a.viewCams) {
        if (a.batchFrames < 1 || a.batchFrames > TPT_Q_VIEWS_MAX) return QV_INVALID;
        return QV_VIEWS;
    }
    if (a.aovSums && a.moveCentres) {
        if (a.batchFrames < 1 || a.batchFrames > TPT_Q_VIEWS_MAX || a.scene.nGroups > 0 || !a.momentsOut) return QV_INVALID;
        return QV_CLIP;
    }
    if (a.aovSums) {
        if (a.batchFrames != 1 || a.viewCams || a.moveCentres) return QV_INVALID;
        return a.momentsOut ? QV_MOMENTS : QV_AOV;
    }
    if (a.moveCentres) {
        if (a.batchFrames < 1 || a.batchFrames > TPT_Q_VIEWS_MAX || a.scene.nGroups > 0) return QV_INVALID;
        return QV_ANIMATION;
    }
    return a.batchFrames > 1 ? QV_BATCH : QV_FRAME;
}

inline size_t tptLdsBytes(const tpt::KernelArgs& a, int fold, bool ldsScene)
{
    const int nPad = a.scene.nPairs * 2;
    size_t bytes = 0;
    if (ldsScene) bytes += (size_t)nPad * 16 + (((size_t)nPad * 4 + 15) & ~(size_t)15);
    bytes += (size_t)a.scene.nLights * 32;
    if (ldsScene) bytes += (size_t)a.scene.nSpheres * 48;
    if (fold == tpt::FOLD_RECURSIVE) bytes += (size_t)a.ldsStackLevels * TPT_BLOCK * 16;
    return bytes;
}
inline size_t tptQueueLdsBytes(const tpt::KernelArgs& a, bool ldsScene)
{
    using namespace tpt;
    const int nPad = a.scene.nPairs * 2;
    const QueueVariant variant = tptQueueVariant(a);
    const bool views = variant == QV_VIEWS || variant == QV_CAMERA_CLIP;
    const bool moving = variant == QV_ANIMATION || variant == QV_CLIP || variant == QV_CAMERA_CLIP;
    size_t bytes = 0;
    if (ldsScene) bytes += TPT_Q_SPH_FIXED + ((size_t)nPad * 16 <= TPT_Q_SPH_FIXED ? 0 : (size_t)nPad * 16) + (((size_t)nPad * 4 + 15) & ~(size_t)15) + (size_t)a.scene.nSpheres * 48;
    bytes += (size_t)a.scene.nLights * 32;
    bytes += (size_t)TPT_Q_NF4 * (ldsScene ? TPT_Q_PATHS : TPT_Q_PATHS_GROUPED) * 16 + (size_t)Q_COUNT * TPT_Q_P * 2 + ((sizeof(QueueCtl) + 63) & ~(size_t)63) + ((sizeof(FrameConsts) + 15) & ~(size_t)15);
// ... 18 lines not shown
```

Baseline: 45110.

## Let host cut speculative stream batch launches short via pinned frame limit

Adds a pinned host word per stream-ring slot that the batched trace kernel polls when fetching chunks. When the host abandons a speculative multi-frame STREAM launch (discard, close, or a frame mismatch), it writes how many frames are still needed, so the kernel stops handing out chunks for frames nobody will use. This is meant to save GPU time spent tracing discarded lookahead frames. In exchange, block 0 makes system-scope loads on every chunk fetch, a new kernel variant is compiled, and the host may wait on a slot's event before reusing its cut word.

Result: slower. 18190 (-59.7%).

```diff
diff --git a/include/tpt_hip.h b/include/tpt_hip.h
--- a/include/tpt_hip.h
+++ b/include/tpt_hip.h
@@ -81,6 +81,7 @@
                                float* deviceTiles, int64_t* deviceViewRays, unsigned testFlags);
 TPT_API int tptSetFrameOverlap(int frames);
 TPT_API int tptSetStreamBatching(int enable);
+TPT_API int tptGetStreamCutInfo(int64_t* launchesCut, int64_t* framesCut);
 TPT_API int tptDisplayRGBA8(const float* deviceTile, int screenWidth, int screenHeight, unsigned char* deviceRGBA);
 TPT_API int tptRayCounterRead(int64_t* outTotalRays);
 TPT_API int tptSetRayCounter(void* deviceU64);
diff --git a/include/tpt_test_hooks.h b/include/tpt_test_hooks.h
--- a/include/tpt_test_hooks.h
+++ b/include/tpt_test_hooks.h
@@ -12,6 +12,8 @@
 TPT_API int tptTestSetDealCapacities(int superGroupEntries, int groupEntries, int survivorEntries);
 TPT_API int tptDebugStats(unsigned long long* out128, int reset);
 TPT_API int tptDebugChunkOrder(unsigned* outCost, unsigned* outOrder, int capacity);
+TPT_API int tptTestPresetStreamCut(int frames);
+TPT_API int tptTestReadStreamFrameRays(int64_t* out8);
 #ifdef __cplusplus
 }
 #endif
diff --git a/toypathtracer_amd/api.py b/toypathtracer_amd/api.py
--- a/toypathtracer_amd/api.py
+++ b/toypathtracer_amd/api.py
@@ -27,9 +27,9 @@
     "tptSetSamplesPerPixel", "tptSetConfig", "tptSetSeedMode", "tptSetFoldMode", "tptSetScene", "tptSetCamera", "tptSetStream",
     "tptSetRowShard", "tptLocalRowCount", "tptLocalRowToGlobal", "tptDrawDevice", "tptRayCounterRead", "tptSetRayCounter", "tptSetFrameOverlap", "tptDisplayRGBA8", "tptKernelTimingBegin", "tptKernelTimingEnd",
     "tptSynchronize", "tptTimerBegin", "tptTimerEnd", "tptSetKernelVariant",
-    "tptDrawDeviceBatch", "tptDrawDeviceViews", "tptDrawDeviceAnimation", "tptDrawDeviceAov", "tptDenoiseDevice", "tptDrawDeviceMoments", "tptDrawDeviceAnimationMoments", "tptDrawDeviceCameraClip", "tptDenoiseDeviceVariance", "tptTemporalAccumulateDevice", "tptDrawDeviceAdaptive", "tptAdaptiveSamplesDevice", "tptDrawShardedBatch", "tptGetLookaheadHits", "tptCommGetUniqueId", "tptCommInit", "tptCommInitLoopback", "tptCommInfo", "tptCommDestroy", "tptDrawSharded", "tptSetShardExchangeInterval", "tptShardedFinish", "tptGetLaunchInfo", "tptGetPipelineInfo", "tptGetSceneInfo", "tptSetHostBufferMode", "tptSetHostLookahead", "tptSetStreamBatching", "tptSetTileMirror", "tptGetLastError", "tptSetErrorHandler", "tptGetDeviceName",
+    "tptDrawDeviceBatch", "tptDrawDeviceViews", "tptDrawDeviceAnimation", "tptDrawDeviceAov", "tptDenoiseDevice", "tptDrawDeviceMoments", "tptDrawDeviceAnimationMoments", "tptDrawDeviceCameraClip", "tptDenoiseDeviceVariance", "tptTemporalAccumulateDevice", "tptDrawDeviceAdaptive", "tptAdaptiveSamplesDevice", "tptDrawShardedBatch", "tptGetLookaheadHits", "tptCommGetUniqueId", "tptCommInit", "tptCommInitLoopback", "tptCommInfo", "tptCommDestroy", "tptDrawSharded", "tptSetShardExchangeInterval", "tptShardedFinish", "tptGetLaunchInfo", "tptGetPipelineInfo", "tptGetSceneInfo", "tptSetHostBufferMode", "tptSetHostLookahead", "tptSetStreamBatching", "tptGetStreamCutInfo", "tptSetTileMirror", "tptGetLastError", "tptSetErrorHandler", "tptGetDeviceName",
 ]
-HOOK_SYMBOLS = ["tptTestMath", "tptTestMathExhaustive", "tptTestHitSpheres", "tptTestMatrixFilter", "tptTestGroupFilter", "tptTestSetDealCapacities", "tptDebugStats", "tptDebugChunkOrder"]
+HOOK_SYMBOLS = ["tptTestMath", "tptTestMathExhaustive", "tptTestHitSpheres", "tptTestMatrixFilter", "tptTestGroupFilter", "tptTestSetDealCapacities", "tptDebugStats", "tptDebugChunkOrder", "tptTestPresetStreamCut", "tptTestReadStreamFrameRays"]
 CXX_ABI_SYMBOLS = [
     "_Z14InitializeTestv", "_Z12ShutdownTestv", "_Z10UpdateTestfiiij", "_Z8DrawTestfiiiPfRij",
     "_Z14GetObjectCountRiS_S_S_", "_Z12GetSceneDescPvS_S_S_Pi",
@@ -61,11 +61,11 @@
         "tptSetRayCounter": [p], "tptSetTileMirror": [p, p], "tptSetFrameOverlap": [i], "tptDisplayRGBA8": [p, i, i, p], "tptKernelTimingBegin": [i],
         "tptKernelTimingEnd": [C.POINTER(f), C.POINTER(i)],
         "tptSynchronize": [], "tptTimerBegin": [], "tptTimerEnd": [C.POINTER(f)], "tptSetKernelVariant": [i, i, i],
-        "tptGetLaunchInfo": [C.POINTER(i)] * 4, "tptGetPipelineInfo": [C.POINTER(i)] * 4, "tptGetSceneInfo": [C.POINTER(i)] * 3, "tptCommGetUniqueId": [p], "tptCommInit": [p, i, i, i], "tptCommInitLoopback": [i, i], "tptCommInfo": [C.POINTER(i)] * 3, "tptCommDestroy": [], "tptDrawSharded": [f, i, i, i, p, u], "tptSetShardExchangeInterval": [i], "tptDrawShardedBatch": [f, i, i, i, i, p, u], "tptDrawDeviceBatch": [f, i, i, i, i, p, u], "tptDrawDeviceViews": [f, i, i, i, i, p, p, p, u], "tptDrawDeviceAnimation": [i, i, p, i, i, p, p, p, u], "tptDrawDeviceAov": [f, i, i, i, p, p, p, u], "tptDenoiseDevice": [i, i, p, p, p, p, i, f, f, f, u], "tptDrawDeviceMoments": [f, i, i, i, p, p, p, p, u], "tptDrawDeviceAnimationMoments": [i, i, p, i, i] + [p] * 7 + [u], "tptDrawDeviceCameraClip": [i, i, p, p, i, i] + [p] * 8 + [u], "tptDenoiseDeviceVariance": [i, i, p, p, p, p, f, p, i, f, f, f, u], "tptTemporalAccumulateDevice": [i, i] + [p] * 14 + [f] * 4, "tptDrawDeviceAdaptive": [f, i, i, i, p, p, p, p, p, u], "tptAdaptiveSamplesDevice": [i, i, p, f, i, i, p, p, p], "tptShardedFinish": [C.POINTER(C.c_int64)], "tptSetHostBufferMode": [i], "tptGetLookaheadHits": [C.POINTER(C.c_longlong)], "tptSetHostLookahead": [i], "tptSetStreamBatching": [i],
+        "tptGetLaunchInfo": [C.POINTER(i)] * 4, "tptGetPipelineInfo": [C.POINTER(i)] * 4, "tptGetSceneInfo": [C.POINTER(i)] * 3, "tptCommGetUniqueId": [p], "tptCommInit": [p, i, i, i], "tptCommInitLoopback": [i, i], "tptCommInfo": [C.POINTER(i)] * 3, "tptCommDestroy": [], "tptDrawSharded": [f, i, i, i, p, u], "tptSetShardExchangeInterval": [i], "tptDrawShardedBatch": [f, i, i, i, i, p, u], "tptDrawDeviceBatch": [f, i, i, i, i, p, u], "tptDrawDeviceViews": [f, i, i, i, i, p, p, p, u], "tptDrawDeviceAnimation": [i, i, p, i, i, p, p, p, u], "tptDrawDeviceAov": [f, i, i, i, p, p, p, u], "tptDenoiseDevice": [i, i, p, p, p, p, i, f, f, f, u], "tptDrawDeviceMoments": [f, i, i, i, p, p, p, p, u], "tptDrawDeviceAnimationMoments": [i, i, p, i, i] + [p] * 7 + [u], "tptDrawDeviceCameraClip": [i, i, p, p, i, i] + [p] * 8 + [u], "tptDenoiseDeviceVariance": [i, i, p, p, p, p, f, p, i, f, f, f, u], "tptTemporalAccumulateDevice": [i, i] + [p] * 14 + [f] * 4, "tptDrawDeviceAdaptive": [f, i, i, i, p, p, p, p, p, u], "tptAdaptiveSamplesDevice": [i, i, p, f, i, i, p, p, p], "tptShardedFinish": [C.POINTER(C.c_int64)], "tptSetHostBufferMode": [i], "tptGetLookaheadHits": [C.POINTER(C.c_longlong)], "tptSetHostLookahead": [i], "tptSetStreamBatching": [i], "tptGetStreamCutInfo": [C.POINTER(C.c_int64)] * 2,
     }
     if hooks:
         sigs.update({"tptDebugStats": [p, i], "tptDebugChunkOrder": [p, p, i], "tptTestMath": [i, p, p, p, i], "tptTestMathExhaustive": [i, u, u, p, p],
-                     "tptTestHitSpheres": [i, p, p, p, i], "tptTestMatrixFilter": [p, p, p, p, i], "tptTestGroupFilter": [p, i, p, p, p], "tptTestSetDealCapacities": [i, i, i]})
+                     "tptTestHitSpheres": [i, p, p, p, i], "tptTestMatrixFilter": [p, p, p, p, i], "tptTestGroupFilter": [p, i, p, p, p], "tptTestSetDealCapacities": [i, i, i], "tptTestPresetStreamCut": [i], "tptTestReadStreamFrameRays": [p]})
     for name, args in sigs.items():
         fn = getattr(lib, name)
         fn.argtypes = args
@@ -614,6 +614,12 @@
     _chk(load_library().tptSetStreamBatching(1 if enable else 0), "tptSetStreamBatching")
 
 
+def stream_cut_info():
+    v = [C.c_int64(), C.c_int64()]
+    _chk(load_library().tptGetStreamCutInfo(C.byref(v[0]), C.byref(v[1])), "tptGetStreamCutInfo")
+    return v[0].value, v[1].value
+
+
 def lookahead_hits():
     v = C.c_longlong()
     _chk(load_library().tptGetLookaheadHits(C.byref(v)), "tptGetLookaheadHits")
@@ -690,6 +696,16 @@
     return (masks, ids, ts) if hits else masks
 
 
+def test_preset_stream_cut(frames):
+    _chk(_hook("tptTestPresetStreamCut")(frames), "tptTestPresetStreamCut")
+
+
+def test_read_stream_frame_rays():
+    out = np.zeros(8, np.int64)
+    _chk(_hook("tptTestReadStreamFrameRays")(out.ctypes.data), "tptTestReadStreamFrameRays")
+    return out
+
+
 def test_set_deal_capacities(super_group_entries=0, group_entries=0, survivor_entries=0):
     _chk(_hook("tptTestSetDealCapacities")(super_group_entries, group_entries, survivor_entries), "tptTestSetDealCapacities")
 
diff --git a/toypathtracer_amd/csrc/tpt_context.h b/toypathtracer_amd/csrc/tpt_context.h
--- a/toypathtracer_amd/csrc/tpt_context.h
+++ b/toypathtracer_amd/csrc/tpt_context.h
@@ -64,6 +64,8 @@
     unsigned flags = 0;
     unsigned long long key = 0;
     unsigned long long* rays = nullptr;
+    unsigned* cut = nullptr;
+    int limit = 0;
 };
 struct LaunchQueue {
     static const int kCap = 4;
@@ -76,6 +78,7 @@
     int push(const PendingLaunch& L);
     int discard();
     void closeStream();
+    void cutStreams();
 };
 
 struct Context {
@@ -176,6 +179,11 @@
     unsigned long long streamBatches = 0;
     int streamRun = 0, streamNext = -1;
     int streamBatch = 1;
+    unsigned* hStreamCut = nullptr;
+    int streamCutSlot[kStreamRing];
+    long long streamLaunchesCut = 0, streamFramesCut = 0;
+    int streamCutPreset = -1;
+    unsigned long long* lastStreamRays = nullptr;
     struct DeviceCaller {
         int lastSlot = -1, syncStreak = 0;
         Streak seq;
@@ -328,7 +336,7 @@
     const int32_t* sampleCounts = nullptr;
 };
 int enqueueTrace(int frameCount, int w, int h, unsigned testFlags, unsigned long long* frameRays, TraceTicket& T, int batch = 1, int rayStride = 0,
-                 const BatchTable* table = nullptr, const AovPlanes* aov = nullptr);
+                 const BatchTable* table = nullptr, const AovPlanes* aov = nullptr, const unsigned* frameCut = nullptr);
 int enqueueResolve(const TraceTicket& T, float* deviceTile, const unsigned long long* frameRays);
 int syncAllStreams();
 int launchTailHelpers();
diff --git a/toypathtracer_amd/csrc/tpt_device.h b/toypathtracer_amd/csrc/tpt_device.h
--- a/toypathtracer_amd/csrc/tpt_device.h
+++ b/toypathtracer_amd/csrc/tpt_device.h
@@ -42,6 +42,7 @@
     f4* momentsOut = nullptr;
     int aovPlane = 0;
     const int32_t* sampleCounts = nullptr;
+    const unsigned* frameCut = nullptr;
 };
 
 }
diff --git a/toypathtracer_amd/csrc/tpt_host.cpp b/toypathtracer_amd/csrc/tpt_host.cpp
--- a/toypathtracer_amd/csrc/tpt_host.cpp
+++ b/toypathtracer_amd/csrc/tpt_host.cpp
@@ -304,6 +304,14 @@
     HIPCHK(hipMemsetAsync(g.dRaysAhead, 0, pendingRays, g.stream));
     g.dRaysBatch = g.dRaysAhead + Context::kMaxSlots;
     g.dRaysStream = g.dRaysBatch + 2 * kMaxBatch;
+    HIPCHK(hipHostMalloc(reinterpret_cast<void**>(&g.hStreamCut), sizeof(unsigned) * Context::kStreamRing, hipHostMallocDefault));
+    for (int k = 0; k < Context::kStreamRing; ++k) {
+        g.hStreamCut[k] = 0u;
+        g.streamCutSlot[k] = -1;
+    }
+    g.streamLaunchesCut = g.streamFramesCut = 0;
+    g.streamCutPreset = -1;
+    g.lastStreamRays = nullptr;
     g.pending.n = 0;
     if (const char* esb = getenv("TPT_STREAM_BATCH")) g.streamBatch = atoi(esb) != 0;
     HIPCHK(hipMalloc(reinterpret_cast<void**>(&g.dRaysOwn), 64));
@@ -401,6 +409,9 @@
     g.tileSrc = nullptr; g.tileW = g.tileH = 0;
     g.pending.n = 0;
     (void)hipFree(g.dRaysAhead); g.dRaysAhead = g.dRaysBatch = g.dRaysStream = nullptr;
+    g.lastStreamRays = nullptr;
+    if (g.hStreamCut) (void)hipHostFree(g.hStreamCut);
+    g.hStreamCut = nullptr;
     g.orderStream = nullptr; g.oldestPending = 0; g.frameSeq = 0;
     g.streamDepth = 1; g.prevInFlight = -1;
     g.hostCaller = Context::HostCaller(); g.devCaller = Context::DeviceCaller();
diff --git a/toypathtracer_amd/csrc/tpt_host_draw.cpp b/toypathtracer_amd/csrc/tpt_host_draw.cpp
--- a/toypathtracer_amd/csrc/tpt_host_draw.cpp
+++ b/toypathtracer_amd/csrc/tpt_host_draw.cpp
@@ -17,7 +17,8 @@
     if (wasOpen && F.kind != PendingLaunch::STREAM) g.aheadHits++;
     T = F.T.plane(F.next);
     rays = F.rays + F.next;
-    if (++F.next < F.T.batch) return;
+    if (++F.next < (F.kind == PendingLaunch::STREAM ? F.limit : F.T.batch)) return;
+    if (F.next < F.T.batch) cutStreams();
     for (int k = 0; k + 1 < n; ++k) e[k] = e[k + 1];
     --n;
 }
@@ -31,6 +32,7 @@
 
 int LaunchQueue::discard()
 {
+    cutStreams();
     if (n > 0 && !holds(PendingLaunch::STREAM))
         for (int k = 0; k < Context::kMaxOverlap; ++k) HIPCHK(hipStreamSynchronize(g.traceStream[k]));
     n = 0;
@@ -39,8 +41,21 @@
 
 void LaunchQueue::closeStream()
 {
+    cutStreams();
     if (holds(PendingLaunch::STREAM)) n = 0;
     g.streamNext = -1;
+}
+
+void LaunchQueue::cutStreams()
+{
+    for (int k = 0; k < n; ++k) {
+        PendingLaunch& L = e[k];
+        if (L.kind != PendingLaunch::STREAM || !L.cut || L.next >= L.T.batch) continue;
+        __atomic_store_n(L.cut, (unsigned)L.next, __ATOMIC_RELAXED);
+        g.streamLaunchesCut++;
+        g.streamFramesCut += L.T.batch - L.next;
+        L.cut = nullptr;
+    }
 }
 
 int traceAhead(int frameCount, int w, int h, unsigned testFlags, unsigned long long key, int want)
diff --git a/toypathtracer_amd/csrc/tpt_host_hooks.cpp b/toypathtracer_amd/csrc/tpt_host_hooks.cpp
--- a/toypathtracer_amd/csrc/tpt_host_hooks.cpp
+++ b/toypathtracer_amd/csrc/tpt_host_hooks.cpp
@@ -175,5 +175,25 @@
     return 0;
 }
 
+int tptTestPresetStreamCut(int frames)
+{
+    if (requireInit()) return -1;
+    if (frames < 1) return fail("tptTestPresetStreamCut: at least one frame (the call that makes the launch is served from it)");
+    g.streamCutPreset = frames;
+    return 0;
+}
+
+int tptTestReadStreamFrameRays(int64_t* out8)
+{
+    if (requireInit()) return -1;
+    if (!out8) return fail("tptTestReadStreamFrameRays: bad arguments");
+    if (!g.lastStreamRays) return fail("tptTestReadStreamFrameRays: no STREAM launch yet");
+    if (int rc = tptSynchronize()) return rc;
+    for (int k = 0; k < Context::kMaxOverlap; ++k) HIPCHK(hipStreamSynchronize(g.traceStream[k]));
+    static_assert(sizeof(int64_t) == sizeof(unsigned long long), "the counters are read as they lie");
+    HIPCHK(hipMemcpy(out8, g.lastStreamRays, sizeof(unsigned long long) * Context::kStreamBatchMax, hipMemcpyDeviceToHost));
+    return 0;
+}
+
 #endif
 }
diff --git a/toypathtracer_amd/csrc/tpt_host_pipeline.cpp b/toypathtracer_amd/csrc/tpt_host_pipeline.cpp
--- a/toypathtracer_amd/csrc/tpt_host_pipeline.cpp
+++ b/toypathtracer_amd/csrc/tpt_host_pipeline.cpp
@@ -372,8 +372,20 @@
     return 0;
 }
 
+static int armStreamCut(unsigned k, int frames)
+{
+    const int slot = g.streamCutSlot[k];
+    if (slot >= 0 && hipEventQuery(g.evTrace[slot]) != hipSuccess) {
+        (void)hipGetLastError();
+        HIPCHK(hipEventSynchronize(g.evTrace[slot]));
+    }
+    g.streamCutSlot[k] = -1;
+    __atomic_store_n(&g.hStreamCut[k], (unsigned)frames, __ATOMIC_RELAXED);
+    return 0;
+}
+
 int enqueueTrace(int frameCount, int w, int h, unsigned testFlags, unsigned long long* frameRays, TraceTicket& T, int batch, int rayStride,
-                 const BatchTable* table, const AovPlanes* aov)
+                 const BatchTable* table, const AovPlanes* aov, const unsigned* frameCut)
 {
     const CameraPOD* viewCams = table ? table->cams : nullptr;
     const f4* centres = table ? table->centres : nullptr;
@@ -456,6 +468,7 @@
     }
     if (frameRays) a.rayCounter = frameRays;
     a.rayCounterStride = rayStride;
+    a.frameCut = P.queued && batch > 1 ? frameCut : nullptr;
     if ((rc = prepareChunkOrder(P))) return rc;
     g.lastBlocksPerCU = P.occ;
     g.lastLds = (int)P.lds;
@@ -524,6 +537,7 @@
         g.ktUsed++;
     }
     if (pipelined) HIPCHK(hipEventRecord(g.evTrace[slot], ts));
+    if (a.frameCut && pipelined) g.streamCutSlot[a.frameCut - g.hStreamCut] = slot;
     if (helpable) {
         Context::HelperRec& R = g.hrec[slot];
         R.a = a; R.ldsScene = P.ldsScene; R.blocks = P.blocks; R.maxBlocks = maxGridBlocks(P); R.lds = P.lds;
@@ -763,15 +777,21 @@
                 PendingLaunch S;
                 S.kind = PendingLaunch::STREAM;
                 S.firstFrame = frameCount; S.w = w; S.h = h; S.flags = testFlags; S.key = key;
-                S.rays = g.dRaysStream + (g.streamBatches % (unsigned long long)Context::kStreamRing) * Context::kStreamBatchMax;
-                rc = enqueueTrace(frameCount, w, h, testFlags, S.rays, S.T, nBatch, 1);
+                const unsigned ring = (unsigned)(g.streamBatches % (unsigned long long)Context::kStreamRing);
+                S.rays = g.dRaysStream + ring * Context::kStreamBatchMax;
+                S.limit = g.streamCutPreset >= 0 && g.streamCutPreset < nBatch ? g.streamCutPreset : nBatch;
+                S.cut = g.hStreamCut + ring;
+                if ((rc = armStreamCut(ring, S.limit))) return rc;
+                rc = enqueueTrace(frameCount, w, h, testFlags, S.rays, S.T, nBatch, 1, nullptr, nullptr, S.cut);
                 if (rc == kRefused && localRows(h) * (long long)w * g.spp >= kStreamLaunchSamples) {
                     nBatch = 1;
                 } else if (rc) {
                     return rc;
                 } else if (S.T.valid) {
                     g.streamBatches++;
-                    g.streamNext = frameCount + nBatch;
+                    g.streamCutPreset = -1;
+                    g.lastStreamRays = S.rays;
+                    g.streamNext = frameCount + S.limit;
                     if ((rc = Q.push(S))) return rc;
                     Q.serveFront(false, T, rays);
                 }
@@ -972,6 +992,14 @@
     return 0;
 }
 
+int tptGetStreamCutInfo(int64_t* launchesCut, int64_t* framesCut)
+{
+    if (requireInit()) return -1;
+    if (launchesCut) *launchesCut = (int64_t)g.streamLaunchesCut;
+    if (framesCut) *framesCut = (int64_t)g.streamFramesCut;
+    return 0;
+}
+
 int tptSetTileMirror(float* deviceMirror, void* deviceCounterOut)
 {
     g.mirror = deviceMirror;
@@ -1013,6 +1041,7 @@
 {
     if (int rc_ = flushShardDeferred()) return rc_;
     if (requireInit()) return -1;
+    g.pending.closeStream();
     HIPCHK(hipEventRecord(g.ev1, g.stream));
     if (int rc = launchTailHelpers()) return rc;
     HIPCHK(hipEventSynchronize(g.ev1));
diff --git a/toypathtracer_amd/csrc/tpt_host_shard.cpp b/toypathtracer_amd/csrc/tpt_host_shard.cpp
--- a/toypathtracer_amd/csrc/tpt_host_shard.cpp
+++ b/toypathtracer_amd/csrc/tpt_host_shard.cpp
@@ -237,6 +237,7 @@
     Context::Shard& S = g.shard;
     if (!S.active) return fail("tptShardedFinish: call tptCommInit first");
     if (int rc = flushShardDeferred()) return rc;
+    g.pending.closeStream();
     if (int rc = launchTailHelpers()) return rc;
     HIPCHK(hipStreamSynchronize(g.stream));
     HIPCHK(hipStreamSynchronize(S.commStream));
diff --git a/toypathtracer_amd/csrc/tpt_kernels.hip b/toypathtracer_amd/csrc/tpt_kernels.hip
--- a/toypathtracer_amd/csrc/tpt_kernels.hip
+++ b/toypathtracer_amd/csrc/tpt_kernels.hip
@@ -1184,7 +1184,7 @@
 #define TPT_Q_MAX_VGPR 60
 #endif
 template <bool LDS_SCENE, bool BATCH, bool VIEWS = false, bool MOVING = false, bool AOV = false, bool MOMENTS = false, bool ADAPTIVE = false,
-          bool CAMERAS = false>
+          bool CAMERAS = false, bool CUT = false>
 __device__ __forceinline__ void traceQueueBody(const KernelArgs& a)
 {
     extern __shared__ __attribute__((aligned(16))) unsigned char smem[];
@@ -1194,6 +1194,7 @@
     static_assert(!MOMENTS || AOV, "moments are summed beside the first-hit sums");
     static_assert(!ADAPTIVE || (MOMENTS && !BATCH), "a count per pixel belongs to a single frame with its moments");
     static_assert(!CAMERAS || (BATCH && MOVING && AOV && MOMENTS && !VIEWS && !ADAPTIVE), "a camera per frame belongs to the frames of a clip with their planes");
+    static_assert(!CUT || (BATCH && !VIEWS && !MOVING && !AOV), "a live frame limit belongs to the plain batched launch");
     constexpr bool CAM_TABLE = VIEWS || CAMERAS;
     constexpr int kPaths = (LDS_SCENE ? TPT_Q_PATHS : TPT_Q_PATHS_GROUPED) - (CAM_TABLE ? TPT_Q_VIEW_PATHS : 0) -
                            (MOVING ? TPT_Q_ANIM_PATHS : 0);
@@ -1290,6 +1291,7 @@
         ctl->globalExhausted = 0u;
     }
     if (BATCH && tid < 32) ctl->frameRays[tid] = 0u;
+    if (CUT && tid == 0) ctl->cutSeen = __hip_atomic_load(a.frameCut, __ATOMIC_RELAXED, __HIP_MEMORY_SCOPE_SYSTEM);
     __syncthreads();
 
     const FrameConsts& fc = a.fc;
@@ -1429,12 +1431,29 @@
                 if (chunkNext >= chunkEnd) {
                     if (noMoreChunks) break;
                     int c = 0;
+                    [[maybe_unused]] unsigned cut = 0xffffffffu;
                     if (lane == 0) {
                         atomicAdd(&ctl->poolTotal, 64u);
+                        if (CUT) {
+                            if (blockIdx.x == 0u) {
+                                cut = __hip_atomic_load(a.frameCut, __ATOMIC_RELAXED, __HIP_MEMORY_SCOPE_SYSTEM);
+                                if (cut < (unsigned)a.batchFrames)
+                                    __hip_atomic_store(&a.work[4], (unsigned)a.batchFrames - cut, __ATOMIC_RELAXED, __HIP_MEMORY_SCOPE_AGENT);
+                            } else {
+                                cut = (unsigned)a.batchFrames - __hip_atomic_load(&a.work[4], __ATOMIC_RELAXED, __HIP_MEMORY_SCOPE_AGENT);
+                            }
+                            const unsigned seen = __hip_atomic_load(&ctl->cutSeen, __ATOMIC_RELAXED, __HIP_MEMORY_SCOPE_WORKGROUP);
+                            cut = cut < seen ? cut : seen;
+                        }
                         c = (int)atomicAdd(&a.work[0], 1u);
                     }
                     c = __builtin_amdgcn_readfirstlane(c);
-                    if (c >= a.numChunks) {
+                    int chunkLimit = a.numChunks;
+                    if (CUT) {
+                        cut = (unsigned)__builtin_amdgcn_readfirstlane((int)cut);
+                        if (cut < (unsigned)a.batchFrames) chunkLimit = (int)cut * a.chunksPerFrame;
+                    }
+                    if (c >= chunkLimit) {
                         if (lane == 0) {
                             atomicSub(&ctl->poolTotal, 64u);
                             __hip_atomic_store(&ctl->globalExhausted, 1u, __ATOMIC_RELAXED, __HIP_MEMORY_SCOPE_WORKGROUP);
@@ -1711,6 +1730,7 @@
             }
             a.work[0] = 0u;
             a.work[1] = 0u;
+            if (CUT) a.work[4] = 0u;
         }
     }
 #if defined(__HIP_DEVICE_COMPILE__) && defined(TPT_STATS) && TPT_STATS >= 2
@@ -1758,21 +1778,21 @@
 {
     traceQueueBody<false, true>(a);
 }
-enum { QF_BATCH = 1, QF_VIEWS = 2, QF_MOVING = 4, QF_AOV = 8, QF_MOMENTS = 16, QF_ADAPTIVE = 32, QF_CAMERAS = 64 };
+enum { QF_BATCH = 1, QF_VIEWS = 2, QF_MOVING = 4, QF_AOV = 8, QF_MOMENTS = 16, QF_ADAPTIVE = 32, QF_CAMERAS = 64, QF_CUT = 128 };
 #define TPT_QUEUE_VARIANT_KERNEL(NAME, F)                                                                                                    \
     template <bool LDS_SCENE>                                                                                                                \
     __global__ void __launch_bounds__(TPT_Q_T, TPT_Q_MIN_WAVES_PER_SIMD) __attribute__((amdgpu_num_vgpr(TPT_Q_MAX_VGPR)))                    \
     NAME(const KernelArgs a)                                                                                                                 \
     {                                                                                                                                        \
         traceQueueBody<LDS_SCENE, ((F) & QF_BATCH) != 0, ((F) & QF_VIEWS) != 0, ((F) & QF_MOVING) != 0, ((F) & QF_AOV) != 0, ((F) & QF_MOMENTS) != 0, \
-                       ((F) & QF_ADAPTIVE) != 0, ((F) & QF_CAMERAS) != 0>(a);                                                                \
+                       ((F) & QF_ADAPTIVE) != 0, ((F) & QF_CAMERAS) != 0, ((F) & QF_CUT) != 0>(a);                                                                \
     }                                                                                                                                        \
     template <>                                                                                                                              \
     __global__ void __launch_bounds__(TPT_Q_T, TPT_Q_MIN_WAVES_PER_SIMD) __attribute__((amdgpu_num_vgpr(TPT_Q_MAX_VGPR_GROUPED)))            \
     NAME<false>(const KernelArgs a)                                                                                                          \
     {                                                                                                                                        \
         traceQueueBody<false, ((F) & QF_BATCH) != 0, ((F) & QF_VIEWS) != 0, ((F) & QF_MOVING) != 0, ((F) & QF_AOV) != 0, ((F) & QF_MOMENTS) != 0, \
-                       ((F) & QF_ADAPTIVE) != 0, ((F) & QF_CAMERAS) != 0>(a);                                                                \
+                       ((F) & QF_ADAPTIVE) != 0, ((F) & QF_CAMERAS) != 0, ((F) & QF_CUT) != 0>(a);                                                                \
     }
 TPT_QUEUE_VARIANT_KERNEL(tptTraceViewsKernel, QF_BATCH | QF_VIEWS)
 TPT_QUEUE_VARIANT_KERNEL(tptTraceAnimationKernel, QF_BATCH | QF_MOVING)
@@ -1781,6 +1801,7 @@
 TPT_QUEUE_VARIANT_KERNEL(tptTraceClipKernel, QF_BATCH | QF_MOVING | QF_AOV | QF_MOMENTS)
 TPT_QUEUE_VARIANT_KERNEL(tptTraceAdaptiveKernel, QF_AOV | QF_MOMENTS | QF_ADAPTIVE)
 TPT_QUEUE_VARIANT_KERNEL(tptCameraClipKernel, QF_BATCH | QF_MOVING | QF_AOV | QF_MOMENTS | QF_CAMERAS)
+TPT_QUEUE_VARIANT_KERNEL(tptStreamBatchKernel, QF_BATCH | QF_CUT)
 #undef TPT_QUEUE_VARIANT_KERNEL
 
 #if defined(TPT_TEST_HOOKS)
@@ -2035,6 +2056,7 @@
     };
     const QueueVariant variant = tptQueueVariant(a);
     if (variant == QV_INVALID) return hipErrorInvalidValue;
+    if (variant == QV_BATCH && a.frameCut) return launchQueueKernel(ldsScene ? tptStreamBatchKernel<true> : tptStreamBatchKernel<false>, a, blocks, lds, stream);
     return launchQueueKernel(kernel[variant][ldsScene ? 1 : 0], a, blocks, lds, stream);
 }
 #if defined(TPT_TEST_HOOKS)
diff --git a/toypathtracer_amd/csrc/tpt_queue_layout.h b/toypathtracer_amd/csrc/tpt_queue_layout.h
--- a/toypathtracer_amd/csrc/tpt_queue_layout.h
+++ b/toypathtracer_amd/csrc/tpt_queue_layout.h
@@ -75,6 +75,7 @@
     unsigned poolTotal;
     unsigned globalExhausted;
     unsigned frameRays[32];
+    unsigned cutSeen;
 };
 static_assert(sizeof(QueueCtl::frameRays) / 4 == TPT_Q_VIEWS_MAX, "one ray count per frame of a batch");
 static_assert(sizeof(tptLerpTable::v) / sizeof(float) == TPT_Q_VIEWS_MAX, "one lerp factor per frame of a batch");
```
